# USCCACS/RXMD

Measured on AMD Instinct MI355X. Metric: MD steps/sec (RDX, 979,776 atoms/GPU; one step advances every GPU's domain: weak scaling, wall-clock steps/s of the whole job), higher is better.
Workload: dtype f64

## Files before the change

include/rxmd_hip.h:

```cpp
#ifndef RXMD_HIP_H
#define RXMD_HIP_H
#ifdef __cplusplus
extern "C" {
#endif

typedef struct rxmd_hip_engine *rxmd_handle;

#define RXMD_OK 0
#define RXMD_E_ARG (-1)
#define RXMD_E_FFIELD (-2)
#define RXMD_E_NBUFFER (-3)
#define RXMD_E_MAXNEIGHBS (-4)
#define RXMD_E_MAXNEIGHBS10 (-5)
#define RXMD_E_HIP (-6)
#define RXMD_E_STATE (-7)
#define RXMD_E_COMM (-8)
#define RXMD_E_NAN (-9)

typedef struct rxmd_config {
  const char *ffield_path;
  double lattice[6];
  int vprocs[3];
  int myid;
  int isQEq;
  int NMAXQEq;
  double QEq_tol;
  int qstep;
  double dt_fs;
  double Lex_fqs, Lex_k;
  int nbuffer;
  int maxneighbs;
  int maxneighbs10;
  int device;
  int qeq_mode;
  int lg;
  const char *pqeq_path;
  int efield_dir;
  int reserved1;
  double efield_strength;
} rxmd_config;

void rxmd_hip_default_config(rxmd_config *cfg);
int rxmd_hip_create(const rxmd_config *cfg, rxmd_handle *out);
int rxmd_hip_destroy(rxmd_handle h);
const char *rxmd_hip_last_error(rxmd_handle h);

int rxmd_hip_set_atoms_rxff(rxmd_handle h, int natoms, const double *rec10);
int rxmd_hip_get_atoms_rxff(rxmd_handle h, double *rec10, int capacity);
int rxmd_hip_get_atoms(rxmd_handle h, int capacity, long long *gid, int *type, double *pos, double *v, double *f, double *q);
int rxmd_hip_set_charges(rxmd_handle h, int natoms, const double *q);
int rxmd_hip_set_velocities(rxmd_handle h, int natoms, const double *v);
int rxmd_hip_get_shells(rxmd_handle h, double *spos3, int capacity);
int rxmd_hip_get_bonds(rxmd_handle h, int capacity, int maxnb, int *count, long long *partner_gid, double *bo);
int rxmd_hip_set_shells(rxmd_handle h, int natoms, const double *spos3);

int rxmd_hip_qeq(rxmd_handle h, int *iters, double *est);
int rxmd_hip_force(rxmd_handle h, double pe[14]);
int rxmd_hip_step(rxmd_handle h, int nsteps);
int rxmd_hip_minimise(rxmd_handle h, double ftol, int max_loops, double *pe, long long *evaluations);
int rxmd_hip_last_qeq_iters(rxmd_handle h);
int rxmd_hip_thermostat(rxmd_handle h, int mdmode, double treq_K, double vsfact, double gke_per_atom);
int rxmd_hip_get_energy(rxmd_handle h, double *ke, double *qsum, double pe[14], double astr[6]);

int rxmd_hip_set_lattice(rxmd_handle h, const double lat[6]);
int rxmd_hip_get_lattice(rxmd_handle h, double lat[6]);
int rxmd_hip_set_barostat(rxmd_handle h, int mode, int axes, const double p0_GPa[3], double tau_fs, double bulk_modulus_GPa,
                          int every, double max_strain);
int rxmd_hip_get_barostat(rxmd_handle h, double p6_GPa[6], double mu[3], double *volume, long long *couplings);

int rxmd_hip_set_qeq_precision(rxmd_handle h, int matrix_bits);
int rxmd_hip_get_qeq_precision(rxmd_handle h, int *requested_bits, int *in_use_bits);

int rxmd_hip_QEq(rxmd_handle h, int nbuffer, int natoms, const double *atype, const double *pos, double *q);
int rxmd_hip_FORCE(rxmd_handle h, int nbuffer, int natoms, const double *atype, const double *pos, double *f, const double *q, double pe[14]);
int rxmd_hip_PQEq(rxmd_handle h, int nbuffer, int natoms, const double *atype, const double *pos, double *q, double *spos);
int rxmd_hip_FORCE_pqeq(rxmd_handle h, int nbuffer, int natoms, const double *atype, const double *pos, double *f, const double *q, const double *spos, double pe[14]);
int rxmd_hip_put_lex(rxmd_handle h, int natoms, const double *qsfp, const double *qsfv);
int rxmd_hip_get_lex(rxmd_handle h, int natoms, double *qsfp, double *qsfv);

int rxmd_hip_evaluate_device(rxmd_handle h, int natoms, const long long *gid, const int *type, const double *pos3, const double *q_in,
                             double *f3, double *q_out, double pe[14], double virial6[6], void *stream);

#define RXMD_BONDS_GID 1
long long rxmd_hip_get_bonds_device(rxmd_handle h, int flags, double bo_min, long long capacity, long long *src, long long *dst, double *bo,
                                    double *bo3, double *vec3, void *stream);

int rxmd_hip_bonds_vjp_device(rxmd_handle h, int flags, double bo_min, long long E, const double *grad_bo, const double *grad_bo3,
                              const double *grad_vec3, double *grad_pos3, void *stream);

typedef struct rxmd_stats {
  int natoms, nghost_qeq, nghost_force;
  long long nnz10;
  long long nbonds;
  int max_n10, max_nb;
  int qeq_iters_last; long long qeq_iters_total; long long qeq_calls;
  double ms_qeq, ms_qeq_list, ms_qeq_spmv, ms_force, ms_lists, ms_bo, ms_nonbond, ms_bonded, ms_step_total;
  long long spmv_launches;
  int n10_stride, nbuffer, cells10[3], cells3[3];
  int n_boundary_rows;
  int spmv_noop_launches;
  int reserved[6];
  double ms_ghost_build, ms_migrate, ms_halo, ms_halo_exposed, ms_allreduce, ms_fold;
  long long halo_calls, allreduce_calls;
  double ms_k_list10, ms_k_nonbond, ms_k_e3b, ms_k_e4b, ms_k_ehb, ms_k_bondorder, ms_k_assemble;
  double ms_k_winbuild;
  int win_groups, win_max_units, win_in_use, reserved2;
  double place_ms_first, place_ms_kept;
  double place_total_ms, place_bytes_held;
  int place_draws;
  int spmv_nstep, spmv_var, reserved3;
  double ms_k_blist;
  double ms_bond_exposed;
  int bond_overlap;
  long long spmv_launches_timed;
  int timer_pairs_dropped;
} rxmd_stats;
int rxmd_hip_get_stats(rxmd_handle h, rxmd_stats *out);
int rxmd_hip_reset_timers(rxmd_handle h);
int rxmd_hip_set_qeq_mode(rxmd_handle h, int mode);

int rxmd_hip_get_table(rxmd_handle h, int which, double *out, int capacity);
int rxmd_hip_get_cutoffs(rxmd_handle h, double *rc, int capacity, double *maxrc);
int rxmd_hip_debug_get(rxmd_handle h, int what, double *out, int capacity);

typedef struct rxmd_comm_ops {
  void *ctx;
  long long (*exchange)(void *ctx, int to, const double *send, long long nsend, int from, double *recv, long long cap);
  int (*allreduce_sum)(void *ctx, double *buf, int n);
  long long (*exchange_known)(void *ctx, int to, const double *send, long long nsend, int from, double *recv, long long nrecv);
} rxmd_comm_ops;
int rxmd_hip_set_comm(rxmd_handle h, const rxmd_comm_ops *ops);
int rxmd_hip_rccl_unique_id(unsigned char out128[128]);
int rxmd_hip_comm_init_rccl(rxmd_handle h, const unsigned char id128[128], int rank, int world);
int rxmd_hip_copy_to_host(const double *dev, double *host, long long ndoubles);
int rxmd_hip_copy_to_device(double *dev, const double *host, long long ndoubles);
int rxmd_hip_device_count(void);
int rxmd_hip_set_exchange_buffers(rxmd_handle h, double *send, double *recv, long long ndoubles);
int rxmd_host_comm_selftest(const rxmd_comm_ops *ops, int myid, int nprocs);

long long rxmd_host_geninit(const char *ffield_path, int natoms0, const char *elem4, const double *frac,
                            const double lattice[6], const int mc[3], const int vprocs[3], int myid,
                            double *rec10, long long capacity, double lattice_out[6]);
long long rxmd_host_read_rxff(const char *path, int myid, double lattice_out[6], int vprocs_out[3], double *rec10, long long capacity);
int rxmd_host_ffield_table(const char *ffield_path, const long long *natoms_per_type, int which, double *out, long long capacity);
int rxmd_host_ffield_lg(int on);
int rxmd_host_describe_options(char *buf, int capacity);
int rxmd_hip_has_device_code(void);

#ifdef __cplusplus
}
#endif
#endif
```

rxmd_amd/_lib.py:

```python
import ctypes as C
import os

HERE = os.path.dirname(os.path.abspath(__file__))
SO_PATH = os.environ.get("RXMD_HIP_LIB") or os.path.join(HERE, "librxmd_hip.so")


class RxmdConfig(C.Structure):
    _fields_ = [("ffield_path", C.c_char_p), ("lattice", C.c_double * 6), ("vprocs", C.c_int * 3), ("myid", C.c_int),
                ("isQEq", C.c_int), ("NMAXQEq", C.c_int), ("QEq_tol", C.c_double), ("qstep", C.c_int), ("dt_fs", C.c_double),
                ("Lex_fqs", C.c_double), ("Lex_k", C.c_double), ("nbuffer", C.c_int), ("maxneighbs", C.c_int),
                ("maxneighbs10", C.c_int), ("device", C.c_int), ("qeq_mode", C.c_int), ("lg", C.c_int),
                ("pqeq_path", C.c_char_p), ("efield_dir", C.c_int), ("reserved1", C.c_int), ("efield_strength", C.c_double)]


class RxmdStats(C.Structure):
    _fields_ = [("natoms", C.c_int), ("nghost_qeq", C.c_int), ("nghost_force", C.c_int), ("nnz10", C.c_longlong), ("nbonds", C.c_longlong),
                ("max_n10", C.c_int), ("max_nb", C.c_int), ("qeq_iters_last", C.c_int), ("qeq_iters_total", C.c_longlong), ("qeq_calls", C.c_longlong),
                ("ms_qeq", C.c_double), ("ms_qeq_list", C.c_double), ("ms_qeq_spmv", C.c_double), ("ms_force", C.c_double), ("ms_lists", C.c_double),
                ("ms_bo", C.c_double), ("ms_nonbond", C.c_double), ("ms_bonded", C.c_double), ("ms_step_total", C.c_double),
                ("spmv_launches", C.c_longlong), ("n10_stride", C.c_int), ("nbuffer", C.c_int), ("cells10", C.c_int * 3), ("cells3", C.c_int * 3),
                ("n_boundary_rows", C.c_int), ("spmv_noop_launches", C.c_int), ("reserved", C.c_int * 6),
                ("ms_ghost_build", C.c_double), ("ms_migrate", C.c_double), ("ms_halo", C.c_double), ("ms_halo_exposed", C.c_double),
                ("ms_allreduce", C.c_double), ("ms_fold", C.c_double), ("halo_calls", C.c_longlong), ("allreduce_calls", C.c_longlong),
                ("ms_k_list10", C.c_double), ("ms_k_nonbond", C.c_double), ("ms_k_e3b", C.c_double), ("ms_k_e4b", C.c_double), ("ms_k_ehb", C.c_double),
                ("ms_k_bondorder", C.c_double), ("ms_k_assemble", C.c_double), ("ms_k_winbuild", C.c_double),
                ("win_groups", C.c_int), ("win_max_units", C.c_int), ("win_in_use", C.c_int), ("reserved2", C.c_int),
                ("place_ms_first", C.c_double), ("place_ms_kept", C.c_double),
                ("place_total_ms", C.c_double), ("place_bytes_held", C.c_double), ("place_draws", C.c_int),
                ("spmv_nstep", C.c_int), ("spmv_var", C.c_int), ("reserved3", C.c_int), ("ms_k_blist", C.c_double),
                ("ms_bond_exposed", C.c_double), ("bond_overlap", C.c_int), ("spmv_launches_timed", C.c_longlong), ("timer_pairs_dropped", C.c_int)]

    def asdict(self):
        d = {}
        for name, _ in self._fields_:
            v = getattr(self, name)
            d[name] = list(v) if hasattr(v, "__len__") else v
        d.pop("reserved"); d.pop("reserved2"); d.pop("reserved3")
        return d


EXCHANGE_FN = C.CFUNCTYPE(C.c_longlong, C.c_void_p, C.c_int, C.c_void_p, C.c_longlong, C.c_int, C.c_void_p, C.c_longlong)
ALLREDUCE_FN = C.CFUNCTYPE(C.c_int, C.c_void_p, C.POINTER(C.c_double), C.c_int)


class RxmdCommOps(C.Structure):
    _fields_ = [("ctx", C.c_void_p), ("exchange", EXCHANGE_FN), ("allreduce_sum", ALLREDUCE_FN), ("exchange_known", EXCHANGE_FN)]


H = C.c_void_p
PD = C.c_void_p
SYMBOLS = [
    ("rxmd_hip_default_config", None, [C.POINTER(RxmdConfig)]),
    ("rxmd_hip_create", C.c_int, [C.POINTER(RxmdConfig), C.POINTER(H)]),
    ("rxmd_hip_destroy", C.c_int, [H]),
    ("rxmd_hip_last_error", C.c_char_p, [H]),
    ("rxmd_hip_set_atoms_rxff", C.c_int, [H, C.c_int, PD]),
    ("rxmd_hip_get_atoms_rxff", C.c_int, [H, PD, C.c_int]),
    ("rxmd_hip_get_atoms", C.c_int, [H, C.c_int, PD, PD, PD, PD, PD, PD]),
    ("rxmd_hip_set_charges", C.c_int, [H, C.c_int, PD]),
    ("rxmd_hip_set_velocities", C.c_int, [H, C.c_int, PD]),
    ("rxmd_hip_get_shells", C.c_int, [H, PD, C.c_int]),
    ("rxmd_hip_get_bonds", C.c_int, [H, C.c_int, C.c_int, C.c_void_p, C.c_void_p, PD]),
    ("rxmd_hip_set_shells", C.c_int, [H, C.c_int, PD]),
    ("rxmd_hip_qeq", C.c_int, [H, C.POINTER(C.c_int), C.POINTER(C.c_double)]),
    ("rxmd_hip_force", C.c_int, [H, PD]),
    ("rxmd_hip_step", C.c_int, [H, C.c_int]),
    ("rxmd_hip_get_energy", C.c_int, [H, C.POINTER(C.c_double), C.POINTER(C.c_double), PD, PD]),
    ("rxmd_hip_set_lattice", C.c_int, [H, PD]),
    ("rxmd_hip_get_lattice", C.c_int, [H, PD]),
    ("rxmd_hip_set_barostat", C.c_int, [H, C.c_int, C.c_int, PD, C.c_double, C.c_double, C.c_int, C.c_double]),
    ("rxmd_hip_get_barostat", C.c_int, [H, PD, PD, C.POINTER(C.c_double), C.POINTER(C.c_longlong)]),
    ("rxmd_hip_set_qeq_precision", C.c_int, [H, C.c_int]),
    ("rxmd_hip_get_qeq_precision", C.c_int, [H, C.POINTER(C.c_int), C.POINTER(C.c_int)]),
    ("rxmd_hip_QEq", C.c_int, [H, C.c_int, C.c_int, PD, PD, PD]),
    ("rxmd_hip_FORCE", C.c_int, [H, C.c_int, C.c_int, PD, PD, PD, PD, PD]),
    ("rxmd_hip_evaluate_device", C.c_int, [H, C.c_int, PD, PD, PD, PD, PD, PD, PD, PD, C.c_void_p]),
    ("rxmd_hip_get_bonds_device", C.c_longlong, [H, C.c_int, C.c_double, C.c_longlong, PD, PD, PD, PD, PD, C.c_void_p]),
    ("rxmd_hip_bonds_vjp_device", C.c_int, [H, C.c_int, C.c_double, C.c_longlong, PD, PD, PD, PD, C.c_void_p]),
    ("rxmd_hip_get_stats", C.c_int, [H, C.POINTER(RxmdStats)]),
    ("rxmd_hip_reset_timers", C.c_int, [H]),
    ("rxmd_hip_PQEq", C.c_int, [H, C.c_int, C.c_int, PD, PD, PD, PD]),
    ("rxmd_hip_FORCE_pqeq", C.c_int, [H, C.c_int, C.c_int, PD, PD, PD, PD, PD, PD]),
    ("rxmd_hip_put_lex", C.c_int, [H, C.c_int, PD, PD]),
    ("rxmd_hip_get_lex", C.c_int, [H, C.c_int, PD, PD]),
    ("rxmd_hip_minimise", C.c_int, [H, C.c_double, C.c_int, C.POINTER(C.c_double), C.POINTER(C.c_longlong)]),
    ("rxmd_hip_last_qeq_iters", C.c_int, [H]),
    ("rxmd_hip_thermostat", C.c_int, [H, C.c_int, C.c_double, C.c_double, C.c_double]),
    ("rxmd_hip_rccl_unique_id", C.c_int, [C.c_char_p]),
    ("rxmd_hip_comm_init_rccl", C.c_int, [H, C.c_char_p, C.c_int, C.c_int]),
    ("rxmd_hip_set_qeq_mode", C.c_int, [H, C.c_int]),
    ("rxmd_hip_get_table", C.c_int, [H, C.c_int, PD, C.c_int]),
    ("rxmd_hip_get_cutoffs", C.c_int, [H, PD, C.c_int, C.POINTER(C.c_double)]),
    ("rxmd_hip_debug_get", C.c_int, [H, C.c_int, PD, C.c_int]),
    ("rxmd_hip_set_comm", C.c_int, [H, C.POINTER(RxmdCommOps)]),
    ("rxmd_hip_copy_to_host", C.c_int, [PD, PD, C.c_longlong]),
    ("rxmd_hip_copy_to_device", C.c_int, [PD, PD, C.c_longlong]),
    ("rxmd_hip_device_count", C.c_int, []),
    ("rxmd_hip_set_exchange_buffers", C.c_int, [H, PD, PD, C.c_longlong]),
    ("rxmd_host_comm_selftest", C.c_int, [C.POINTER(RxmdCommOps), C.c_int, C.c_int]),
    ("rxmd_host_geninit", C.c_longlong, [C.c_char_p, C.c_int, C.c_char_p, PD, PD, PD, PD, C.c_int, PD, C.c_longlong, PD]),
    ("rxmd_host_read_rxff", C.c_longlong, [C.c_char_p, C.c_int, PD, PD, PD, C.c_longlong]),
    ("rxmd_host_ffield_table", C.c_int, [C.c_char_p, PD, C.c_int, PD, C.c_longlong]),
    ("rxmd_host_ffield_lg", C.c_int, [C.c_int]),
    ("rxmd_host_describe_options", C.c_int, [C.c_char_p, C.c_int]),
    ("rxmd_hip_has_device_code", C.c_int, []),
]


def describe_options():
    lib = load()
    n = lib.rxmd_host_describe_options(None, 0)
    buf = C.create_string_buffer(n + 1)
    lib.rxmd_host_describe_options(buf, n + 1)
    return buf.value.decode()

_lib = None


def load():
    global _lib
# ... 14 lines not shown
```

rxmd_amd/csrc/bonded.hip:

```cpp
#include "engine.h"

#include <hipcub/hipcub.hpp>

#include <algorithm>
#include <cstdlib>
#include <type_traits>

namespace rxmd {

static inline int nblk(long long n, int b) { return n > 0 ? static_cast<int>((n + b - 1) / b) : 1; }

static constexpr double MINBO0 = 1e-4, cutof2_esub = 1e-4;
static constexpr double MAXANGLE = 0.999999999999, MINANGLE = -0.999999999999, NSMALL = 1e-10;
static constexpr double PI_ = 3.14159265358979;

__device__ inline double wave_sum_b(double v) { return wave_sum64(v); }
__device__ inline void block_energy_add(double v, double *dst) {
  __shared__ double sm[8];
  v = wave_sum_b(v);
  const int w = threadIdx.x >> 6;
  __syncthreads();
  if ((threadIdx.x & 63) == 0) sm[w] = v;
  __syncthreads();
  if (threadIdx.x == 0) {
// ... 894 lines not shown
  }
  if (qn > 0) evaluate(qn);

  wave_lds_sync();
  const double a_cf = s_acc[w][lane][0], a_fx = s_acc[w][lane][1], a_fy = s_acc[w][lane][2], a_fz = s_acc[w][lane][3];
  const double a_cjk1 = s_acc[w][lane][4], a_cjk2 = s_acc[w][lane][5], a_cdk = s_acc[w][lane][6];
  if (sl_me < nj_me) {
    const int o = ob_me + sl_me;
    if (a_cf != 0.0 || a_cjk1 != 0.0) cf1[o] += a_cf + a_cjk1;
    if (a_cjk2 != 0.0) cf2[o] += a_cjk2;
    if (a_cdk != 0.0) cdn[o] += a_cdk;
    if (a_fx != 0.0 || a_fy != 0.0 || a_fz != 0.0) { fnx[o] += a_fx; fny[o] += a_fy; fnz[o] += a_fz; }
  }
  if (self_me) {
    double sx = a_fx, sy = a_fy, sz = a_fz, scd = a_cdk;
    if (ONCE) {
      const int gb = gbase(g_me);
      for (int t = 0; t < nj_me; ++t) { sx -= s_acc[w][gb + t][1]; sy -= s_acc[w][gb + t][2]; sz -= s_acc[w][gb + t][3]; scd += s_acc[w][gb + t][6]; }
    }
    cds[j_me] += scd;
    fx[j_me] += sx; fy[j_me] += sy; fz[j_me] += sz;
  }
  wave_lds_sync();
  }
  }
  e8 = wave_sum_b(e8); e9 = wave_sum_b(e9);
  if (lane == 0) {
    if (e8 != 0.0) atomicAdd(pe + 8, e8);
    if (e9 != 0.0) atomicAdd(pe + 9, e9);
  }
}

__global__ void __launch_bounds__(256) k_e4b_deliver(int nbonds, int TW, const double4 *__restrict__ tkl, unsigned *__restrict__ tflag4,
                                                      double *__restrict__ cf1, double *__restrict__ fnx, double *__restrict__ fny, double *__restrict__ fnz) {
  const int o = xcd_swizzle(blockIdx.x, gridDim.x) * blockDim.x + threadIdx.x;
  if (o >= nbonds) return;
  const int nw = TW >> 2;
  unsigned *fw = tflag4 + static_cast<size_t>(o) * nw;
  const double4 *row = tkl + static_cast<size_t>(o) * TW;
  double c = 0.0, f0 = 0.0, f1 = 0.0, f2 = 0.0;
  bool any = false;
  for (int wd = 0; wd < nw; ++wd) {
    unsigned m = fw[wd];
    if (m == 0u) continue;
    fw[wd] = 0u;
    any = true;
    for (int b = 0; b < 4; ++b, m >>= 8)
      if (m & 255u) { const double4 t = row[4 * wd + b]; c += t.x; f0 += t.y; f1 += t.z; f2 += t.w; }
  }
  if (any) { cf1[o] += c; fnx[o] += f0; fny[o] += f1; fnz[o] += f2; }
}

constexpr int EHB_CAP = 256;
constexpr int EHB_REGIONS = 64;
__global__ void __launch_bounds__(256) k_ehb_donors(int N, unsigned donor_types, const int *__restrict__ boff, const unsigned char *__restrict__ btype, const double *__restrict__ bo0,
                                                     const int *__restrict__ type, int2 *__restrict__ don, int *__restrict__ cnt, int region_cap) {
  const int i = blockIdx.x * blockDim.x + threadIdx.x, lane = threadIdx.x & 63, reg = blockIdx.x & (EHB_REGIONS - 1);
  unsigned hm = 0u;
  if (i < N && ((donor_types >> (type[i] & 31)) & 1u)) {
    const int ob = boff[i], n = min(boff[i + 1] - ob, 32);
    unsigned hs = 0u;
    for (int s = 0; s < n; ++s) hs |= (btype[ob + s] == 2 ? 1u : 0u) << s;
    for (unsigned m_ = hs; m_; m_ &= m_ - 1u) {
      const int s = __ffs(m_) - 1;
      if (bo0[ob + s] > MINBO0) hm |= 1u << s;
    }
  }
  const unsigned long long m = __ballot(hm != 0u);
  if (m == 0ULL) return;
  const int first = __ffsll(static_cast<long long>(m)) - 1;
  int base = 0;
  if (lane == first) base = atomicAdd(cnt + reg, __popcll(m));
  base = __shfl(base, first, 64);
  if (hm != 0u) don[static_cast<size_t>(reg) * region_cap + base + __popcll(m & ((1ULL << lane) - 1ULL))] = make_int2(i, static_cast<int>(hm));
}

template <bool SLOTS>
__global__ void __launch_bounds__(256) k_ehb_sweep(int S10, DevFF ff, const int2 *__restrict__ don, const int *__restrict__ ndon, int region_cap, const int *__restrict__ boff, const int *__restrict__ nbr,
                                                    const int *__restrict__ type, const double *__restrict__ x, const double *__restrict__ y, const double *__restrict__ z,
                                                    const double *__restrict__ bo0, const int *__restrict__ nb10, const int *__restrict__ n10, const double4 *__restrict__ pk, const int *__restrict__ perm,
                                                    double *__restrict__ cf1, double *__restrict__ fnx, double *__restrict__ fny, double *__restrict__ fnz,
                                                    double *__restrict__ fx, double *__restrict__ fy, double *__restrict__ fz, double *__restrict__ pe,
                                                    double *__restrict__ fsx, double *__restrict__ fsy, double *__restrict__ fsz,
                                                    const unsigned short *__restrict__ sl10, const int *__restrict__ rpos, const int *__restrict__ win_k, const unsigned char *__restrict__ stype, int G
#ifdef RXMD_EHB_DEBUG
                                                    , int *dbg, int lim_n, int lim_b, int lim_nb
#endif
                                                    ) {
#ifdef RXMD_EHB_DEBUG
#define EHB_CHECK(code, v, lim, aux) if ((v) < 0 || (v) >= (lim)) { if (atomicCAS(dbg, 0, (code)) == 0) { dbg[1] = (v); dbg[2] = (aux); dbg[3] = (lim); } return; }
#define EHB_CHECKC(code, v, lim, aux) if ((v) < 0 || (v) >= (lim)) { if (atomicCAS(dbg, 0, (code)) == 0) { dbg[1] = (v); dbg[2] = (aux); dbg[3] = (lim); } continue; }
#else
#define EHB_CHECK(code, v, lim, aux)
#define EHB_CHECKC(code, v, lim, aux)
#endif
  __shared__ unsigned s_cand[4][EHB_CAP];
  __shared__ double s_px[4][EHB_CAP], s_py[4][EHB_CAP], s_pz[4][EHB_CAP];
  __shared__ int s_k[4][EHB_CAP];
  __shared__ double s_hp[4][16][4];
  const int lane = threadIdx.x & 63, w = __builtin_amdgcn_readfirstlane(static_cast<int>(threadIdx.x >> 6));
  int pre = ndon[lane & (EHB_REGIONS - 1)];
#pragma unroll
  for (int o = 1; o < EHB_REGIONS; o <<= 1) { const int t = __shfl_up(pre, o, 64); if (lane >= o) pre += t; }
  const int nw = gridDim.x * 4, nd = __shfl(pre, EHB_REGIONS - 1, 64);
  double e10 = 0.0;
  for (int d = blockIdx.x * 4 + w; d < nd; d += nw) {
    const int reg = __popcll(__ballot(pre <= d));
    const int before = reg > 0 ? __shfl(pre, reg - 1, 64) : 0;
    const int2 rec = don[static_cast<size_t>(reg) * region_cap + (d - before)];
    const int i = __builtin_amdgcn_readfirstlane(rec.x);
    const unsigned hmask = static_cast<unsigned>(__builtin_amdgcn_readfirstlane(rec.y));
    EHB_CHECK(1, i, lim_n, d)
    const int ti = type[i], ob = boff[i], n = n10[i] & N10_COUNT;
    EHB_CHECK(2, ob, lim_b - 32, i)
    EHB_CHECK(3, n, S10 + 1, i)
    const double xi = x[i], yi = y[i], zi = z[i];
    const size_t row = static_cast<size_t>(i) * S10;
    const int *wk = SLOTS ? win_k + static_cast<size_t>(rpos[i] / WIN_ROWS) * WIN_MAXUNITS : nullptr;
    const int inx_l = (lane >= 1 && lane <= ff.nso && lane < 16) ? ff.inxn3hb[(ti * ff.n1 + 2) * ff.n1 + lane] : 0;
    if (lane < 16) { const DevHbP hp = ff.hb[inx_l]; s_hp[w][lane][0] = hp.r0hb; s_hp[w][lane][1] = hp.phb1; s_hp[w][lane][2] = hp.phb2; s_hp[w][lane][3] = hp.phb3; }
    int jl = 0; double bl = 0.0, xjl = 0.0, yjl = 0.0, zjl = 0.0;
    if (lane < 32 && ((hmask >> lane) & 1u)) { jl = nbr[ob + lane];
#ifdef RXMD_EHB_DEBUG
      if (jl < 0 || jl >= lim_nb) { if (atomicCAS(dbg, 0, 4) == 0) { dbg[1] = jl; dbg[2] = i; dbg[3] = lane; } jl = 0; }
#endif
      bl = bo0[ob + lane]; xjl = x[jl]; yjl = y[jl]; zjl = z[jl]; }
    V3 fi_t = {0, 0, 0};
    int qn = 0;

    auto flush = [&]() {
      wave_lds_sync();
      for (int q = lane; q < qn; q += 64) {
        EHB_CHECKC(5, static_cast<int>(s_cand[w][q] & NB10_IDX_MASK), lim_nb, i)
        const int ks = static_cast<int>(s_cand[w][q] & NB10_IDX_MASK);
        const double2 pxy = *reinterpret_cast<const double2 *>(pk + ks);
        s_px[w][q] = pxy.x; s_py[w][q] = pxy.y; s_pz[w][q] = reinterpret_cast<const double *>(pk + ks)[2]; s_k[w][q] = perm[ks];
      }
      wave_lds_sync();
      double akx[EHB_CAP / 64], aky[EHB_CAP / 64], akz[EHB_CAP / 64];
#pragma unroll
      for (int b = 0; b < EHB_CAP / 64; ++b) { akx[b] = 0.0; aky[b] = 0.0; akz[b] = 0.0; }
      for (unsigned hm = hmask; hm; hm &= hm - 1u) {
        const int s = __ffs(hm) - 1;
        const int j = __shfl(jl, s, 64);
        const double BOij = __shfl(bl, s, 64);
        const double xj = __shfl(xjl, s, 64), yj = __shfl(yjl, s, 64), zj = __shfl(zjl, s, 64);
        const V3 rij = {xi - xj, yi - yj, zi - zj};
        const double nij = sqrt(dot(rij, rij));
        double cfs = 0.0, nterm = 0.0;
        V3 fi_s = {0, 0, 0}, fj_s = {0, 0, 0};
#pragma unroll
        for (int b = 0; b < EHB_CAP / 64; ++b) {
          const int qq = 64 * b + lane;
          if (qq >= qn) continue;
          const int k = s_k[w][qq];
          if (k == j || k == i) continue;
          const double *hp = s_hp[w][(s_cand[w][qq] >> NB10_IDX_BITS) & 15u];
          const double r0hb = hp[0], phb1 = hp[1], phb2 = hp[2], phb3 = hp[3];
          const double pxk = s_px[w][qq], pyk = s_py[w][qq], pzk = s_pz[w][qq];
          const V3 rik = {xi - pxk, yi - pyk, zi - pzk};
          if (!(dot(rik, rik) < 100.0)) continue;
          const V3 rjk = {xj - pxk, yj - pyk, zj - pzk};
          const double njk = sqrt(dot(rjk, rjk));
          double cos_ijk = -dot(rij, rjk) / (nij * njk);
          if (cos_ijk > MAXANGLE) cos_ijk = MAXANGLE;
          if (cos_ijk < MINANGLE) cos_ijk = MINANGLE;
          const double sh2 = 0.5 * (1.0 - cos_ijk);
          const double sin_xhz4 = sh2 * sh2, cos_xhz1 = 1.0 - cos_ijk;
          const double exp_hb2 = exp(-phb2 * BOij);
          const double exp_hb3 = exp(-phb3 * (r0hb / njk + njk / r0hb - 2.0));
          const double PEhb = phb1 * (1.0 - exp_hb2) * exp_hb3 * sin_xhz4;
          e10 += PEhb; nterm += 1.0;
          cfs += phb1 * phb2 * exp_hb2 * exp_hb3 * sin_xhz4;
          const double CEhb2 = -0.5 * phb1 * (1.0 - exp_hb2) * exp_hb3 * cos_xhz1;
          const double CEhb3 = -PEhb * phb3 * (-r0hb / (njk * njk) + 1.0 / r0hb) * (1.0 / njk);
          V3 fi, fk;
          angle_forces(CEhb2, rij, nij, rjk, njk, fi, fk);
          const V3 ff3 = {CEhb3 * rjk.x, CEhb3 * rjk.y, CEhb3 * rjk.z};
          fi_s.x += fi.x; fi_s.y += fi.y; fi_s.z += fi.z;
          fj_s.x += -(fi.x + fk.x) - ff3.x; fj_s.y += -(fi.y + fk.y) - ff3.y; fj_s.z += -(fi.z + fk.z) - ff3.z;
          akx[b] += fk.x + ff3.x; aky[b] += fk.y + ff3.y; akz[b] += fk.z + ff3.z;
        }
        cfs = wave_sum_b(cfs); nterm = wave_sum_b(nterm);
        fj_s.x = wave_sum_b(fj_s.x); fj_s.y = wave_sum_b(fj_s.y); fj_s.z = wave_sum_b(fj_s.z);
        fi_t.x += fi_s.x; fi_t.y += fi_s.y; fi_t.z += fi_s.z;
        if (lane == 0 && nterm > 0.0) {
          const int o = ob + s;
          cf1[o] += cfs;
          fnx[o] += fj_s.x; fny[o] += fj_s.y; fnz[o] += fj_s.z;
        }
      }
#pragma unroll
      for (int b = 0; b < EHB_CAP / 64; ++b) {
        const int qq = 64 * b + lane;
        if (qq < qn && (akx[b] != 0.0 || aky[b] != 0.0 || akz[b] != 0.0)) {
          const int ks = static_cast<int>(s_cand[w][qq] & NB10_IDX_MASK);
          EHB_CHECKC(6, ks, lim_nb, qq)
          atomicAdd(fsx + ks, akx[b]); atomicAdd(fsy + ks, aky[b]); atomicAdd(fsz + ks, akz[b]);
        }
      }
// ... 52 lines not shown
  k_elnpr_atoms<<<nblk(N, 256), 256, 0, stream>>>(N, dff, boff, type, bt1, bt2, delta, deltalp, dDlp, ecoef, pe_d);
  k_elnpr_bonds<<<nblk(nbonds_res, 256), 256, 0, stream>>>(nbonds_res, dff, bown, nbr, btype, type, bo2, bo3, delta, deltalp, dDlp, ecoef, cf1, cf2, cf3, cdn);
  Timed kt3(this, &st.ms_k_e3b);
  if (opt.e3b_queue != 0 && dff.n1 <= 8 && dff.nvaty <= 255) {
    const int maxl = h_err[2];
    auto go = [&](auto kern, int na, int minw) {
      const int NG = nblk(N, 4 * na);
      kern<<<std::min(NG, (num_cu * minw + 7) & ~7), 256, 0, stream>>>(N, NG, dff, boff, nbr, btype, type, pos[0], pos[1], pos[2], bo0, bo2, bo3, delta, nlp, dDlp, epen, ecoa, cf1, cf2, cf3, cdn, fnx, fny, fnz,
                                                                     cds, frc[0], frc[1], frc[2], pe_d, static_cast<int>(opt.e4b_probe));
    };
    const bool w3 = opt.e3b_queue == 3;
    if (maxl <= 12) { if (w3) go(k_e3q<3, 16>, 16, 3); else go(k_e3q<2, 16>, 16, 2); }
    else if (maxl <= 24) { if (w3) go(k_e3q<3, 8>, 8, 3); else go(k_e3q<2, 8>, 8, 2); }
    else { if (w3) go(k_e3q<3, 4>, 4, 3); else go(k_e3q<2, 4>, 4, 2); }
  } else
    k_e3b<<<nblk(N, 256), 256, 4 * 5 * E3B_CAP * sizeof(double), stream>>>(N, dff, boff, nbr, btype, type, pos[0], pos[1], pos[2], bo0, bo2, bo3, delta, nlp, dDlp, epen, ecoa, cf1, cf2, cf3, cdn, fnx, fny, fnz,
                                          cds, frc[0], frc[1], frc[2], pe_d);
  RX_HIP(hipGetLastError());
  kt3.end();
  BoxImg bx;
  for (int a = 0; a < 3; ++a) { for (int c = 0; c < 3; ++c) { bx.H[3 * a + c] = box.H[a][c]; bx.Hi[3 * a + c] = box.Hi[a][c]; } bx.L[a] = box.lat[a]; }
  bx.ortho = grid.ortho; bx.probe = 0;
  bx.probe = static_cast<int>(opt.e4b_probe);
  const int want = static_cast<int>(opt.e4b_slots);
  const bool narrow = h_err[2] <= 15 && want != 32 && want != 4;
  Timed kt4(this, &st.ms_k_e4b);
  bool once = opt.e4b_once != 0;
  const int TW = (std::max(h_err[2], 8) + 3) & ~3;
  if (once) {
    const size_t need = static_cast<size_t>(std::max(nbonds, 1)) * TW;
    if (need > e4b_cap) {
      size_t fre = 0, tot = 0;
      RX_HIP(hipMemGetInfo(&fre, &tot));
      const size_t want_entries = need + need / 4;
      if (want_entries * 33 > (fre + e4b_cap * 33) / 2) once = false; else alloc_e4b_delivery(want_entries);
    }
  }
  if (once) {
    if (e4b_dirty) RX_HIP(hipMemsetAsync(e4b_flag, 0, e4b_cap, stream));
    e4b_dirty = true;
  }
  const int n4 = dff.n1 * dff.n1 * dff.n1 * dff.n1;
  const size_t tor_bytes = (dff.n1 <= 8 && dff.ntoty <= 255) ? static_cast<size_t>((n4 + 15) & ~15) : 0;
  const bool wpb1 = opt.e4b_wpb == 1;
  auto launch = [&](auto inst, int per_wave) {
    constexpr int L = decltype(inst)::value;
    auto go = [&](auto kern, int wpb) {
      const int VB = nblk(N, per_wave * wpb);
      const int grid = opt.e4b_persist != 0 ? std::min(VB, (num_cu * (12 / wpb) + 7) & ~7) : VB;
      kern<<<grid, 64 * wpb, tor_bytes, stream>>>(N, dff, boff, nbr, btype, nbrcnt, type, gid, pos[0], pos[1], pos[2], bo0, bo2, delta, etor, econ, cf1, cf2, cdn, fnx, fny, fnz,
                                                  cds, frc[0], frc[1], frc[2], pe_d, bx, brev, e4b_t, e4b_flag, TW, VB);
    };
    if (once) { if (wpb1) go(k_e4b<L, true, 1>, 1); else go(k_e4b<L, true, 4>, 4); }
    else      { if (wpb1) go(k_e4b<L, false, 1>, 1); else go(k_e4b<L, false, 4>, 4); }
    RX_HIP(hipGetLastError());
  };
  if (want == 4) launch(std::integral_constant<int, 1>{}, 4);
  else if (narrow && want != 16) launch(std::integral_constant<int, 0>{}, 8);
  else if (narrow) launch(std::integral_constant<int, 4>{}, 4);
  else launch(std::integral_constant<int, 5>{}, 2);
  if (once) {
    k_e4b_deliver<<<nblk(nbonds, 256), 256, 0, stream>>>(nbonds, TW, e4b_t, reinterpret_cast<unsigned *>(e4b_flag), cf1, fnx, fny, fnz);
    e4b_dirty = false;
  }
  kt4.end();
  Timed kth(this, &st.ms_k_ehb);
  if (ehb_donor_types != 0u) {
    const int region_cap = (nblk(N, 256) + EHB_REGIONS - 1) / EHB_REGIONS * 256;
    if (static_cast<size_t>(region_cap) * EHB_REGIONS > ehb_don_cap) throw EngineError(RXMD_E_STATE, "hydrogen-bond donor list: capacity");
    RX_HIP(hipMemsetAsync(ehb_cnt, 0, sizeof(int) * EHB_REGIONS, stream));
    k_ehb_donors<<<nblk(N, 256), 256, 0, stream>>>(N, ehb_donor_types, boff, btype, bo0, type, ehb_don, ehb_cnt, region_cap);
    k_zero3<<<nblk(G, 256), 256, 0, stream>>>(G, fsort[0], fsort[1], fsort[2]);
    if (ehb_blocks_per_cu == 0) {
      int nbk = 0;
      RX_HIP(hipOccupancyMaxActiveBlocksPerMultiprocessor(&nbk, k_ehb_sweep<false>, 256, 0));
      ehb_blocks_per_cu = std::max(nbk, 1);
      RX_HIP(hipOccupancyMaxActiveBlocksPerMultiprocessor(&nbk, k_ehb_sweep<true>, 256, 0));
      ehb_blocks_per_cu_sl = std::max(nbk, 1);
    }
    const bool slots = !nb10_valid;
    const int ehb_grid = num_cu * (slots ? ehb_blocks_per_cu_sl : ehb_blocks_per_cu);
#ifdef RXMD_EHB_DEBUG
    RX_HIP(hipMemsetAsync(ehb_cnt + EHB_REGIONS, 0, 4 * sizeof(int), stream));
#define RX_EHB(SL) k_ehb_sweep<SL><<<ehb_grid, 256, 0, stream>>>(S10, dff, ehb_don, ehb_cnt, region_cap, boff, nbr, type, pos[0], pos[1], pos[2], bo0, nb10, n10, sorted_xyzi, perm, cf1, fnx, fny, fnz, frc[0], frc[1], frc[2], pe_d, fsort[0], fsort[1], fsort[2], sl10, rpos, win_k, sorted_type, G, ehb_cnt + EHB_REGIONS, N, static_cast<int>(bcap), NB)
    if (slots) RX_EHB(true); else RX_EHB(false);
#undef RX_EHB
    { int hd[EHB_REGIONS + 4]; RX_HIP(hipMemcpyAsync(hd, ehb_cnt, sizeof(hd), hipMemcpyDeviceToHost, stream)); RX_HIP(hipStreamSynchronize(stream));
      for (int r = 1; r < EHB_REGIONS; ++r) hd[0] += hd[r];
      hd[4] = hd[EHB_REGIONS]; hd[5] = hd[EHB_REGIONS + 1]; hd[6] = hd[EHB_REGIONS + 2]; hd[7] = hd[EHB_REGIONS + 3];
      std::fprintf(stderr, "[ehb debug] donors %d  blocks/CU %d  first violation: code %d value %d aux %d lim %d   (N %d bcap %zu NB %d S10 %d rows10 %d)\n", hd[0], ehb_blocks_per_cu, hd[4], hd[5], hd[6], hd[7], N, bcap, NB, S10, rows10); }
#else
#define RX_EHB(SL) k_ehb_sweep<SL><<<ehb_grid, 256, 0, stream>>>(S10, dff, ehb_don, ehb_cnt, region_cap, boff, nbr, type, pos[0], pos[1], pos[2], bo0, nb10, n10, sorted_xyzi, perm, cf1, fnx, fny, fnz, frc[0], frc[1], frc[2], pe_d, fsort[0], fsort[1], fsort[2], sl10, rpos, win_k, sorted_type, G)
    if (slots) RX_EHB(true); else RX_EHB(false);
#undef RX_EHB
#endif
    k_add_sorted3<<<nblk(G, 256), 256, 0, stream>>>(G, perm, fsort[0], fsort[1], fsort[2], frc[0], frc[1], frc[2]);
  }
}

}
```

rxmd_amd/csrc/capi.hip:

```cpp
#include <algorithm>
#include <chrono>
#include <cmath>
#include <cstdio>
#include <cstring>
#include <fstream>
#include <new>
#include <string>
#include <vector>

#include "engine.h"

namespace rxmd { double stream_probe_ms(Engine &e, int blocks); void spmv_bisect_ms(Engine &e, double *out4); void spmv_isolated_ms(Engine &e, double *out); void spmv_tile_probe_ms(Engine &e, double *out); }
using rxmd::Engine;
using rxmd::EngineError;

struct rxmd_hip_engine {
  Engine *e = nullptr;
  std::string err;
};

static thread_local std::string g_create_error;

template <class F>
static int guarded(rxmd_handle h, F &&f) {
// ... 319 lines not shown
int rxmd_hip_QEq(rxmd_handle h, int nbuffer, int natoms, const double *atype, const double *pos, double *q) {
  if (!atype || !pos || !q) return RXMD_E_ARG;
  return guarded(h, [&](Engine &e) {
    require_lex(e, natoms);
    upload_reference_arrays(e, nbuffer, natoms, atype, pos, q);
    e.lex_pending = false;
    e.qeq();
    RX_HIP(hipMemcpy(q, e.q, sizeof(double) * natoms, hipMemcpyDeviceToHost));
  });
}

int rxmd_hip_FORCE(rxmd_handle h, int nbuffer, int natoms, const double *atype, const double *pos, double *f, const double *q, double pe[14]) {
  if (!atype || !pos || !f || !q) return RXMD_E_ARG;
  return guarded(h, [&](Engine &e) {
    upload_reference_arrays(e, nbuffer, natoms, atype, pos, q);
    e.force();
    for (int a = 0; a < 3; ++a)
      RX_HIP(hipMemcpy(f + a * static_cast<size_t>(nbuffer), e.frc[a], sizeof(double) * natoms, hipMemcpyDeviceToHost));
    if (pe) std::memcpy(pe, e.pe, sizeof(double) * 14);
  });
}

static void upload_shells(Engine &e, int nbuffer, int natoms, const double *spos) {
  if (!e.ff.pqeq) throw EngineError(RXMD_E_STATE, "the engine was created without a PQEq parameter file");
  for (int a = 0; a < 3; ++a) RX_HIP(hipMemcpy(e.shl[a], spos + a * static_cast<size_t>(nbuffer), sizeof(double) * natoms, hipMemcpyHostToDevice));
}
int rxmd_hip_PQEq(rxmd_handle h, int nbuffer, int natoms, const double *atype, const double *pos, double *q, double *spos) {
  if (!atype || !pos || !q || !spos) return RXMD_E_ARG;
  return guarded(h, [&](Engine &e) {
    require_lex(e, natoms);
    upload_reference_arrays(e, nbuffer, natoms, atype, pos, q);
    e.lex_pending = false;
    upload_shells(e, nbuffer, natoms, spos);
    e.qeq();
    RX_HIP(hipMemcpy(q, e.q, sizeof(double) * natoms, hipMemcpyDeviceToHost));
    for (int a = 0; a < 3; ++a) RX_HIP(hipMemcpy(spos + a * static_cast<size_t>(nbuffer), e.shl[a], sizeof(double) * natoms, hipMemcpyDeviceToHost));
  });
}
int rxmd_hip_FORCE_pqeq(rxmd_handle h, int nbuffer, int natoms, const double *atype, const double *pos, double *f, const double *q, const double *spos, double pe[14]) {
  if (!atype || !pos || !f || !q || !spos) return RXMD_E_ARG;
  return guarded(h, [&](Engine &e) {
    upload_reference_arrays(e, nbuffer, natoms, atype, pos, q);
    upload_shells(e, nbuffer, natoms, spos);
    e.force();
    for (int a = 0; a < 3; ++a)
      RX_HIP(hipMemcpy(f + a * static_cast<size_t>(nbuffer), e.frc[a], sizeof(double) * natoms, hipMemcpyDeviceToHost));
    if (pe) std::memcpy(pe, e.pe, sizeof(double) * 14);
  });
}

int rxmd_hip_evaluate_device(rxmd_handle h, int natoms, const long long *gid, const int *type, const double *pos3, const double *q_in,
                             double *f3, double *q_out, double pe[14], double virial6[6], void *stream) {
  return guarded(h, [&](Engine &e) { e.evaluate_device(natoms, gid, type, pos3, q_in, f3, q_out, pe, virial6, static_cast<hipStream_t>(stream)); });
}

long long rxmd_hip_get_bonds_device(rxmd_handle h, int flags, double bo_min, long long capacity, long long *src, long long *dst, double *bo,
                                    double *bo3, double *vec3, void *stream) {
  long long n = 0;
  const int rc = guarded(h, [&](Engine &e) { n = e.bonds_device(flags, bo_min, capacity, src, dst, bo, bo3, vec3, static_cast<hipStream_t>(stream)); });
  return rc < 0 ? rc : n;
}

int rxmd_hip_bonds_vjp_device(rxmd_handle h, int flags, double bo_min, long long E, const double *grad_bo, const double *grad_bo3,
                              const double *grad_vec3, double *grad_pos3, void *stream) {
  return guarded(h, [&](Engine &e) { e.bonds_vjp_device(flags, bo_min, E, grad_bo, grad_bo3, grad_vec3, grad_pos3, static_cast<hipStream_t>(stream)); });
}

int rxmd_hip_get_stats(rxmd_handle h, rxmd_stats *out) {
  if (!out) return RXMD_E_ARG;
  return guarded(h, [&](Engine &e) {
    if (e.atoms_set && e.lists_valid) {
      RX_HIP(hipStreamSynchronize(e.stream));
      e.collect_timers();
      std::vector<int> n10(e.N), nb(e.G);
      RX_HIP(hipMemcpy(n10.data(), e.n10, sizeof(int) * e.N, hipMemcpyDeviceToHost));
      RX_HIP(hipMemcpy(nb.data(), e.nbrcnt, sizeof(int) * e.G, hipMemcpyDeviceToHost));
      long long s10 = 0, sb = 0; int m10 = 0, mb = 0;
      for (int v : n10) { v &= rxmd::N10_COUNT; s10 += v; m10 = std::max(m10, v); }
      for (int v : nb) { sb += v; mb = std::max(mb, v); }
      e.st.nnz10 = s10; e.st.nbonds = sb; e.st.max_n10 = m10; e.st.max_nb = mb;
    }
    e.st.natoms = e.N;
    e.st.n_boundary_rows = (e.multi() && e.lists_valid && !e.rows_split_pending_invalid()) ? e.n_bnd : 0;
    e.st.win_groups = e.win_groups; e.st.win_max_units = e.win_maxunits; e.st.win_in_use = e.win_used ? 1 : 0;
    e.st.spmv_launches_timed = e.pass_timed_n;
    e.st.ms_qeq_spmv = e.pass_timed_n > 0 ? e.pass_timed_ms / static_cast<double>(e.pass_timed_n) * static_cast<double>(e.st.spmv_launches) : 0.0;
    *out = e.st;
  });
}

int rxmd_hip_reset_timers(rxmd_handle h) {
  return guarded(h, [&](Engine &e) {
    e.st.ms_qeq = e.st.ms_qeq_list = e.st.ms_qeq_spmv = e.st.ms_force = e.st.ms_lists = e.st.ms_bo = e.st.ms_nonbond = e.st.ms_bonded = e.st.ms_step_total = 0.0;
    e.st.spmv_launches = 0; e.st.spmv_noop_launches = 0; e.st.qeq_iters_total = 0; e.st.qeq_calls = 0;
    e.st.ms_ghost_build = e.st.ms_migrate = e.st.ms_halo = e.st.ms_halo_exposed = e.st.ms_allreduce = e.st.ms_fold = 0.0;
    e.st.halo_calls = e.st.allreduce_calls = 0; e.st.timer_pairs_dropped = 0; e.pass_timed_ms = 0.0; e.pass_timed_n = 0; e.st.spmv_launches_timed = 0;
    e.st.ms_k_list10 = e.st.ms_k_nonbond = e.st.ms_k_e3b = e.st.ms_k_e4b = e.st.ms_k_ehb = e.st.ms_k_bondorder = e.st.ms_k_assemble = e.st.ms_k_winbuild = e.st.ms_k_blist = e.st.ms_bond_exposed = 0.0;
  });
}

int rxmd_hip_set_qeq_mode(rxmd_handle h, int mode) {
  return guarded(h, [&](Engine &e) {
    if (mode != 0 && mode != 1) throw EngineError(RXMD_E_ARG, "qeq_mode must be 0 or 1");
    e.cfg.qeq_mode = mode;
  });
}

int rxmd_hip_get_table(rxmd_handle h, int which, double *out, int capacity) {
  int n = 0;
  const int rc = guarded(h, [&](Engine &e) {
    if (!e.tables_ready) throw EngineError(RXMD_E_STATE, "tables are built when atoms are first set");
    n = e.ff.nboty;
    if (!out || capacity < n * rxmd::NTABLE) throw EngineError(RXMD_E_ARG, "capacity too small");
    const std::vector<double> *src[5] = {&e.ff.tblEvdw, &e.ff.tbldEvdw, &e.ff.tblEclmb, &e.ff.tbldEclmb, &e.ff.tblQEq};
    if (which < 0 || which > 4) throw EngineError(RXMD_E_ARG, "which must be 0..4");
    for (int r = 1; r <= n; ++r)
      for (int i = 1; i <= rxmd::NTABLE; ++i) out[static_cast<size_t>(r - 1) * rxmd::NTABLE + (i - 1)] = (*src[which])[static_cast<size_t>(r) * (rxmd::NTABLE + 2) + i];
  });
  return rc < 0 ? rc : n;
}

int rxmd_hip_get_cutoffs(rxmd_handle h, double *rc, int capacity, double *maxrc) {
  int n = 0;
  const int r = guarded(h, [&](Engine &e) {
    if (!e.tables_ready) throw EngineError(RXMD_E_STATE, "cutoffs are computed when atoms are first set");
    n = e.ff.nboty;
    if (rc) { if (capacity < n) throw EngineError(RXMD_E_ARG, "capacity too small"); for (int k = 1; k <= n; ++k) rc[k - 1] = e.ff.bond[k].rc; }
    if (maxrc) *maxrc = e.ff.maxrc;
  });
  return r < 0 ? r : n;
}

int rxmd_hip_debug_get(rxmd_handle h, int what, double *out, int capacity) {
  int n = 0;
  const int rc = guarded(h, [&](Engine &e) {
    if (!e.atoms_set) throw EngineError(RXMD_E_STATE, "atoms were never set");
    RX_HIP(hipStreamSynchronize(e.stream));
    auto pull_d = [&](const double *src, int cnt, int stride, int off) {
      std::vector<double> t(cnt);
      RX_HIP(hipMemcpy(t.data(), src, sizeof(double) * cnt, hipMemcpyDeviceToHost));
      for (int i = 0; i < cnt; ++i) out[static_cast<size_t>(i) * stride + off] = t[i];
    };
    const int G = e.G, N = e.N;
    switch (what) {
      case 0: n = G; if (capacity < n) throw EngineError(RXMD_E_ARG, "capacity"); pull_d(e.delta, G, 1, 0); break;
      case 1: n = G; if (capacity < n) throw EngineError(RXMD_E_ARG, "capacity"); pull_d(e.deltap, G, 1, 0); break;
      case 2: { n = G; if (capacity < n) throw EngineError(RXMD_E_ARG, "capacity"); std::vector<int> t(G); RX_HIP(hipMemcpy(t.data(), e.nbrcnt, sizeof(int) * G, hipMemcpyDeviceToHost)); for (int i = 0; i < G; ++i) out[i] = t[i]; break; }
      case 3: n = G; if (capacity < 3 * n) throw EngineError(RXMD_E_ARG, "capacity"); for (int a = 0; a < 3; ++a) pull_d(e.pos[a], G, 3, a); break;
      case 4: { n = G; if (capacity < n) throw EngineError(RXMD_E_ARG, "capacity"); std::vector<long long> t(G); RX_HIP(hipMemcpy(t.data(), e.gid, sizeof(long long) * G, hipMemcpyDeviceToHost)); for (int i = 0; i < G; ++i) out[i] = static_cast<double>(t[i]); break; }
      case 5: { n = G; if (capacity < n) throw EngineError(RXMD_E_ARG, "capacity"); std::vector<int> t(G); RX_HIP(hipMemcpy(t.data(), e.type, sizeof(int) * G, hipMemcpyDeviceToHost)); for (int i = 0; i < G; ++i) out[i] = t[i]; break; }
      case 6: { n = N; if (capacity < n) throw EngineError(RXMD_E_ARG, "capacity"); std::vector<int> t(N); RX_HIP(hipMemcpy(t.data(), e.n10, sizeof(int) * N, hipMemcpyDeviceToHost)); for (int i = 0; i < N; ++i) out[i] = t[i] & rxmd::N10_COUNT; break; }
      case 7: {
        n = N; if (capacity < n) throw EngineError(RXMD_E_ARG, "capacity");
        std::vector<int> c(N); RX_HIP(hipMemcpy(c.data(), e.n10, sizeof(int) * N, hipMemcpyDeviceToHost));
        for (int &v : c) v &= rxmd::N10_COUNT;
        std::vector<double> row(e.S10);
        for (int i = 0; i < N; ++i) {
          RX_HIP(hipMemcpy(row.data(), e.hess + static_cast<size_t>(i) * e.S10, sizeof(double) * c[i], hipMemcpyDeviceToHost));
          double s = 0; for (int k = 0; k < c[i]; ++k) s += row[k];
          out[i] = s;
        }
        break;
      }
      case 8: n = G; if (capacity < n) throw EngineError(RXMD_E_ARG, "capacity"); pull_d(e.cd, G, 1, 0); break;
      case 9: n = G; if (capacity < n) throw EngineError(RXMD_E_ARG, "capacity"); pull_d(e.q, G, 1, 0); break;
      case 10: n = G; if (capacity < n) throw EngineError(RXMD_E_ARG, "capacity"); pull_d(e.cc_, G, 1, 0); break;
      case 14: {
        n = 2; if (capacity < 2) throw EngineError(RXMD_E_ARG, "capacity");
        out[0] = rxmd::poison_enabled() ? 1.0 : 0.0;
        RX_HIP(hipMemcpy(out + 1, e.hess + (e.S10 - 1), sizeof(double), hipMemcpyDeviceToHost));
        break;
      }
      case 15: n = 2; if (capacity < 2) throw EngineError(RXMD_E_ARG, "capacity"); out[0] = e.nb10_valid ? 1.0 : 0.0; out[1] = e.nb10_sticky ? 1.0 : 0.0; break;
      case 13: {
        n = static_cast<int>(e.est_trace.size()); if (capacity < n) throw EngineError(RXMD_E_ARG, "capacity");
        for (int k = 0; k < n; ++k) out[k] = e.est_trace[k];
        break;
      }
      case 11: {
        n = N; if (capacity < n) throw EngineError(RXMD_E_ARG, "capacity");
        if (!e.win_valid) { for (int i = 0; i < N; ++i) out[i] = -1.0; break; }
        e.require_nb10();
        RX_HIP(hipStreamSynchronize(e.stream));
        const size_t nrs = static_cast<size_t>(e.win_groups) * rxmd::WIN_ROWS;
        std::vector<int> c(N), rs(nrs), wc(e.win_groups), wk(static_cast<size_t>(e.win_groups) * rxmd::WIN_MAXUNITS);
        RX_HIP(hipMemcpy(c.data(), e.n10, sizeof(int) * N, hipMemcpyDeviceToHost));
        RX_HIP(hipMemcpy(rs.data(), e.rows_sorted, sizeof(int) * nrs, hipMemcpyDeviceToHost));
        RX_HIP(hipMemcpy(wc.data(), e.win_cnt, sizeof(int) * e.win_groups, hipMemcpyDeviceToHost));
        RX_HIP(hipMemcpy(wk.data(), e.win_k, sizeof(int) * wk.size(), hipMemcpyDeviceToHost));
        std::vector<int> ent(e.S10); std::vector<unsigned short> sl(e.S10);
        for (int i = 0; i < N; ++i) out[i] = -2.0;
        for (size_t r = 0; r < nrs; ++r) {
          const int i = rs[r], g = static_cast<int>(r / rxmd::WIN_ROWS);
          if (i < 0 || i >= N) continue;
          const int cnt = c[i] & rxmd::N10_COUNT;
          RX_HIP(hipMemcpy(ent.data(), e.nb10 + static_cast<size_t>(i) * e.S10, sizeof(int) * cnt, hipMemcpyDeviceToHost));
          RX_HIP(hipMemcpy(sl.data(), e.sl10 + static_cast<size_t>(i) * e.S10, sizeof(unsigned short) * cnt, hipMemcpyDeviceToHost));
          int good = 0;
          for (int k = 0; k < cnt; ++k) {
            const unsigned en = static_cast<unsigned>(ent[k]);
            const int slot = sl[k] & 0x7fff, unit = slot / rxmd::WIN_UNIT;
            const bool gh = (sl[k] & 0x8000) != 0;
            if (unit < wc[g] && wk[static_cast<size_t>(g) * rxmd::WIN_MAXUNITS + unit] + (slot % rxmd::WIN_UNIT) == static_cast<int>(en & rxmd::NB10_IDX_MASK) && gh == ((en & rxmd::NB10_GHOST) != 0)) ++good;
          }
          out[i] = good;
        }
        break;
      }
      case 12: {
        n = 4; if (capacity < 8) throw EngineError(RXMD_E_ARG, "capacity");
        const int grids[4] = {2048, 8192, 32768, 131072};
        for (int g = 0; g < 4; ++g) { out[2 * g] = rxmd::stream_probe_ms(e, grids[g]); out[2 * g + 1] = static_cast<double>(e.rows10) * e.S10 * 8.0; }
        n = 8; break;
      }
#ifdef RXMD_EXPERIMENTS
      case 104: n = 20; if (capacity < 20) throw EngineError(RXMD_E_ARG, "capacity"); rxmd::spmv_isolated_ms(e, out); break;
      case 105: n = 5; if (capacity < 5) throw EngineError(RXMD_E_ARG, "capacity"); rxmd::spmv_tile_probe_ms(e, out); break;
      case 102: n = 7; if (capacity < 7) throw EngineError(RXMD_E_ARG, "capacity"); rxmd::spmv_bisect_ms(e, out); break;
#endif
      default: throw EngineError(RXMD_E_ARG, "unknown debug tap");
    }
  });
  return rc < 0 ? rc : n;
}

int rxmd_hip_copy_to_host(const double *dev, double *host, long long n) {
  if (n < 0 || (n > 0 && (!dev || !host))) return RXMD_E_ARG;
  return (n == 0 || hipMemcpy(host, dev, sizeof(double) * static_cast<size_t>(n), hipMemcpyDeviceToHost) == hipSuccess) ? RXMD_OK : RXMD_E_HIP;
}
int rxmd_hip_copy_to_device(double *dev, const double *host, long long n) {
  if (n < 0 || (n > 0 && (!dev || !host))) return RXMD_E_ARG;
  return (n == 0 || hipMemcpy(dev, host, sizeof(double) * static_cast<size_t>(n), hipMemcpyHostToDevice) == hipSuccess) ? RXMD_OK : RXMD_E_HIP;
}
int rxmd_hip_device_count(void) {
  int n = 0;
  return hipGetDeviceCount(&n) == hipSuccess ? n : 0;
}

int rxmd_hip_set_comm(rxmd_handle h, const rxmd_comm_ops *ops) {
  return guarded(h, [&](Engine &e) {
    if (!ops) { e.has_comm = false; return; }
    e.comm = *ops; e.has_comm = true;
  });
}

int rxmd_hip_comm_init_rccl(rxmd_handle h, const unsigned char id128[128], int rank, int world) {
  return guarded(h, [&](Engine &e) {
    if (!id128) throw EngineError(RXMD_E_ARG, "NULL unique id");
    e.rccl_init(id128, rank, world);
  });
}

int rxmd_hip_set_exchange_buffers(rxmd_handle h, double *send, double *recv, long long ndoubles) {
  return guarded(h, [&](Engine &e) {
    if (!send || !recv || ndoubles < 1024) throw EngineError(RXMD_E_ARG, "bad exchange buffers");
    e.bufs.free_group(rxmd::G_XBUF);
    e.xbuf_send = send; e.xbuf_recv = recv; e.xbuf_doubles = static_cast<size_t>(ndoubles); e.xbuf_owned = false;
  });
}

int rxmd_host_comm_selftest(const rxmd_comm_ops *ops, int myid, int nprocs) {
  if (!ops || !ops->exchange || !ops->allreduce_sum || nprocs < 1 || myid < 0 || myid >= nprocs) return RXMD_E_ARG;
  const int right = (myid + 1) % nprocs, left = (myid + nprocs - 1) % nprocs;
  std::vector<double> snd(4096), rcv(4096);
  for (int dir = 0; dir < 2; ++dir) {
    const int to = dir ? left : right, from = dir ? right : left;
    const long long ns = 7 + 13 * myid + dir;
    for (long long k = 0; k < ns; ++k) snd[k] = 1000.0 * myid + k + 0.5 * dir;
    const long long nr = ops->exchange(ops->ctx, to, snd.data(), ns, from, rcv.data(), 4096);
    if (nr != 7 + 13 * from + dir) return RXMD_E_COMM;
    for (long long k = 0; k < nr; ++k) if (rcv[k] != 1000.0 * from + k + 0.5 * dir) return RXMD_E_COMM;
    const long long nz = ops->exchange(ops->ctx, to, snd.data(), 0, from, rcv.data(), 4096);
    if (nz != 0) return RXMD_E_COMM;
    if (ops->exchange_known) {
      const long long nk = ops->exchange_known(ops->ctx, to, snd.data(), ns, from, rcv.data(), 7 + 13 * from + dir);
      if (nk != 7 + 13 * from + dir) return RXMD_E_COMM;
      for (long long k = 0; k < nk; ++k) if (rcv[k] != 1000.0 * from + k + 0.5 * dir) return RXMD_E_COMM;
    }
  }
  double v[3] = {1.0 * (myid + 1), 0.25, -2.0 * myid};
// ... 105 lines not shown
```

rxmd_amd/csrc/engine.h:

```cpp
#pragma once
#include <hip/hip_runtime.h>

#include <string>
#include <type_traits>
#include <vector>

#include "../../include/rxmd_hip.h"
#include "ffparams.h"
#include "options.h"

namespace rxmd {

#define RX_HIP(call)                                                                              \
  do {                                                                                            \
    hipError_t e_ = (call);                                                                       \
    if (e_ != hipSuccess) throw EngineError(RXMD_E_HIP, std::string(#call) + ": " + hipGetErrorString(e_)); \
  } while (0)

struct EngineError {
  int code;
  std::string msg;
  EngineError(int c, std::string m) : code(c), msg(std::move(m)) {}
};

// ... 28 lines not shown
struct Box {
  double H[3][3], Hi[3][3];
  double lat[6];
  double lbox[3];
  double obox[3];
  double volume;
};

struct Grid {
  int n[3];
  double org[3];
  double inv[3];
  int ncell;
  int fz, nzf;
  int nfine;
  double wid[3];
  double cw[3];
  double iwz;
  int ortho;
  int probe;
};

struct RefMesh {
  double Hi[9], obox[3];
  double lc[3];
  double nbl[3];
  double nblr[3];
  double qlo[3], qhi[3];
};

constexpr int WAVE = 64;

enum { S_MU = 0, S_LMIN_S, S_LMIN_T, S_GOLD_S, S_GOLD_T, S_GNEW_S, S_GNEW_T, S_EST, S_GH_S, S_GH_T, S_HSH_S, S_HSH_T, S_SSUM, S_TSUM, S_BETA_S, S_BETA_T, S_RAW0, S_RAW1, S_RAW2, S_RAW3, S_RAW4, S_RAW5, S_RAW6, S_RAW7, S_STOP, S_STOP1, S_TOL, S_COUNT };
constexpr int SCAL_CG_N = 32, SCAL_N = 208, H_SCAL_N = 320;
constexpr int SCAL_PE = 32, SCAL_PE_N = 16, H_SCAL_PE = 32;
constexpr int SCAL_ASTR = 48;
constexpr int SCAL_PRINTE = 56, H_SCAL_PRINTE = 56;
constexpr int SCAL_REDUCE = 64, H_SCAL_REDUCE = 48;
constexpr int SCAL_EVAL_HEAD = 72, H_SCAL_EVAL_VIRIAL = 310;
constexpr int H_SCAL_TOL = 60;
constexpr int S_SNAP = 128, S_SNAP_STRIDE = 32;
constexpr int H_SCAL_SNAP = 64, H_SNAP_STRIDE = 64, H_SNAP_SEQ = 63;
constexpr int H_SCAL_TSUM = 192, H_SCAL_TSUM_N = 6 * 16;
constexpr int SCAL_BAR_HEAD = 192, SCAL_BAR_STEP = 200, H_SCAL_BAR_OUT = 288, H_SCAL_BAR_REDUCE = 304;
struct ScalSlot { int at, n; };
constexpr bool slots_disjoint_within(const ScalSlot *s, int count, int total) {
  for (int i = 0; i < count; ++i) for (int j = 0; j <= i; ++j)
    if (s[i].at < 0 || s[i].n <= 0 || s[i].at + s[i].n > total || (j < i && s[i].at < s[j].at + s[j].n && s[j].at < s[i].at + s[i].n)) return false;
  return true;
}
constexpr ScalSlot SCAL_SLOTS[] = {{0, SCAL_CG_N}, {SCAL_PE, SCAL_PE_N}, {SCAL_ASTR, 6}, {SCAL_PRINTE, 6}, {SCAL_REDUCE, 8}, {SCAL_EVAL_HEAD, 6}, {S_SNAP, 2 * S_SNAP_STRIDE}, {SCAL_BAR_HEAD, 6}, {SCAL_BAR_STEP, 6}};
constexpr ScalSlot H_SCAL_SLOTS[] = {{0, SCAL_CG_N}, {H_SCAL_PE, SCAL_PE_N}, {H_SCAL_REDUCE, 8}, {H_SCAL_PRINTE, 2}, {H_SCAL_TOL, 1}, {H_SCAL_SNAP, 2 * H_SNAP_STRIDE}, {H_SCAL_TSUM, H_SCAL_TSUM_N}, {H_SCAL_BAR_OUT, 9}, {H_SCAL_BAR_REDUCE, 6}, {H_SCAL_EVAL_VIRIAL, 6}};
static_assert(slots_disjoint_within(SCAL_SLOTS, sizeof(SCAL_SLOTS) / sizeof(ScalSlot), SCAL_N), "two slots of the device scalar block overlap, or one leaves the block");
static_assert(slots_disjoint_within(H_SCAL_SLOTS, sizeof(H_SCAL_SLOTS) / sizeof(ScalSlot), H_SCAL_N), "two slots of the pinned scalar block overlap, or one leaves the block");
static_assert(S_COUNT <= SCAL_CG_N && S_COUNT <= S_SNAP_STRIDE && S_COUNT <= H_SNAP_SEQ, "the CG scalars fit their range and either snapshot slot");
static_assert(S_RAW0 + 8 <= S_STOP, "the eight raw sums stay inside the CG scalars");

__device__ inline int xcd_swizzle(int bid, int nwg) {
  const int q = nwg >> 3, r = nwg & 7, x = bid & 7;
  return (x < r ? x * (q + 1) : r * (q + 1) + (x - r) * q) + (bid >> 3);
}

template <int CTRL, int ROW_MASK>
__device__ inline double dpp_move(double v) {
  const int lo = __double2loint(v), hi = __double2hiint(v);
  if (ROW_MASK == 0xf) return __hiloint2double(__builtin_amdgcn_mov_dpp(hi, CTRL, ROW_MASK, 0xf, false), __builtin_amdgcn_mov_dpp(lo, CTRL, ROW_MASK, 0xf, false));
  return __hiloint2double(__builtin_amdgcn_update_dpp(0, hi, CTRL, ROW_MASK, 0xf, false), __builtin_amdgcn_update_dpp(0, lo, CTRL, ROW_MASK, 0xf, false));
}
__device__ inline double wave_sum64(double v) {
  v += dpp_move<0xb1, 0xf>(v);
  v += dpp_move<0x4e, 0xf>(v);
  v += dpp_move<0x141, 0xf>(v);
  v += dpp_move<0x140, 0xf>(v);
  v += dpp_move<0x142, 0xa>(v);
  v += dpp_move<0x143, 0xc>(v);
  return __hiloint2double(__builtin_amdgcn_readlane(__double2hiint(v), 63), __builtin_amdgcn_readlane(__double2loint(v), 63));
}

#ifndef WIN_ROWS_DEF
#define WIN_ROWS_DEF 16
#endif
constexpr int WIN_ROWS = WIN_ROWS_DEF;
constexpr int WIN_UNIT = 8;
constexpr int WIN_MAXUNITS = 448;
constexpr int WIN_BMW = 2048;

enum class Fill : unsigned char { None, Zero, Pattern };
void *dev_alloc(size_t bytes, Fill fill);
void dev_free(void *p);
void *pinned_alloc(size_t bytes, bool coherent_mapped);
void pinned_free(void *p);
bool poison_enabled();
template <class T> void dev_alloc(T *&p, size_t n, Fill fill) { p = static_cast<T *>(dev_alloc(n * sizeof(T), fill)); }
template <class T> void dev_free(T *&p) { dev_free(static_cast<void *>(p)); p = nullptr; }

struct Engine;
enum class Dim : unsigned char { Fixed, NB, Rows10, List10, Cap };
enum class Refill : unsigned char { Never, Whole, Ghosts };
enum class Space : unsigned char { Device, Pinned, PinnedCoherent };
enum { G_SETUP, G_BOND, G_WIN, G_CELLSTART, G_LIST10, G_PARTIALS, G_ON_DEMAND, G_CUBTMP = G_ON_DEMAND, G_FFBLOB, G_PQBLOB, G_E4B, G_SEG, G_SEG_PINNED, G_XBUF, G_DH_SERVE, G_BGRAPH, G_BVJP, G_COUNT };
enum : unsigned { BUF_PQEQ = 1u, BUF_RESIDENT = 2u, BUF_QEQ_F32 = 4u };
struct Buf { void **pp; size_t elem; int group; Dim dim; size_t mul, add_; Fill fill; Refill refill; unsigned flags; Space space; size_t bytes; };
struct Buffers {
  std::vector<Buf> v;
  size_t cap[G_COUNT] = {};
  template <class T> void add(T *&p, int group, Dim dim, size_t mul, size_t addend, Fill fill, Refill refill, unsigned flags = 0) {
    size_t elem = 1;
    if constexpr (!std::is_void_v<T>) elem = sizeof(T);
    add_raw(reinterpret_cast<void **>(&p), elem, group, dim, mul, addend, fill, refill, flags);
  }
  void add_raw(void **pp, size_t elem, int group, Dim dim, size_t mul, size_t addend, Fill fill, Refill refill, unsigned flags = 0) {
    v.push_back(Buf{pp, elem, group, dim, mul, addend, fill, refill, flags, Space::Device, 0});
  }
  template <class T> void add_pinned(T *&p, int group, size_t n, bool coherent_mapped) {
    v.push_back(Buf{reinterpret_cast<void **>(&p), sizeof(T), group, Dim::Fixed, 0, n, Fill::Zero, Refill::Never, 0u, coherent_mapped ? Space::PinnedCoherent : Space::Pinned, 0});
  }
  size_t count(const Buf &b, const Engine &e) const;
  void alloc_one(Buf &b, const Engine &e); void free_one(Buf &b);
  void alloc_setup(const Engine &e);
  void alloc_group(const Engine &e, int group, size_t capacity = 0);
  void free_group(int group); void free_all();
  void refill(const Engine &e);
  std::vector<std::vector<char>> save_residents(const Engine &e) const;
  void restore_residents(const std::vector<std::vector<char>> &h);
};
constexpr size_t EHB_DON_EXTRA = 64 * 256 + 256;

template <class T> struct Restore {
  T &ref; const T old;
  explicit Restore(T &r) : ref(r), old(r) {}
  Restore(T &r, T inside) : ref(r), old(r) { r = inside; }
  ~Restore() { ref = old; }
};
struct StreamSwap {
  hipStream_t &a, &b; bool *inside;
  StreamSwap(hipStream_t &a_, hipStream_t &b_, bool *inside_ = nullptr) : a(a_), b(b_), inside(inside_) { std::swap(a, b); if (inside) *inside = true; }
  ~StreamSwap() { if (inside) *inside = false; std::swap(a, b); }
};

struct ScaleArgs;
struct WinPassArgs; struct RowPassArgs;
struct Engine {
  const Options opt = Options::from_env();
  rxmd_config cfg{};
  std::string ffield_path, pqeq_path, err;
  ForceField ff;
  Box box{};
  int vID[3] = {0, 0, 0}, target_node[7] = {0}, nprocs = 1;
  double dt = 0, Lex_w2 = 0;
  std::vector<double> dthm, hmas;
  rxmd_comm_ops comm{};
  bool has_comm = false, tables_ready = false, atoms_set = false, lists_valid = false, ghosts_valid = false;

  int NB = 0, MAXNB = 30, S10 = 0, rows10 = 0;
  int max_row10 = 0, min_row10 = 0;
  int num_cu = 256;
  int N = 0, G = 0, copyptr[7] = {0};
  int cc[3] = {1, 1, 1};
  double shell[3] = {0, 0, 0};
  Grid grid{};
  RefMesh rmesh{};

  Buffers bufs;
  void declare_buffers();
  DevFF dff{};
  void *ffblob = nullptr, *pqblob = nullptr;
// ... 90 lines not shown
  long long bonds_device(int flags, double bo_min, long long capacity, long long *src_d, long long *dst_d, double *bo_d, double *bo3_d, double *vec3_d, hipStream_t user);
  int *bg_flag = nullptr, *bg_off = nullptr;
  long long select_bonds(double bo_min);
  void bonds_vjp_device(int flags, double bo_min, long long E, const double *grad_bo_d, const double *grad_bo3_d, const double *grad_vec3_d, double *grad_pos3_d, hipStream_t user);
  double *bv_c1 = nullptr, *bv_c2 = nullptr, *bv_c3 = nullptr, *bv_t = nullptr, *bv_cc = nullptr, *bv_g[3] = {nullptr, nullptr, nullptr}; int bv_nb = 0;
  void build_ghosts_and_lists(bool qeq_prepass = false);
  void qeq_start_vectors();
  int *rows_int = nullptr, *rows_bnd = nullptr; int n_bnd = 0; bool rows_split_pending = false;
  bool rows_split_pending_invalid() const { return n_bnd < 0 || n_bnd > N; }
  bool sums_from_list = false;
  void qeq();
  struct WinInstance { int nstep, var; bool f32; };
  WinInstance win_instance() const;
  WinPassArgs win_args(bool roword = false) const;
  RowPassArgs row_args() const;
  struct PassCall { int mode; bool store; double2 *ra = nullptr, *rg = nullptr; const int *rowlist = nullptr; int nrows = 0, pbase = 0; const double *stopflag = nullptr; bool roword = false; };
  int matrix_pass(const PassCall &c);
  void cg_reduce(int stage, int nsets, const double *stopflag = nullptr);
  struct CgCall { int nmax, vb, vb_upd; bool onepass, runahead, est_with_update, cg_scatter; };
  double qeq_start(const CgCall &c);
  int qeq_runahead(const CgCall &c, double &Est);
  int qeq_host_paced(const CgCall &c, double &Est);
  struct TimedSection;
  void qeq_finish(int it, double Est, TimedSection &t_qeq);
  void force(bool defer_host_read = false, bool observe_energy = true);
  void finish_force();
  bool force_pending = false;
  unsigned long long snap_seq = 0; double snap_expect[2] = {0.0, 0.0};
  void wait_snapshot(int parity, double seq);
  unsigned long long pass_counter = 0; bool pass_timed_k[2] = {false, false}; double pass_timed_ms = 0.0; long long pass_timed_n = 0;
  void step(int nsteps);
  void migrate();
  void thermostat(int mdmode, double treq_K, double vsfact, double gke);
  int minimise(double ftol, int max_loops, double *pe_final, long long *evaluations);

  void set_lattice(const double lat[6], bool check_ranks);
  void apply_lattice(const double lat[6]);
  void check_lattice(const double lat[6]) const;
  struct BoxGeom { int cc[3]; double shell[3]; Grid grid; RefMesh rmesh; };
  BoxGeom geometry_for(const Box &b) const;
  void derive_box_geometry();
  long long capacity_want(const double shell_n[3]) const;
  void grow_capacity(int new_nb);
  void alloc_window_groups(size_t ng);
  size_t cellstart_cap = 0, win_ng_cap = 0;
  long long nsize_setup = 0;
  int bar_mode = 0, bar_axes = 7, bar_every = 1;
  double bar_p0[3] = {0, 0, 0}, bar_tau = 0, bar_B = 0, bar_max = 0;
  double bar_p6[6] = {0, 0, 0, 0, 0, 0}, bar_mu[3] = {1, 1, 1}, bar_vol = 0;
  long long bar_couplings = 0;
  void set_barostat(int mode, int axes, const double p0[3], double tau_fs, double bulk_GPa, int every, double max_strain);
  void barostat_couple();

  void setup_after_atoms(const std::vector<long long> &natoms_per_type_global);
  void upload_ff();
  void alloc_device();
  void free_device();
  void ghost_build();
  void ghost_build_fused(); void migrate_fused(); void ensure_seg_buffers(int nblocks);
  unsigned long long *h_pub = nullptr; unsigned pub_seq = 0u;
  void pinned_wait(int nwords, unsigned seq, const char *what);
  int *seg_cnt = nullptr, *seg_tot = nullptr, *h_seg = nullptr; unsigned char *seg_code_ = nullptr; int seg_blocks_cap = 0;
  void bin_cells();
  void build_bonded_list(bool pack_only = false);
  void build_list10();
  void build_prologue(int what);
  bool list10_retry = false;
  void build_windows();
  void tune_window_placement();
  bool place_tuned = false;
  int *rows_sorted = nullptr, *win_k = nullptr, *win_cnt = nullptr;
  int *win_flag = nullptr;
  int *rowcols = nullptr, *grp_base = nullptr;
  int *win_gint = nullptr, *win_gbnd = nullptr; int win_nbnd = 0;
  unsigned short *sl10 = nullptr;
  double2 *r_qst = nullptr, *r_hst = nullptr, *r_hst2 = nullptr, *r_gst = nullptr, *r_sall = nullptr, *r_sgh = nullptr, *r_wall = nullptr, *r_wgh = nullptr;
  bool rows_live = false;
  int *r_type = nullptr, *r_n10 = nullptr, *r_xpos = nullptr, *rpos = nullptr, *g_rrow = nullptr;
  int win_groups = 0, win_maxunits = 0;
  size_t win_groups_bound(long long n) const { return win_groups_bound_for(grid, n); }
  static size_t win_groups_bound_for(const Grid &g, long long n) { return static_cast<size_t>(n) / WIN_ROWS + static_cast<size_t>(g.n[0]) * g.n[1] + 1; }
  double qeq_iters_smooth = -1.0;
  bool win_valid = false, win_used = false;
  void halo_refresh(double2 *v2, double *v1);
  void halo_staged(double *v, int ncomp);
  struct Round { int d0, n; };
  bool stage_pairs = true;
  bool known_counts_pair() const { return stage_pairs && (nccl || (has_comm && comm.exchange_known)); }
  int *flags2 = nullptr, *scanout2 = nullptr;
  int *sel_flags(int k) const { return k ? flags2 : flags; }
  int *sel_scan(int k) const { return k ? scanout2 : scanout; }
  int stage_sends(int d) const { return sendoff[d + 1] - sendoff[d]; }
  int stage_ghosts(int d) const { return copyptr[d] - copyptr[d - 1]; }
  void select_round(Round r, int nscan, double dr, int skip_dead, int total[2]);
  void exchange_round(Round r, bool reverse, const long long nsend[2], long long nrecv[2], bool counts_known);
  void rccl_exchange_round(int n, const int to[2], const int from[2], const long long nsend[2], long long nrecv[2], bool counts_known);
  long long *gowner = nullptr;
  bool halo_direct = false, dh_ready = false;
  int *dh_ghost = nullptr, *dh_serve = nullptr;
  int *dh_keys = nullptr, *dh_keys2 = nullptr, *dh_vals = nullptr, *dh_off = nullptr; int dh_serve_cap = 0;
  std::vector<long long> dh_need_off, dh_serve_off;
  void direct_halo_setup();
  void halo_direct_exchange(double *v, int ncomp);
  void exchange_many(const std::vector<long long> &soff, const std::vector<long long> &roff, int ncomp);
  void rccl_exchange_many(const std::vector<long long> &soff, const std::vector<long long> &roff, int ncomp);
  void ensure_xbuf(size_t doubles);
  size_t migrate_xbuf_doubles(size_t from_send_count) const;
  void grow_xbuf_keep_send(size_t need, size_t keep);
  bool multi() const { return nprocs > 1 || force_staged; }
  void *nccl = nullptr; double *cnt_dev = nullptr, *cnt_host = nullptr; bool force_staged = false, force_remote = false;
  void rccl_init(const unsigned char id128[128], int rank, int world);
  void rccl_destroy();
  void rccl_allreduce_dev(double *dev, int n);
  void sync_stream();
  void sync_event(hipEvent_t e);
  double comm_timeout_s = 300.0;
  bool spin_wait = true;
  void allreduce_scal4(int n = 4);
  void allreduce_host(double *buf, int n);
  void allreduce_device(double *dev, int n, int h_stage, int site = -1);
  void ghost_build_staged();
  void sorted_copy(const double2 *v);
  void fold_ghost_forces(double *fx, double *fy, double *fz);
  void bond_orders();
  void bonded_energies();
  void charge_halo();
  void nonbonded(bool to_fnb = false, bool energy = true);
  void pqeq_sorted_shells();
  void pqeq_update_shells();
  bool pq_matrix_stale = false;
  void nonbonded_pqeq();
  void efield_force();
  void remove_momentum();
  void type_sums_device();
  double *tsum = nullptr; struct ScaleArgs *sargs = nullptr;
  void assemble_forces();
  void accumulate_stress(bool kinetic);
  void check_device_error(const char *where, bool fetch = true);
  void fetch_device_error();
  double reduce_partials(int ncomp, int nblocks, double *out);
  struct KtPair { hipEvent_t a = nullptr, b = nullptr; double *dst = nullptr, *dst2 = nullptr; long long *cnt = nullptr; double scale = 1.0; };
  std::vector<KtPair> kt_free, kt_pending;
  KtPair kt_cur{};
  unsigned long long kt_site_calls[4] = {0, 0, 0, 0};
  int kt_every = 1, kt_phase = 0;
  struct Timed {
    Engine &e; const bool section; KtPair p{};
    Timed(Engine *eng, double *dst, double *dst2 = nullptr, long long *cnt = nullptr, int site = -1, bool section_ = false) : e(*eng), section(section_) {
      double scale = 1.0;
      if (!section && site < 0 && e.kt_every > 1) {
        if (cnt) { *cnt += 1; cnt = nullptr; }
        if (e.kt_phase % e.kt_every != 0) return;
        scale = static_cast<double>(e.kt_every);
      }
      if (site >= 0) {
        if (cnt) { *cnt += 1; cnt = nullptr; }
        const unsigned long long every = static_cast<unsigned long long>(e.opt.pass_timing_every > 1 ? e.opt.pass_timing_every : 1);
        if ((e.kt_site_calls[site & 3]++ % every) != 0) return;
        scale = static_cast<double>(every);
      }
      if (e.kt_free.empty() || (!section && e.kt_cur.a)) { if (e.kt_free.empty()) ++e.st.timer_pairs_dropped; return; }
      p = e.kt_free.back(); e.kt_free.pop_back();
      p.dst = dst; p.dst2 = dst2; p.cnt = cnt; p.scale = scale;
      hipEventRecord(p.a, e.stream);
      if (!section) e.kt_cur = p;
    }
// ... 20 lines not shown
```

rxmd_amd/csrc/engine.hip:

```cpp
#include "engine.h"
#include <cstdlib>

#include <hipcub/hipcub.hpp>

#include <algorithm>
#include <cmath>
#include <cstring>

namespace rxmd {

static const double UTIME = 1e3 / 20.455;
static const int NMINCELL = 4;
static inline int nblk(long long n, int b) { return n > 0 ? static_cast<int>((n + b - 1) / b) : 1; }


static void make_box(Box &b, const double lat[6], const int vprocs[3], const int vID[3]) {
  const double pi = std::atan(1.0) * 4.0;
  const double la = lat[0], lb = lat[1], lc = lat[2];
  const double lal = lat[3] * pi / 180.0, lbe = lat[4] * pi / 180.0, lga = lat[5] * pi / 180.0;
  const double hh1 = lc * (std::cos(lal) - std::cos(lbe) * std::cos(lga)) / std::sin(lga);
  const double hh2 = lc * std::sqrt(1.0 - std::cos(lal) * std::cos(lal) - std::cos(lbe) * std::cos(lbe) - std::cos(lga) * std::cos(lga) +
                                    2 * std::cos(lal) * std::cos(lbe) * std::cos(lga)) / std::sin(lga);
  double(*H)[3] = b.H;
  H[0][0] = la; H[1][0] = 0; H[2][0] = 0;
// ... 487 lines not shown
}
__global__ void k_sorted_pos(int G, int N, const int *perm, const int *groot, const double *x, const double *y, const double *z, const int *type, double4 *out, unsigned char *st, int *rootperm, int *invpos) {
  const int k = blockIdx.x * blockDim.x + threadIdx.x;
  if (k >= G) return;
  const int i = perm[k];
  const double xi = x[i], yi = y[i], zi = z[i];
  const int ti = type[i];
  out[k] = make_double4(xi, yi, zi, __longlong_as_double((static_cast<long long>(ti) << 32) | static_cast<unsigned int>(i)));
  st[k] = static_cast<unsigned char>(ti);
  rootperm[k] = (i < N) ? i : groot[i];
  invpos[i] = k;
}
__global__ void k_sorted_vec(int G, const int *__restrict__ rootperm, const double2 *__restrict__ v, double2 *__restrict__ xs) {
  const int k = blockIdx.x * blockDim.x + threadIdx.x;
  if (k < G) xs[k] = v[rootperm[k]];
}

void Engine::bin_cells() {
  k_cell_ids<<<nblk(G, 256), 256, 0, stream>>>(G, grid, spos[0], spos[1], spos[2], cellid, perm_in);
  size_t tb = cubtmp_bytes;
  int bits = 1;
  while ((1LL << bits) < grid.nfine + 1 && bits < 31) ++bits;
  RX_HIP(hipcub::DeviceRadixSort::SortPairs(cubtmp, tb, cellid, cellid_sorted, perm_in, perm, G, 0, bits, stream));
  k_cell_starts<<<nblk(grid.nfine + 1, 256), 256, 0, stream>>>(G, grid.nfine, cellid_sorted, cellstart);
  sorted_positions();
  if (ff.pqeq) pqeq_sorted_shells();
}
void Engine::sorted_positions() {
  k_sorted_pos<<<nblk(G, 256), 256, 0, stream>>>(G, N, perm, groot, pos[0], pos[1], pos[2], type, sorted_xyzi, sorted_type, rootperm, invpos);
  sorted_w_charge = false;
}

void Engine::sorted_copy(const double2 *v) {
  if (multi()) {
    halo_staged(reinterpret_cast<double *>(const_cast<double2 *>(v)), 2);
    k_sorted_vec<<<nblk(G, 256), 256, 0, stream>>>(G, perm, v, xs);
    return;
  }
  k_sorted_vec<<<nblk(G, 256), 256, 0, stream>>>(G, rootperm, v, xs);
}

__global__ void k_publish_words(int n, const int *__restrict__ src, unsigned long long *hpub, unsigned seq) {
  if (threadIdx.x < n) __hip_atomic_store(hpub + threadIdx.x, (static_cast<unsigned long long>(seq) << 32) | static_cast<unsigned>(src[threadIdx.x]), __ATOMIC_RELAXED, __HIP_MEMORY_SCOPE_SYSTEM);
}
void Engine::build_ghosts_and_lists(bool qeq_prepass) {
  if (!atoms_set) throw EngineError(RXMD_E_STATE, "atoms were never set");
  TimedSection t_lists(this, &st.ms_lists);
  bufs.refill(*this);
  { Timed kt(this, &st.ms_ghost_build); ghost_build(); }
  bin_cells();
  build_prologue(3);
  { Timed kt(this, &st.ms_k_blist); build_bonded_list(); }
  sums_from_list = qeq_prepass;
  if (qeq_prepass) qeq_start_vectors();
  build_list10();
  if (h_pub && !multi()) {
    const unsigned seq = ++pub_seq;
    k_publish_words<<<1, 64, 0, stream>>>(16, d_err, h_pub, seq);
    pinned_wait(16, seq, "list build");
    for (int k = 0; k < 16; ++k) h_err[k] = static_cast<int>(h_pub[k] & 0xffffffffull);
  } else
    fetch_device_error();
  if (static_cast<size_t>(h_err[7]) > bcap) {
    free_bond_tables();
    alloc_bond_tables(static_cast<size_t>(h_err[7]) + static_cast<size_t>(h_err[7]) / 4 + 4096);
    build_bonded_list(true);
    fetch_device_error();
  }
  try {
    check_device_error("list build", false);
  } catch (const EngineError &er) {
    if (er.code != RXMD_E_MAXNEIGHBS10 || cfg.maxneighbs10 > 0) { collect_timers(); throw; }
    const int need = h_err[1];
    S10 = (static_cast<int>(need * 1.1) + 64 + 63) / 64 * 64;
    bufs.free_group(G_LIST10); bufs.alloc_group(*this, G_LIST10);
    st.n10_stride = S10;
    { Restore<bool> retry(list10_retry, true); build_list10(); }
    check_device_error("list build");
  }
  nbonds = h_err[7]; nbonds_res = h_err[9];
  win_groups = h_err[8];
  max_row10 = h_err[3]; min_row10 = std::min(h_err[4], h_err[3]);
  win_maxunits = h_err[5]; win_valid = win_groups > 0 && h_err[6] == 0 && win_maxunits > 0 && (!multi() || (win_nbnd >= 0 && win_nbnd <= win_groups)) && !opt.spmv_no_win;
  lists_valid = true;
  if (!nb10_valid && !win_valid) require_nb10();
  collect_timers();
  pq_matrix_stale = false;
}

void Engine::set_qeq_precision(int bits) {
  if (bits != 64 && bits != 32) throw EngineError(RXMD_E_ARG, "matrix_bits must be 64 or 32");
  if (bits == 32 && ff.pqeq) throw EngineError(RXMD_E_ARG, "the fp32 matrix stream is not available with PQEq (it carries a second value stream)");
  if (bits == qeq_bits_req) return;
  qeq_bits_req = bits;
  lists_valid = false;
  if (hess) {
    sync_stream();
    bufs.free_group(G_LIST10); bufs.alloc_group(*this, G_LIST10);
    nb10_valid = false;
  }
}

struct Mat3 { double m[9]; };
__global__ void k_affine_remap(int n, Mat3 M, double *__restrict__ x, double *__restrict__ y, double *__restrict__ z,
                               double *__restrict__ dx, double *__restrict__ dy, double *__restrict__ dz) {
  const int i = blockIdx.x * blockDim.x + threadIdx.x;
  if (i >= n) return;
  const double r0 = x[i], r1 = y[i], r2 = z[i];
  x[i] = M.m[0] * r0 + M.m[1] * r1 + M.m[2] * r2;
  y[i] = M.m[3] * r0 + M.m[4] * r1 + M.m[5] * r2;
  z[i] = M.m[6] * r0 + M.m[7] * r1 + M.m[8] * r2;
  if (dx) {
    const double d0 = dx[i], d1 = dy[i], d2 = dz[i];
    dx[i] = M.m[0] * d0 + M.m[1] * d1 + M.m[2] * d2;
    dy[i] = M.m[3] * d0 + M.m[4] * d1 + M.m[5] * d2;
    dz[i] = M.m[6] * d0 + M.m[7] * d1 + M.m[8] * d2;
  }
}

void Engine::check_lattice(const double lat[6]) const {
  if (!lattice_spans_box(lat)) throw EngineError(RXMD_E_ARG, "lattice does not span a box (edges must be positive, angles inside (0,180) and not coplanar)");
  if (tables_ready)
    for (int a = 0; a < 3; ++a)
      if (static_cast<int>(lat[a] / cfg.vprocs[a] / ff.maxrc) < 1) throw EngineError(RXMD_E_ARG, "local box smaller than the bond cutoff");
  if (bar_mode == 2 && !lattice_orthorhombic(lat)) throw EngineError(RXMD_E_ARG, "the per-axis barostat (mode 2) is on: the lattice must stay orthorhombic");
}

long long Engine::capacity_want(const double shell_n[3]) const {
  const long long nsize = std::max<long long>(nsize_setup, N);
  double fac = 1.0;
  for (int a = 0; a < 3; ++a) fac *= 1.0 + 2.0 * std::min(shell_n[a] / box.lbox[a], 1.0);
  const long long want = static_cast<long long>(nsize * fac * 1.12) + 4096;
  return std::min<long long>(want, 2000000000LL);
}

void Engine::set_lattice(const double lat[6], bool check_ranks) {
  bool local_ok = true;
  std::string why;
  try { check_lattice(lat); } catch (const EngineError &er) { if (nprocs == 1 || !check_ranks) throw; local_ok = false; why = er.msg; }
  if (check_ranks && nprocs > 1) {
    double s[7];
    for (int a = 0; a < 6; ++a) s[a] = cfg.myid == 0 ? lat[a] : 0.0;
    s[6] = local_ok ? 0.0 : 1.0;
    allreduce_host(s, 7);
    double bad = 0.0;
    for (int a = 0; a < 6; ++a) if (!(s[a] == lat[a])) bad = 1.0;
    allreduce_host(&bad, 1);
    if (!local_ok) throw EngineError(RXMD_E_ARG, why);
    if (s[6] != 0.0) throw EngineError(RXMD_E_ARG, "set_lattice is collective: another rank's lattice failed its checks");
    if (bad != 0.0) throw EngineError(RXMD_E_ARG, "set_lattice is collective: the ranks passed different lattices");
  }
  apply_lattice(lat);
}

void Engine::apply_lattice(const double lat[6]) {
  if (force_pending) finish_force();
  Box nbx{};
  make_box(nbx, lat, cfg.vprocs, vID);
  BoxGeom g{};
  if (tables_ready) {
    g = geometry_for(nbx);
    const long long want = cfg.nbuffer <= 0 ? capacity_want(g.shell) : NB;
    if (want >= (1LL << NB10_IDX_BITS)) throw EngineError(RXMD_E_NBUFFER, "the new lattice needs more than 2^26 atoms+ghosts per GPU (the packed 10 A list entry)");
    if (want > NB) grow_capacity(static_cast<int>(want));
    const size_t need_cs = static_cast<size_t>(g.grid.nfine) + 2, need_ng = win_groups_bound_for(g.grid, rows10) + 1;
    if (need_cs > cellstart_cap || need_ng > win_ng_cap) sync_stream();
// ... 55 lines not shown
```

rxmd_amd/csrc/lists.hip:

```cpp
#include "engine.h"

#include <hipcub/hipcub.hpp>

#include <cstdlib>

namespace rxmd {

static inline int nblk(long long n, int b) { return n > 0 ? static_cast<int>((n + b - 1) / b) : 1; }


constexpr double SWEEP_PAD = 1e-6;
__device__ inline double axis_gap(const Grid &g, int a, double s, int c_self, int c2) {
  if (c2 == c_self) return 0.0;
  const double face = g.org[a] + static_cast<double>(c2 > c_self ? c2 : c2 + 1) * g.cw[a];
  const double d = (c2 > c_self ? face - s : s - face) * g.wid[a];
  return d > 0.0 ? d : 0.0;
}
__device__ inline void ref_norm(const RefMesh &m, double x, double y, double z, double (&s)[3]) {
  s[0] = (m.Hi[0] * x + m.Hi[1] * y + m.Hi[2] * z) - m.obox[0];
  s[1] = (m.Hi[3] * x + m.Hi[4] * y + m.Hi[5] * z) - m.obox[1];
  s[2] = (m.Hi[6] * x + m.Hi[7] * y + m.Hi[8] * z) - m.obox[2];
}
__device__ inline bool ref_bonded_cells_adjacent(const RefMesh &m, const double (&si)[3], const double (&sj)[3]) {
  for (int a = 0; a < 3; ++a) {
// ... 102 lines not shown
  const int j = nbr_sm[static_cast<size_t>(i) * BL_STRIDE + s];
  const int nj = nbrcnt[j];
  const int4 *lj = reinterpret_cast<const int4 *>(nbr_sm + static_cast<size_t>(j) * BL_STRIDE);
  int4 v[BL_STRIDE / 4];
#pragma unroll
  for (int q = 0; q < BL_STRIDE / 4; ++q) v[q] = (4 * q < nj) ? lj[q] : make_int4(-1, -1, -1, -1);
  int found = -1;
#pragma unroll
  for (int q = 0; q < BL_STRIDE / 4; ++q) {
    if (4 * q + 0 < nj && v[q].x == i) found = 4 * q + 0;
    if (4 * q + 1 < nj && v[q].y == i) found = 4 * q + 1;
    if (4 * q + 2 < nj && v[q].z == i) found = 4 * q + 2;
    if (4 * q + 3 < nj && v[q].w == i) found = 4 * q + 3;
  }
  if (found < 0) { atomicCAS(&err[0], DERR_NONE, DERR_NBRINDX); found = 0; }
  nbr[ob + s] = j; brev[ob + s] = boff[j] + found; bown[ob + s] = i; btype[ob + s] = static_cast<unsigned char>(type[j]);
}

__device__ inline bool pq_lookup(const DevFF &ff, const double4 *__restrict__ tab, int row, double r2, double &E, double &F) {
  if (r2 > ff.rctap2) { E = 0.0; F = 0.0; return false; }
  const int itb = static_cast<int>(r2 * ff.UDRi);
  double t = r2 - itb * ff.UDR;
  t = t * ff.UDRi;
  const double4 nd = tab[static_cast<size_t>(row) * (NTABLE + 2) + itb];
  E = nd.x + t * nd.y; F = nd.z + t * nd.w;
  return true;
}
__device__ inline double wave_sum_l(double v) { return wave_sum64(v); }

template <bool ORTHO>
__global__ void __launch_bounds__(32 * WIN_ROWS) k_win_columns(int N, Grid g, const int *__restrict__ cellid, const int *__restrict__ cellstart,
                                                               const double *__restrict__ spx, const double *__restrict__ spy, const double *__restrict__ spz, double rcp,
                                                               const int *__restrict__ rows_sorted, int *__restrict__ rowcols, int *__restrict__ grp_base,
                                                               int *__restrict__ win_k, int *__restrict__ win_cnt, int *err) {
  __shared__ int t_lo[32], t_hi[32];
  const int lane = threadIdx.x & 63, w = __builtin_amdgcn_readfirstlane(static_cast<int>(threadIdx.x >> 6));
  const int grp = xcd_swizzle(blockIdx.x, gridDim.x);
  if (grp >= err[8]) return;
  if (threadIdx.x < 32) { t_lo[threadIdx.x] = 0x7fffffff; t_hi[threadIdx.x] = -1; }
  __syncthreads();
  const int l5 = lane & 31;
  const int ridx = grp * WIN_ROWS + 2 * w + (lane >> 5);
  const int i = rows_sorted[ridx];
  if (i < N) {
    const int c = cellid[i];
    const int cy = (c / g.nzf) % g.n[1], cx = c / (g.nzf * g.n[1]);
    int k0 = 0, len = 0;
    if (l5 < 25) column_run<ORTHO>(g, cellstart, spx[i], spy[i], spz[i], cx, cy, cx + l5 / 5 - 2, cy + l5 % 5 - 2, rcp, k0, len);
    if (len > 0) { atomicMin(&t_lo[l5], k0); atomicMax(&t_hi[l5], k0 + len); }
    __builtin_nontemporal_store(k0, rowcols + static_cast<size_t>(ridx) * 64 + l5); __builtin_nontemporal_store(len, rowcols + static_cast<size_t>(ridx) * 64 + 32 + l5);
  }
  __syncthreads();
  if (w != 0) return;
  int lo8 = 0, nu = 0;
  if (lane < 25 && t_hi[lane] >= 0) { lo8 = t_lo[lane] & ~(WIN_UNIT - 1); nu = (t_hi[lane] - lo8 + WIN_UNIT - 1) / WIN_UNIT; }
  int inc = nu;
#pragma unroll
  for (int o = 1; o < 32; o <<= 1) { const int t2 = __shfl_up(inc, o, 64); if (lane >= o) inc += t2; }
  const int ub = inc - nu, nunits = __shfl(inc, 31, 64);
  if (lane < 32) grp_base[static_cast<size_t>(grp) * 32 + lane] = lo8 - WIN_UNIT * ub;
  const bool fail = nunits > WIN_MAXUNITS;
  if (lane == 0) {
    win_cnt[grp] = fail ? 0 : nunits;
    if (fail) atomicExch(&err[6], 1);
    if (__hip_atomic_load(&err[5], __ATOMIC_RELAXED, __HIP_MEMORY_SCOPE_AGENT) < nunits) atomicMax(&err[5], nunits);
  }
  if (!fail && lane < 25)
    for (int u = 0; u < nu; ++u) win_k[static_cast<size_t>(grp) * WIN_MAXUNITS + ub + u] = lo8 + WIN_UNIT * u;
}

constexpr int L10_ROWS = 8;
constexpr int L10_CAP = 1600;
template <bool SELFCHECK, bool PQ, bool ORTHO, bool F32 = false>
__global__ void __launch_bounds__(64 * L10_ROWS) k_list10(int N, int S10, Grid g, RefMesh rm, DevFF ff, const int *__restrict__ cellid, const int *__restrict__ cellstart,
                                                 const double4 *__restrict__ sorted,
                                                 const double *__restrict__ x, const double *__restrict__ y, const double *__restrict__ z,
                                                 const double *__restrict__ spx, const double *__restrict__ spy, const double *__restrict__ spz,
                                                 const int *__restrict__ type, const long long *__restrict__ gid,
                                                 int *__restrict__ nb10, double *__restrict__ hess, int *__restrict__ n10, int *err,
                                                 const double4 *__restrict__ sorted_shl, const double *__restrict__ shx, const double *__restrict__ shy, const double *__restrict__ shz,
                                                 double *__restrict__ hsc, double4 *__restrict__ pqrow,
                                                 const double2 *__restrict__ xs0, double2 *__restrict__ s_all, double2 *__restrict__ s_gh, int *__restrict__ rowflag,
                                                 const int *__restrict__ rows_sorted, unsigned short *__restrict__ sl10, const int *__restrict__ rowcols, const int *__restrict__ grp_base, int *__restrict__ gflag,
                                                 float *__restrict__ hess32 = nullptr) {
  __shared__ int s_q[L10_ROWS][128];
  __shared__ int s_K[L10_ROWS][32], s_E[L10_ROWS][32], s_L[L10_ROWS][32];
  __shared__ int s_ix2[256];
  __shared__ double s_x[L10_CAP], s_y[L10_CAP], s_z[L10_CAP];
  __shared__ int s_j[L10_CAP];
  __shared__ int t_lo[32], t_hi[32], t_off[33];
  const int lane = threadIdx.x & 63, w = __builtin_amdgcn_readfirstlane(static_cast<int>(threadIdx.x >> 6));
  for (int t = threadIdx.x; t < ff.n1 * ff.n1 && t < 256; t += blockDim.x) s_ix2[t] = ff.inxn2[t];
  if (threadIdx.x < 32) { t_lo[threadIdx.x] = 0x7fffffff; t_hi[threadIdx.x] = -1; }
  __syncthreads();
  const int ridx = xcd_swizzle(blockIdx.x, gridDim.x) * L10_ROWS + w;
  if (ridx - w >= err[8] * WIN_ROWS) return;
  const int i_raw = rows_sorted[ridx];
  const bool rowlive = i_raw < N;
  const int i = rowlive ? i_raw : 0;
  const int grp = ridx / WIN_ROWS;
  constexpr bool live = true;
  int *sq = s_q[w];
  int *cK = s_K[w], *cE = s_E[w], *cL = s_L[w];
  const double xi = x[i], yi = y[i], zi = z[i];
  const int ti = type[i];
  const size_t row = static_cast<size_t>(i) * S10;
  double sni[3] = {0.0, 0.0, 0.0};
  if (!ORTHO) ref_norm(rm, xi, yi, zi, sni);
  double sxi = 0.0, syi = 0.0, szi = 0.0, Zi = 0.0, p_f = 0.0, p_hz = 0.0, p_bz = 0.0, p_ss = 0.0;
  if (PQ) { sxi = shx[i]; syi = shy[i]; szi = shz[i]; Zi = ff.Zpq[ti]; }
  double ra = 0.0, rg = 0.0;
  bool anyghost = false;
  int cnt = 0;
  int qn = 0;
  bool staged = false;

  auto emit = [&](int nproc) {
#ifdef RXMD_EXPERIMENTS
    if (g.probe == 2) { cnt += nproc; return; }
#endif
    if (lane < nproc) {
      const int qw = sq[lane], slot = cnt + lane;
      if (slot < S10) {
        const int t_ = qw >> 20, cc_ = qw & 0xfffff;
        const int k = cK[t_] + cc_;
        double px, py, pz; int j, tj;
        if (staged) { const int li = cL[t_] + cc_; px = s_x[li]; py = s_y[li]; pz = s_z[li]; const int jw = s_j[li]; j = jw & static_cast<int>(NB10_IDX_MASK); tj = (jw >> NB10_IDX_BITS) & 31; }
        else { const double4 p = sorted[k]; const long long wv = __double_as_longlong(p.w); px = p.x; py = p.y; pz = p.z; j = static_cast<int>(wv & 0xffffffffLL); tj = static_cast<int>((wv >> 32) & 255); }
        const double d0 = xi - px, d1 = yi - py, d2 = zi - pz;
        const double r2 = d0 * d0 + d1 * d1 + d2 * d2;
        const float r2f = static_cast<float>(r2);
        double h = 0.0, hc = 0.0;
        const int inxn = s_ix2[ti * ff.n1 + tj];
        bool inq = true;
        if (!ORTHO && j >= N) {
          const double g0 = spx[j], g1 = spy[j], g2 = spz[j];
          inq = g0 > rm.qlo[0] && g0 <= rm.qhi[0] && g1 > rm.qlo[1] && g1 <= rm.qhi[1] && g2 > rm.qlo[2] && g2 <= rm.qhi[2];
        }
        if (PQ) {
          if (inq && static_cast<double>(r2f) < ff.rctap2) {
            const double C0q = 14.4;
            const double4 sj = sorted_shl[k];
            const double Zj = ff.Zpq[tj];
            const int prow = ff.inxnpq[ti * ff.npq1 + tj];
            double E, F;
            pq_lookup(ff, ff.tabPcc, prow, r2, E, F);
            h = C0q * E;
            p_hz += h * Zj;
            double e0 = d0 - sj.x, e1 = d1 - sj.y, e2 = d2 - sj.z;
            pq_lookup(ff, ff.tabPsc, prow, e0 * e0 + e1 * e1 + e2 * e2, E, F);
            p_f += h * Zj - C0q * E * Zj;
            e0 = d0 + sxi; e1 = d1 + syi; e2 = d2 + szi;
            pq_lookup(ff, ff.tabPsc, prow, e0 * e0 + e1 * e1 + e2 * e2, E, F);
            hc = C0q * E * Zi;
            p_bz += hc * Zj;
            e0 -= sj.x; e1 -= sj.y; e2 -= sj.z;
            pq_lookup(ff, ff.tabPss, prow, e0 * e0 + e1 * e1 + e2 * e2, E, F);
            p_ss += 0.5 * C0q * E * Zi * Zj;
          }
          __builtin_nontemporal_store(hc, hsc + row + slot);
        } else if (inq && static_cast<double>(r2f) < ff.rctap2 && inxn != 0) {
          const int itb = static_cast<int>(static_cast<double>(r2f) * ff.UDRi);
          double drtb = static_cast<double>(r2f) - itb * ff.UDR;
          drtb = drtb * ff.UDRi;
          const double2 T = ff.tabQEq2[static_cast<size_t>(inxn) * (NTABLE + 2) + itb];
          h = (1.0 - drtb) * T.x + drtb * T.y;
          if (F32) h = static_cast<double>(static_cast<float>(h));
        }
        {
#ifdef RXMD_EXPERIMENTS
          if (!(g.probe & 4))
#endif
          __builtin_nontemporal_store(static_cast<unsigned short>((k - cE[t_]) | (j >= N ? 0x8000 : 0)), sl10 + row + slot);
        }
        if (xs0) {
          const double qsj = xs0[k].x;
          ra += h * qsj;
          if (PQ) rg += hc * qsj; else if (j >= N) rg += h * qsj;
        }
        anyghost |= (j >= N);
#ifdef RXMD_EXPERIMENTS
        if (!(g.probe & 8))
#endif
        if (nb10) {
          unsigned ent = static_cast<unsigned>(k) | (static_cast<unsigned>(tj) << NB10_IDX_BITS) | (j >= N ? NB10_GHOST : 0u);
          if (SELFCHECK && gid[j] == gid[i]) ent |= NB10_SELF;
          __builtin_nontemporal_store(static_cast<int>(ent), nb10 + row + slot);
        }
#ifdef RXMD_EXPERIMENTS
// ... 116 lines not shown
    if (lane == 0) pqrow[i] = make_double4(p_f, p_hz, p_bz, p_ss);
  }
  const unsigned long long mg = __ballot(anyghost);
  if (lane == 0 && rowflag) rowflag[i] = (mg != 0ULL) ? 1 : 0;
  if (lane == 0) {
    n10[i] = cnt | (mg != 0ULL ? N10_GHOST_ROW : 0);
    if (__hip_atomic_load(&err[3], __ATOMIC_RELAXED, __HIP_MEMORY_SCOPE_AGENT) < cnt) atomicMax(&err[3], cnt);
    if (__hip_atomic_load(&err[4], __ATOMIC_RELAXED, __HIP_MEMORY_SCOPE_AGENT) > cnt) atomicMin(&err[4], cnt);
    if (gflag && mg != 0ULL) gflag[grp] = 1;
  }
  }
}

__global__ void k_split_rows(int N, const int *__restrict__ flag, const int *__restrict__ scan, int *__restrict__ rows_int, int *__restrict__ rows_bnd) {
  const int i = blockIdx.x * blockDim.x + threadIdx.x;
  if (i >= N) return;
  if (flag[i]) rows_bnd[scan[i]] = i; else rows_int[i - scan[i]] = i;
}

__global__ void k_resident_flags(int G, int N, const int *__restrict__ perm, int *__restrict__ flag, int *__restrict__ rows_sorted, int nrows_fill, int *__restrict__ win_cnt, int *__restrict__ win_flag, int ngroups_fill) {
  const int k = blockIdx.x * blockDim.x + threadIdx.x;
  if (k <= G) flag[k] = (k < G && perm[k] < N) ? 1 : 0;
  for (int t = k; t < nrows_fill; t += gridDim.x * blockDim.x) rows_sorted[t] = 0x7f7f7f7f;
  for (int t = k; t < ngroups_fill; t += gridDim.x * blockDim.x) { win_cnt[t] = 0; win_flag[t] = 0; }
  if (k == 0) win_flag[ngroups_fill] = 0;
}
__global__ void k_col_groups(int ncol, int nzf, const int *__restrict__ cellstart, const int *__restrict__ rank, int *__restrict__ colg) {
  const int c = blockIdx.x * blockDim.x + threadIdx.x;
  if (c > ncol) return;
  colg[c] = c < ncol ? (rank[cellstart[(c + 1) * nzf]] - rank[cellstart[c * nzf]] + WIN_ROWS - 1) / WIN_ROWS : 0;
}
__global__ void k_rows_sorted(int G, int N, int nzf, const int *__restrict__ perm, const int *__restrict__ rank, const int *__restrict__ cid_sorted, const int *__restrict__ cellstart,
                              const int *__restrict__ colgo, int *__restrict__ rows_sorted, int *__restrict__ rpos, int ncol, int *__restrict__ err) {
  const int k = blockIdx.x * blockDim.x + threadIdx.x;
  if (k == 0) err[8] = colgo[ncol];
  if (k >= G || perm[k] >= N) return;
  const int c = cid_sorted[k] / nzf;
  const int r = rank[k] - rank[cellstart[c * nzf]];
  const int place = (colgo[c] + r / WIN_ROWS) * WIN_ROWS + (r % WIN_ROWS);
  rows_sorted[place] = perm[k];
  rpos[perm[k]] = place;
}
__global__ void k_split_groups(int ng, const int *__restrict__ flag, const int *__restrict__ scan, int *__restrict__ g_int, int *__restrict__ g_bnd) {
  const int g = blockIdx.x * blockDim.x + threadIdx.x;
  if (g >= ng) return;
  if (flag[g]) g_bnd[scan[g]] = g; else g_int[g - scan[g]] = g;
}

void Engine::build_windows() {
  win_groups = static_cast<int>(win_groups_bound(N));
  k_resident_flags<<<nblk(G + 1, 256), 256, 0, stream>>>(G, N, perm, flags2, rows_sorted, win_groups * WIN_ROWS, win_cnt, win_flag, win_groups);
  size_t tb = cubtmp_bytes;
  RX_HIP(hipcub::DeviceScan::ExclusiveSum(cubtmp, tb, flags2, scanout2, G + 1, stream));
  const int ncol = grid.n[0] * grid.n[1];
  k_col_groups<<<nblk(ncol + 1, 256), 256, 0, stream>>>(ncol, grid.nzf, cellstart, scanout2, flags);
  tb = cubtmp_bytes;
  RX_HIP(hipcub::DeviceScan::ExclusiveSum(cubtmp, tb, flags, scanout, ncol + 1, stream));
  k_rows_sorted<<<nblk(G, 256), 256, 0, stream>>>(G, N, grid.nzf, perm, scanout2, cellid_sorted, cellstart, scanout, rows_sorted, rpos, ncol, d_err);
}

__global__ void k_build_prologue(int *__restrict__ err, int *__restrict__ nbrcnt_end, int what) {
  if (threadIdx.x != 0 || blockIdx.x != 0) return;
  if (what & 1) { err[2] = 0; *nbrcnt_end = 0; }
  if (what & 2) { err[3] = 0; err[4] = 0x7f7f7f7f; err[5] = 0; err[6] = 0; }
}
void Engine::build_prologue(int what) { k_build_prologue<<<1, 64, 0, stream>>>(d_err, nbrcnt + G, what); }

void Engine::build_bonded_list(bool pack_only) {
  if (!pack_only) {
  if (grid.ortho) k_bonded_list<true><<<nblk(G, 256), 256, 0, stream>>>(G, MAXNB, grid, rmesh, dff, cellid, cellstart, sorted_xyzi, pos[0], pos[1], pos[2], spos[0], spos[1], spos[2], type, nbr_sm, nbrcnt, d_err);
  else k_bonded_list<false><<<nblk(G, 256), 256, 0, stream>>>(G, MAXNB, grid, rmesh, dff, cellid, cellstart, sorted_xyzi, pos[0], pos[1], pos[2], spos[0], spos[1], spos[2], type, nbr_sm, nbrcnt, d_err);
  }
  size_t tb = cubtmp_bytes;
  RX_HIP(hipcub::DeviceScan::ExclusiveSum(cubtmp, tb, nbrcnt, boff, G + 1, stream));
  k_bond_csr<<<dim3(nblk(G, 32), (MAXNB + 7) / 8), 256, 0, stream>>>(G, N, NB, static_cast<long long>(bcap), nbr_sm, nbrcnt, boff, nbr, brev, bown, type, btype, d_err);
}

bool Engine::needs_nb10(bool selfcheck) const {
#ifdef RXMD_EXPERIMENTS
  return true;
#endif
  return nb10_sticky || opt.nb10_always || ff.pqeq || selfcheck || opt.spmv_win == 0 || opt.nonbond_win == 0 || opt.spmv_no_win || !win_valid;
}
void Engine::require_nb10() {
  if (nb10_valid) return;
  nb10_sticky = true;
  if (!lists_valid) return;
  const bool wv = win_valid, wq = sorted_w_charge;
  const int wg = win_groups;
  if (wq) sorted_positions();
  { Restore<bool> sums(sums_from_list, false), retry(list10_retry, true); build_list10(); }
  win_valid = wv; win_groups = wg;
  if (wq) sorted_charge_only();
}

constexpr int L10_ROWS_LAUNCH = L10_ROWS;
void Engine::build_list10() {
  grid.probe = static_cast<int>(opt.list_probe);
  if (list10_retry) build_prologue(2);
  const bool selfcheck = (grid.wid[0] < 2.0 * ff.rctap + 1.0) || (grid.wid[1] < 2.0 * ff.rctap + 1.0) || (grid.wid[2] < 2.0 * ff.rctap + 1.0);
  list_selfcheck = selfcheck;
  int *const nb10_w = needs_nb10(selfcheck) ? nb10 : nullptr;
  nb10_valid = nb10_w != nullptr;
#define RX_LIST10(SC, PQF) do { if (grid.ortho) RX_LIST10_O(SC, PQF, true); else RX_LIST10_O(SC, PQF, false); } while (0)
#define RX_LIST10_O(SC, PQF, OR) do { if (!PQF && f32) RX_LIST10_F(SC, false, OR, true); else RX_LIST10_F(SC, PQF, OR, false); } while (0)
#define RX_LIST10_F(SC, PQF, OR, F)                                                                                                            \
  k_list10<SC, PQF, OR, F><<<std::max(win_groups, 1) * (WIN_ROWS / L10_ROWS_LAUNCH), 64 * L10_ROWS_LAUNCH, 0, stream>>>(N, S10, grid, rmesh, dff, cellid, cellstart, sorted_xyzi, pos[0], pos[1], pos[2], spos[0], spos[1], spos[2], type, gid, \
                                                    nb10_w, hess, n10, d_err, sorted_shl, shl[0], shl[1], shl[2], hsc, pqrow, sums_from_list ? xs : nullptr, sall, sgh, multi() ? flags : nullptr, \
                                                    rows_sorted, sl10, rowcols, grp_base, gflag, F ? hess32 : nullptr)
  const bool f32 = qeq_bits_req == 32 && !ff.pqeq && hess32 != nullptr;
  win_valid = false;
  build_windows();
  int *gflag = win_flag;
  Timed kt10(this, &st.ms_k_list10);
  if (grid.ortho) k_win_columns<true><<<std::max(win_groups, 1), 32 * WIN_ROWS, 0, stream>>>(N, grid, cellid, cellstart, spos[0], spos[1], spos[2], dff.rctap_pad, rows_sorted, rowcols, grp_base, win_k, win_cnt, d_err);
  else k_win_columns<false><<<std::max(win_groups, 1), 32 * WIN_ROWS, 0, stream>>>(N, grid, cellid, cellstart, spos[0], spos[1], spos[2], dff.rctap_pad, rows_sorted, rowcols, grp_base, win_k, win_cnt, d_err);
  if (ff.pqeq) { if (selfcheck) RX_LIST10(true, true); else RX_LIST10(false, true); }
  else { if (selfcheck) RX_LIST10(true, false); else RX_LIST10(false, false); }
  kt10.end();
#undef RX_LIST10
#undef RX_LIST10_O
#undef RX_LIST10_F
  if (multi()) {
    size_t tb = cubtmp_bytes;
    RX_HIP(hipcub::DeviceScan::ExclusiveSum(cubtmp, tb, win_flag, scanout2, win_groups + 1, stream));
    k_split_groups<<<nblk(win_groups, 256), 256, 0, stream>>>(win_groups, win_flag, scanout2, win_gint, win_gbnd);
    RX_HIP(hipMemcpyAsync(&win_nbnd, scanout2 + win_groups, sizeof(int), hipMemcpyDeviceToHost, stream));
  }
  if (multi()) {
    RX_HIP(hipMemsetAsync(flags + N, 0, sizeof(int), stream));
    size_t tb = cubtmp_bytes;
    RX_HIP(hipcub::DeviceScan::ExclusiveSum(cubtmp, tb, flags, scanout, N + 1, stream));
    k_split_rows<<<nblk(N, 256), 256, 0, stream>>>(N, flags, scanout, rows_int, rows_bnd);
    RX_HIP(hipMemcpyAsync(&n_bnd, scanout + N, sizeof(int), hipMemcpyDeviceToHost, stream));
    rows_split_pending = true;
  }
}

}
```

rxmd_amd/csrc/nonbonded.hip:

```cpp
#include "engine.h"

#include <cstdlib>

namespace rxmd {

static inline int nblk(long long n, int b) { return n > 0 ? static_cast<int>((n + b - 1) / b) : 1; }
static constexpr double CEchrge = 23.02;

__global__ void k_sorted_charge(int G, const int *__restrict__ rootperm, const double *__restrict__ q, double4 *__restrict__ pk) {
  const int k = blockIdx.x * blockDim.x + threadIdx.x;
  if (k < G) pk[k].w = q[rootperm[k]];
}

__device__ inline double wave_sum_n(double v) { return wave_sum64(v); }

struct NbAcc { double f0, f1, f2, v0, v1, v2, v3, v4, v5, e11, e12; };
template <bool ENERGY>
__device__ inline void nb_pair(const DevFF &ff, const int *__restrict__ ix2, double xi, double yi, double zi, double qi, const double4 &pj, int tj, NbAcc &a) {
  const double d0 = xi - pj.x, d1 = yi - pj.y, d2 = zi - pj.z;
  const double r2 = d0 * d0 + d1 * d1 + d2 * d2;
  if (r2 > ff.rctap2) return;
  const int inxn = ix2[tj];
  const int itb = static_cast<int>(r2 * ff.UDRi);
  double t = r2 - itb * ff.UDR;
  t = t * ff.UDRi;
  const DevNBTab nd = ff.tabNB[static_cast<size_t>(inxn) * (NTABLE + 2) + itb];
  const double qij = qi * pj.w;
  const double CEvdw = nd.CEvdw + t * nd.dCEvdw_;
  const double CEclmb = (nd.CEclmb + t * nd.dCEclmb_) * qij;
  if (ENERGY) {
    a.e11 += 0.5 * (nd.Evdw + t * nd.dEvdw_);
    a.e12 += 0.5 * (nd.Eclmb + t * nd.dEclmb_) * qij;
  }
  const double c = CEvdw + CEclmb;
  a.f0 -= c * d0; a.f1 -= c * d1; a.f2 -= c * d2;
  const double hc = -0.5 * c;
  a.v0 += hc * d0 * d0; a.v1 += hc * d1 * d1; a.v2 += hc * d2 * d2; a.v3 += hc * d1 * d2; a.v4 += hc * d2 * d0; a.v5 += hc * d0 * d1;
}

#ifndef NB_UNR
#define NB_UNR 8
#endif
#ifndef NB_WPB
#define NB_WPB 8
#endif
template <bool ENERGY>
__global__ void __launch_bounds__(64 * NB_WPB) k_nonbond(int N, int S10, DevFF ff, const int *__restrict__ nb10, const int *__restrict__ n10,
                                                  const double4 *__restrict__ pk, const double *__restrict__ x, const double *__restrict__ y, const double *__restrict__ z,
                                                  const double *__restrict__ q, const int *__restrict__ type,
                                                  double *__restrict__ fx, double *__restrict__ fy, double *__restrict__ fz, double *__restrict__ pe, int assign) {
  __shared__ double sm[NB_WPB][3], sv[NB_WPB][6];
  const int lane = threadIdx.x & 63, w = __builtin_amdgcn_readfirstlane(static_cast<int>(threadIdx.x >> 6));
  if (threadIdx.x < 6 * NB_WPB) sv[threadIdx.x / 6][threadIdx.x % 6] = 0.0;
  __syncthreads();
  const int i = xcd_swizzle(blockIdx.x, gridDim.x) * (blockDim.x >> 6) + w;
  double e11 = 0.0, e12 = 0.0, e13 = 0.0;
  if (i < N) {
    const double xi = x[i], yi = y[i], zi = z[i], qi = q[i];
    const int ti = type[i];
    const int n = n10[i] & N10_COUNT;
    const size_t row = static_cast<size_t>(i) * S10;
    const int *ix2 = ff.inxn2 + ti * ff.n1;
    NbAcc acc = {0.0, 0.0, 0.0, 0.0, 0.0, 0.0, 0.0, 0.0, 0.0, 0.0, 0.0};
    for (int k0 = lane; k0 < n; k0 += 64 * NB_UNR) {
      unsigned ee[NB_UNR];
#pragma unroll
      for (int u = 0; u < NB_UNR; ++u) { const int k = k0 + 64 * u; ee[u] = (k < n) ? static_cast<unsigned>(__builtin_nontemporal_load(nb10 + row + k)) : NB10_SELF; }
#pragma unroll
      for (int u = 0; u < NB_UNR; ++u) {
        const unsigned e = ee[u];
        if (e & NB10_SELF) continue;
        nb_pair<ENERGY>(ff, ix2, xi, yi, zi, qi, pk[e & NB10_IDX_MASK], static_cast<int>((e >> NB10_IDX_BITS) & 15u), acc);
      }
    }
    e11 = acc.e11; e12 = acc.e12;
    double f0 = wave_sum_n(acc.f0), f1 = wave_sum_n(acc.f1), f2 = wave_sum_n(acc.f2);
    double v0 = acc.v0, v1 = acc.v1, v2 = acc.v2, v3 = acc.v3, v4 = acc.v4, v5 = acc.v5;
    v0 = wave_sum_n(v0); v1 = wave_sum_n(v1); v2 = wave_sum_n(v2); v3 = wave_sum_n(v3); v4 = wave_sum_n(v4); v5 = wave_sum_n(v5);
    if (lane == 0) {
      if (assign) { fx[i] = f0; fy[i] = f1; fz[i] = f2; }
      else { fx[i] += f0; fy[i] += f1; fz[i] += f2; }
      if (ENERGY) { const DevAtomP ap = ff.atom[ti]; e13 = CEchrge * (ap.chi * qi + 0.5 * ap.eta * qi * qi); }
      sv[w][0] = v0 - xi * f0; sv[w][1] = v1 - yi * f1; sv[w][2] = v2 - zi * f2; sv[w][3] = v3 - yi * f2; sv[w][4] = v4 - zi * f0; sv[w][5] = v5 - xi * f1;
    }
  }
  if (ENERGY) {
    e11 = wave_sum_n(e11); e12 = wave_sum_n(e12); e13 = wave_sum_n(e13);
    if (lane == 0) { sm[w][0] = e11; sm[w][1] = e12; sm[w][2] = e13; }
  }
  __syncthreads();
  if (ENERGY && threadIdx.x < 3) {
    double s = 0.0;
    for (int k = 0; k < NB_WPB; ++k) s += sm[k][threadIdx.x];
    if (s != 0.0) atomicAdd(pe + 11 + threadIdx.x, s);
  }
  static_assert(SCAL_ASTR == SCAL_PE + 16, "pe = scal + SCAL_PE: the stress accumulators astr are pe + 16");
  if (threadIdx.x >= 64 && threadIdx.x < 70) {
    const int c = threadIdx.x - 64;
    double s = 0.0;
    for (int k = 0; k < NB_WPB; ++k) s += sv[k][c];
    if (s != 0.0) atomicAdd(pe + 16 + c, s);
  }
}

template <bool ENERGY>
__global__ void __launch_bounds__(64 * WIN_ROWS, 8) k_nonbond_win(int N, int G, int S10, DevFF ff, const unsigned short *__restrict__ sl10, const int *__restrict__ n10,
                                                                const int *__restrict__ rows_sorted, const int *__restrict__ win_k, const int *__restrict__ win_cnt, int maxunits,
                                                                const double4 *__restrict__ pk, const unsigned char *__restrict__ stype,
                                                                const double *__restrict__ x, const double *__restrict__ y, const double *__restrict__ z,
                                                                const double *__restrict__ q, const int *__restrict__ type,
                                                                double *__restrict__ fx, double *__restrict__ fy, double *__restrict__ fz, double *__restrict__ pe, int assign) {
  extern __shared__ double4 s_p[];
  unsigned char *s_t = reinterpret_cast<unsigned char *>(s_p + static_cast<size_t>(maxunits) * WIN_UNIT);
  __shared__ double sm[WIN_ROWS][3], sv[WIN_ROWS][6];
  constexpr int NT = 64 * WIN_ROWS;
  const int lane = threadIdx.x & 63, w = __builtin_amdgcn_readfirstlane(static_cast<int>(threadIdx.x >> 6));
  const int grp = xcd_swizzle(blockIdx.x, gridDim.x);
  const int ridx = grp * WIN_ROWS + w;
  const int i = min(rows_sorted[ridx], N);
  const int nslots = WIN_UNIT * win_cnt[grp];
  const int *wk = win_k + static_cast<size_t>(grp) * WIN_MAXUNITS;
  const int capslots = WIN_UNIT * maxunits;
  for (int t = threadIdx.x; t < min(nslots, capslots); t += NT) {
    const int pos = min(wk[t / WIN_UNIT] + (t & (WIN_UNIT - 1)), G - 1);
    s_p[t] = pk[pos]; s_t[t] = stype[pos];
  }
  if (threadIdx.x < 6 * WIN_ROWS) sv[threadIdx.x / 6][threadIdx.x % 6] = 0.0;
  __syncthreads();
  double e11 = 0.0, e12 = 0.0, e13 = 0.0;
  if (i < N) {
    const double xi = x[i], yi = y[i], zi = z[i], qi = q[i];
    const int ti = type[i];
    const int n = n10[i] & N10_COUNT;
    const size_t row = static_cast<size_t>(i) * S10;
    const int *ix2 = ff.inxn2 + ti * ff.n1;
    NbAcc acc = {0.0, 0.0, 0.0, 0.0, 0.0, 0.0, 0.0, 0.0, 0.0, 0.0, 0.0};
    for (int k0 = lane; k0 < n; k0 += 64 * NB_UNR) {
      unsigned ee[NB_UNR];
#pragma unroll
      for (int u = 0; u < NB_UNR; ++u) { const int k = k0 + 64 * u; ee[u] = (k < n) ? static_cast<unsigned>(__builtin_nontemporal_load(sl10 + row + k)) : 0xffffu; }
#pragma unroll
      for (int u = 0; u < NB_UNR; ++u) {
        if (ee[u] == 0xffffu) continue;
        const int sl = static_cast<int>(ee[u] & 0x7fffu);
        if (sl < capslots) nb_pair<ENERGY>(ff, ix2, xi, yi, zi, qi, s_p[sl], static_cast<int>(s_t[sl]), acc);
        else { const int pos = min(wk[sl / WIN_UNIT] + (sl & (WIN_UNIT - 1)), G - 1); nb_pair<ENERGY>(ff, ix2, xi, yi, zi, qi, pk[pos], static_cast<int>(stype[pos]), acc); }
      }
    }
    e11 = acc.e11; e12 = acc.e12;
    const double f0 = wave_sum_n(acc.f0), f1 = wave_sum_n(acc.f1), f2 = wave_sum_n(acc.f2);
    const double v0 = wave_sum_n(acc.v0), v1 = wave_sum_n(acc.v1), v2 = wave_sum_n(acc.v2), v3 = wave_sum_n(acc.v3), v4 = wave_sum_n(acc.v4), v5 = wave_sum_n(acc.v5);
    if (lane == 0) {
      if (assign) { fx[i] = f0; fy[i] = f1; fz[i] = f2; }
      else { fx[i] += f0; fy[i] += f1; fz[i] += f2; }
      if (ENERGY) { const DevAtomP ap = ff.atom[ti]; e13 = CEchrge * (ap.chi * qi + 0.5 * ap.eta * qi * qi); }
      sv[w][0] = v0 - xi * f0; sv[w][1] = v1 - yi * f1; sv[w][2] = v2 - zi * f2; sv[w][3] = v3 - yi * f2; sv[w][4] = v4 - zi * f0; sv[w][5] = v5 - xi * f1;
    }
  }
  if (ENERGY) {
    e11 = wave_sum_n(e11); e12 = wave_sum_n(e12); e13 = wave_sum_n(e13);
    if (lane == 0) { sm[w][0] = e11; sm[w][1] = e12; sm[w][2] = e13; }
  }
  __syncthreads();
  if (ENERGY && threadIdx.x < 3) {
    double s = 0.0;
    for (int k = 0; k < WIN_ROWS; ++k) s += sm[k][threadIdx.x];
    if (s != 0.0) atomicAdd(pe + 11 + threadIdx.x, s);
  }
  static_assert(SCAL_ASTR == SCAL_PE + 16, "pe = scal + SCAL_PE: the stress accumulators astr are pe + 16");
  if (threadIdx.x >= 64 && threadIdx.x < 70) {
    const int c = threadIdx.x - 64;
    double s = 0.0;
    for (int k = 0; k < WIN_ROWS; ++k) s += sv[k][c];
    if (s != 0.0) atomicAdd(pe + 16 + c, s);
  }
}

void Engine::sorted_charge_only() { k_sorted_charge<<<nblk(G, 256), 256, 0, stream>>>(G, multi() ? perm : rootperm, q, sorted_xyzi); sorted_w_charge = true; }
void Engine::charge_halo() {
  sorted_w_charge = true;
  if (multi()) {
    halo_staged(q, 1);
    k_sorted_charge<<<nblk(G, 256), 256, 0, stream>>>(G, perm, q, sorted_xyzi);
  } else
    k_sorted_charge<<<nblk(G, 256), 256, 0, stream>>>(G, rootperm, q, sorted_xyzi);
}

void Engine::nonbonded(bool to_fnb, bool energy) {
  double *f0 = to_fnb ? fnb[0] : frc[0], *f1 = to_fnb ? fnb[1] : frc[1], *f2 = to_fnb ? fnb[2] : frc[2];
  const int assign = to_fnb ? 1 : 0;
  const bool win_env = opt.nonbond_win != 0;
  const int units = std::min(win_maxunits, 296);
  const size_t lds = static_cast<size_t>(units) * WIN_UNIT * (sizeof(double4) + 1) + 16;
  if (win_valid && win_env && !list_selfcheck) {
#define RX_NB_WIN(EN) k_nonbond_win<EN><<<win_groups, 64 * WIN_ROWS, lds, stream>>>(N, G, S10, dff, sl10, n10, rows_sorted, win_k, win_cnt, units, sorted_xyzi, sorted_type, pos[0], pos[1], pos[2], q, type, \
                                                                 f0, f1, f2, scal + SCAL_PE, assign)
    if (energy) RX_NB_WIN(true); else RX_NB_WIN(false);
#undef RX_NB_WIN
    RX_HIP(hipGetLastError());
    return;
  }
  require_nb10();
  if (energy) k_nonbond<true><<<nblk(N, NB_WPB), 64 * NB_WPB, 0, stream>>>(N, S10, dff, nb10, n10, sorted_xyzi, pos[0], pos[1], pos[2], q, type, f0, f1, f2, scal + SCAL_PE, assign);
  else k_nonbond<false><<<nblk(N, NB_WPB), 64 * NB_WPB, 0, stream>>>(N, S10, dff, nb10, n10, sorted_xyzi, pos[0], pos[1], pos[2], q, type, f0, f1, f2, scal + SCAL_PE, assign);
}

}
```

rxmd_amd/csrc/pqeq.hip:

```cpp
#include "engine.h"

namespace rxmd {

static inline int nblk(long long n, int b) { return n > 0 ? static_cast<int>((n + b - 1) / b) : 1; }
static constexpr double CEchrge = 23.02;
static constexpr double Cclmb0 = 332.0638;

__device__ inline bool pq_lookup2(const DevFF &ff, const double4 *__restrict__ tab, int row, double r2, double &E, double &F) {
  if (r2 > ff.rctap2) { E = 0.0; F = 0.0; return false; }
  const int itb = static_cast<int>(r2 * ff.UDRi);
  double t = r2 - itb * ff.UDR;
  t = t * ff.UDRi;
  const double4 nd = tab[static_cast<size_t>(row) * (NTABLE + 2) + itb];
  E = nd.x + t * nd.y; F = nd.z + t * nd.w;
  return true;
}
__device__ inline double wave_sum_p(double v) { return wave_sum64(v); }

__global__ void k_sorted_shl(int G, const int *__restrict__ perm, const double *__restrict__ sx, const double *__restrict__ sy, const double *__restrict__ sz, double4 *__restrict__ out) {
  const int k = blockIdx.x * blockDim.x + threadIdx.x;
  if (k >= G) return;
  const int i = perm[k];
  out[k] = make_double4(sx[i], sy[i], sz[i], 0.0);
}
__global__ void k_ghost_copy1(int N, int G, const int *__restrict__ groot, double *__restrict__ v) {
  const int g = N + blockIdx.x * blockDim.x + threadIdx.x;
  if (g < G) v[g] = v[groot[g]];
}

void Engine::pqeq_sorted_shells() {
  for (int a = 0; a < 3; ++a) {
    if (multi()) halo_staged(shl[a], 1);
    else if (G > N) k_ghost_copy1<<<nblk(G - N, 256), 256, 0, stream>>>(N, G, groot, shl[a]);
  }
  k_sorted_shl<<<nblk(G, 256), 256, 0, stream>>>(G, perm, shl[0], shl[1], shl[2], sorted_shl);
}

__global__ void __launch_bounds__(256) k_shell_update(int N, int S10, DevFF ff, const int *__restrict__ nb10, const int *__restrict__ n10,
                                                       const double4 *__restrict__ pk, const double4 *__restrict__ sorted_shl,
                                                       const double *__restrict__ x, const double *__restrict__ y, const double *__restrict__ z, const int *__restrict__ type,
                                                       const double *__restrict__ sx, const double *__restrict__ sy, const double *__restrict__ sz,
                                                       double *__restrict__ nx, double *__restrict__ ny, double *__restrict__ nz, int edir, double efield) {
  const int lane = threadIdx.x & 63;
  const int i = xcd_swizzle(blockIdx.x, gridDim.x) * (blockDim.x >> 6) + __builtin_amdgcn_readfirstlane(static_cast<int>(threadIdx.x >> 6));
  if (i >= N) return;
  const int ti = type[i];
  const double s0 = sx[i], s1 = sy[i], s2 = sz[i];
  const double hx = x[i] + s0, hy = y[i] + s1, hz = z[i] + s2;
  const double Zi = ff.Zpq[ti], Ki = ff.Kspq[ti];
  const int n = n10[i] & N10_COUNT;
  const size_t row = static_cast<size_t>(i) * S10;
  double f0 = 0.0, f1 = 0.0, f2 = 0.0;
  constexpr int SU = 8;
  for (int k0 = lane; k0 < n; k0 += 64 * SU) {
    unsigned ee[SU];
#pragma unroll
    for (int u = 0; u < SU; ++u) { const int k = k0 + 64 * u; ee[u] = (k < n) ? static_cast<unsigned>(__builtin_nontemporal_load(nb10 + row + k)) : 0xffffffffu; }
#pragma unroll
    for (int u = 0; u < SU; ++u) {
    const unsigned e = ee[u];
    if (e == 0xffffffffu) continue;
    const int p = e & NB10_IDX_MASK, tj = (e >> NB10_IDX_BITS) & 15u;
    const double4 pj = pk[p], sj = sorted_shl[p];
    const int prow = ff.inxnpq[ti * ff.npq1 + tj];
    const double Zj = ff.Zpq[tj], qjc = pj.w + Zj;
    double d0 = hx - pj.x, d1 = hy - pj.y, d2 = hz - pj.z, E, F;
    pq_lookup2(ff, ff.tabPsc, prow, d0 * d0 + d1 * d1 + d2 * d2, E, F);
    double c = Cclmb0 * F * qjc * Zi;
    f0 += c * d0; f1 += c * d1; f2 += c * d2;
    d0 -= sj.x; d1 -= sj.y; d2 -= sj.z;
    pq_lookup2(ff, ff.tabPss, prow, d0 * d0 + d1 * d1 + d2 * d2, E, F);
    c = Cclmb0 * F * Zi * Zj;
    f0 -= c * d0; f1 -= c * d1; f2 -= c * d2;
    }
  }
  f0 = wave_sum_p(f0); f1 = wave_sum_p(f1); f2 = wave_sum_p(f2);
  if (lane == 0) {
    f0 -= Ki * s0; f1 -= Ki * s1; f2 -= Ki * s2;
    if (edir == 1) f0 -= Zi * efield; else if (edir == 2) f1 -= Zi * efield; else if (edir == 3) f2 -= Zi * efield;
    double r0 = f0 / Ki, r1 = f1 / Ki, r2 = f2 / Ki;
    const double ddr = sqrt(r0 * r0 + r1 * r1 + r2 * r2);
    if (ddr > 1e-3) { r0 = r0 / ddr * 1e-3; r1 = r1 / ddr * 1e-3; r2 = r2 / ddr * 1e-3; }
    nx[i] = s0 + r0; ny[i] = s1 + r1; nz[i] = s2 + r2;
  }
}

__global__ void k_sorted_charge_p(int G, const int *__restrict__ rootperm, const double *__restrict__ q, double4 *__restrict__ pk) {
  const int k = blockIdx.x * blockDim.x + threadIdx.x;
  if (k < G) pk[k].w = q[rootperm[k]];
}

void Engine::pqeq_update_shells() {
  sorted_w_charge = true;
  if (multi()) { halo_staged(q, 1); k_sorted_charge_p<<<nblk(G, 256), 256, 0, stream>>>(G, perm, q, sorted_xyzi); }
  else k_sorted_charge_p<<<nblk(G, 256), 256, 0, stream>>>(G, rootperm, q, sorted_xyzi);
  require_nb10();
  k_shell_update<<<nblk(N, 4), 256, 0, stream>>>(N, S10, dff, nb10, n10, sorted_xyzi, sorted_shl, pos[0], pos[1], pos[2], type, shl[0], shl[1], shl[2], cds, cd, cc_,
                                                cfg.efield_dir, cfg.efield_strength * 23.060538);
  double *tmp[3] = {cds, cd, cc_};
  for (int a = 0; a < 3; ++a) RX_HIP(hipMemcpyAsync(shl[a], tmp[a], sizeof(double) * N, hipMemcpyDeviceToDevice, stream));
  pqeq_sorted_shells();
  pq_matrix_stale = true;
}

__global__ void __launch_bounds__(256) k_nonbond_pqeq(int N, int S10, DevFF ff, const int *__restrict__ nb10, const int *__restrict__ n10,
                                                       const double4 *__restrict__ pk, const double4 *__restrict__ sorted_shl,
                                                       const double *__restrict__ x, const double *__restrict__ y, const double *__restrict__ z,
                                                       const double *__restrict__ q, const int *__restrict__ type,
                                                       const double *__restrict__ sx, const double *__restrict__ sy, const double *__restrict__ sz,
                                                       double *__restrict__ fx, double *__restrict__ fy, double *__restrict__ fz, double *__restrict__ pe) {
  __shared__ double sm[4][3], sv[4][6];
  const int lane = threadIdx.x & 63, w = __builtin_amdgcn_readfirstlane(static_cast<int>(threadIdx.x >> 6));
  if (threadIdx.x < 24) sv[threadIdx.x / 6][threadIdx.x % 6] = 0.0;
  __syncthreads();
  const int i = xcd_swizzle(blockIdx.x, gridDim.x) * (blockDim.x >> 6) + w;
  double e11 = 0.0, e12 = 0.0, e13 = 0.0;
  if (i < N) {
    const double xi = x[i], yi = y[i], zi = z[i], qi = q[i];
    const double s0 = sx[i], s1 = sy[i], s2 = sz[i];
    const int ti = type[i];
    const double Zi = ff.Zpq[ti], qic = qi + Zi;
    const int n = n10[i] & N10_COUNT;
    const size_t row = static_cast<size_t>(i) * S10;
    const int *ix2 = ff.inxn2 + ti * ff.n1;
    double f0 = 0.0, f1 = 0.0, f2 = 0.0;
    double v0 = 0.0, v1 = 0.0, v2 = 0.0, v3 = 0.0, v4 = 0.0, v5 = 0.0;
    constexpr int PU = 4;
    for (int k0 = lane; k0 < n; k0 += 64 * PU) {
      unsigned ee[PU];
#pragma unroll
      for (int u = 0; u < PU; ++u) { const int k = k0 + 64 * u; ee[u] = (k < n) ? static_cast<unsigned>(__builtin_nontemporal_load(nb10 + row + k)) : NB10_SELF; }
#pragma unroll
      for (int u = 0; u < PU; ++u) {
      const unsigned e = ee[u];
      if (e & NB10_SELF) continue;
      const int p = e & NB10_IDX_MASK, tj = (e >> NB10_IDX_BITS) & 15u;
      const double4 pj = pk[p], sj = sorted_shl[p];
      const double d0 = xi - pj.x, d1 = yi - pj.y, d2 = zi - pj.z;
      const double r2 = d0 * d0 + d1 * d1 + d2 * d2;
      if (r2 > ff.rctap2) continue;
      const int inxn = ix2[tj];
      const int itb = static_cast<int>(r2 * ff.UDRi);
      double t = r2 - itb * ff.UDR;
      t = t * ff.UDRi;
      const DevNBTab nd = ff.tabNB[static_cast<size_t>(inxn) * (NTABLE + 2) + itb];
      e11 += 0.5 * (nd.Evdw + t * nd.dEvdw_);
      const double CEvdw = nd.CEvdw + t * nd.dCEvdw_;
      const double Zj = ff.Zpq[tj], qjc = pj.w + Zj;
      const int prow = ff.inxnpq[ti * ff.npq1 + tj];
      double E, F, a0, a1, a2, c;
      double g0 = CEvdw * d0, g1 = CEvdw * d1, g2 = CEvdw * d2, ec;
      pq_lookup2(ff, ff.tabPcc, prow, r2, E, F);
      c = Cclmb0 * qic * qjc; ec = c * E; g0 += c * F * d0; g1 += c * F * d1; g2 += c * F * d2;
      a0 = d0 + s0; a1 = d1 + s1; a2 = d2 + s2;
      pq_lookup2(ff, ff.tabPsc, prow, a0 * a0 + a1 * a1 + a2 * a2, E, F);
      c = -Cclmb0 * Zi * qjc; ec += c * E; g0 += c * F * a0; g1 += c * F * a1; g2 += c * F * a2;
      a0 = d0 - sj.x; a1 = d1 - sj.y; a2 = d2 - sj.z;
      pq_lookup2(ff, ff.tabPsc, prow, a0 * a0 + a1 * a1 + a2 * a2, E, F);
      c = -Cclmb0 * Zj * qic; ec += c * E; g0 += c * F * a0; g1 += c * F * a1; g2 += c * F * a2;
      a0 += s0; a1 += s1; a2 += s2;
      pq_lookup2(ff, ff.tabPss, prow, a0 * a0 + a1 * a1 + a2 * a2, E, F);
      c = Cclmb0 * Zi * Zj; ec += c * E; g0 += c * F * a0; g1 += c * F * a1; g2 += c * F * a2;
      e12 += 0.5 * ec;
      f0 -= g0; f1 -= g1; f2 -= g2;
      v0 -= 0.5 * d0 * g0; v1 -= 0.5 * d1 * g1; v2 -= 0.5 * d2 * g2; v3 -= 0.5 * d1 * g2; v4 -= 0.5 * d2 * g0; v5 -= 0.5 * d0 * g1;
      }
    }
    f0 = wave_sum_p(f0); f1 = wave_sum_p(f1); f2 = wave_sum_p(f2);
    v0 = wave_sum_p(v0); v1 = wave_sum_p(v1); v2 = wave_sum_p(v2); v3 = wave_sum_p(v3); v4 = wave_sum_p(v4); v5 = wave_sum_p(v5);
    if (lane == 0) {
      sv[w][0] = v0 - xi * f0; sv[w][1] = v1 - yi * f1; sv[w][2] = v2 - zi * f2; sv[w][3] = v3 - yi * f2; sv[w][4] = v4 - zi * f0; sv[w][5] = v5 - xi * f1;
      fx[i] += f0; fy[i] += f1; fz[i] += f2;
      const DevAtomP ap = ff.atom[ti];
      e13 = CEchrge * (ap.chi * qi + 0.5 * ap.eta * qi * qi) + 0.5 * ff.Kspq[ti] * (s0 * s0 + s1 * s1 + s2 * s2);
    }
  }
  e11 = wave_sum_p(e11); e12 = wave_sum_p(e12); e13 = wave_sum_p(e13);
  if (lane == 0) { sm[w][0] = e11; sm[w][1] = e12; sm[w][2] = e13; }
  __syncthreads();
  if (threadIdx.x < 3) {
    double s = 0.0;
    for (int k = 0; k < 4; ++k) s += sm[k][threadIdx.x];
    if (s != 0.0) atomicAdd(pe + 11 + threadIdx.x, s);
  }
  static_assert(SCAL_ASTR == SCAL_PE + 16, "pe = scal + SCAL_PE: the stress accumulators astr are pe + 16");
  if (threadIdx.x >= 64 && threadIdx.x < 70) {
    const int c = threadIdx.x - 64;
    const double s = sv[0][c] + sv[1][c] + sv[2][c] + sv[3][c];
    if (s != 0.0) atomicAdd(pe + 16 + c, s);
  }
}

__global__ void k_efield(int N, DevFF ff, const int *__restrict__ type, const double *__restrict__ q, double ev, double *__restrict__ f) {
  const int i = blockIdx.x * blockDim.x + threadIdx.x;
  if (i < N) f[i] += -(q[i] + ff.Zpq[type[i]]) * ev;
}
void Engine::efield_force() {
  if (cfg.efield_dir < 1 || cfg.efield_dir > 3) return;
  k_efield<<<nblk(N, 256), 256, 0, stream>>>(N, dff, type, q, cfg.efield_strength * 23.060538, frc[cfg.efield_dir - 1]);
}

void Engine::nonbonded_pqeq() {
  require_nb10();
  k_nonbond_pqeq<<<nblk(N, 4), 256, 0, stream>>>(N, S10, dff, nb10, n10, sorted_xyzi, sorted_shl, pos[0], pos[1], pos[2], q, type, shl[0], shl[1], shl[2],
                                                frc[0], frc[1], frc[2], scal + SCAL_PE);
}

}
```

rxmd_amd/csrc/qeq.hip:

```cpp
#include "spmv_kernels.h"

#include <chrono>
#include <map>
#include <mutex>
#include <tuple>
#include <cstdio>

#include <cmath>
#include <memory>
#include <utility>
#include <vector>

namespace rxmd {

__global__ void __launch_bounds__(256) k_stream_probe(size_t n16, const f64x2 *__restrict__ a, double *__restrict__ out) {
  double s = 0.0;
  for (size_t i = static_cast<size_t>(blockIdx.x) * blockDim.x + threadIdx.x; i < n16; i += static_cast<size_t>(gridDim.x) * blockDim.x) {
    const f64x2 v = __builtin_nontemporal_load(a + i);
    s += v.x + v.y;
  }
  if (s == 12345.678) out[0] = s;
}
double stream_probe_ms(Engine &e, int blocks) {
  const size_t n16 = static_cast<size_t>(e.rows10) * e.S10 / 2;
// ... 202 lines not shown
  r_type[r] = type[a]; r_n10[r] = n10[a]; r_xpos[r] = invpos[a]; rpos[a] = r;
}
__global__ void k_ghost_rows(int N, int G, const int *__restrict__ groot, const int *__restrict__ rpos, int *__restrict__ g_rrow) {
  const int t = N + blockIdx.x * blockDim.x + threadIdx.x;
  if (t < G) g_rrow[t] = rpos[groot[t]];
}
__global__ void k_rows_exit(int R, int N, const int *__restrict__ rows, const double *__restrict__ scal, const double2 *__restrict__ r_qst, double2 *__restrict__ qst, double *__restrict__ q) {
  const int r = blockIdx.x * blockDim.x + threadIdx.x;
  if (r >= R) return;
  const int a = rows[r];
  if (a >= N || a < 0) return;
  const double2 v = r_qst[r];
  qst[a] = v;
  q[a] = v.x - scal[S_MU] * v.y;
}

__global__ void k_apply_q(int N, const double *__restrict__ scal, const double2 *__restrict__ qst, double *__restrict__ q) {
  const int i = blockIdx.x * blockDim.x + threadIdx.x;
  if (i >= N) return;
  const double2 v = qst[i];
  q[i] = v.x - scal[S_MU] * v.y;
}
__global__ void k_direction(int N, int first, const double *__restrict__ scal, const double2 *__restrict__ gst, double2 *__restrict__ hst) {
  const int i = blockIdx.x * blockDim.x + threadIdx.x;
  if (i >= N) return;
  const double2 g = gst[i];
  if (first) { hst[i] = g; return; }
  const double2 h = hst[i];
  hst[i] = make_double2(g.x + scal[S_BETA_S] * h.x, g.y + scal[S_BETA_T] * h.y);
}
__global__ void k_qeq_init(int N, int isQEq, double fqs, double *__restrict__ q, double *__restrict__ qsfp, double *__restrict__ qsfv, double2 *__restrict__ qst, double2 *__restrict__ hst) {
  const int i = blockIdx.x * blockDim.x + threadIdx.x;
  if (i >= N) return;
  hst[i] = make_double2(0.0, 0.0);
  if (isQEq == 1) { qsfp[i] = q[i]; qsfv[i] = 0.0; qst[i] = make_double2(q[i], 0.0); }
  else { qst[i] = make_double2(fqs * qsfp[i] + (1.0 - fqs) * q[i], 0.0); }
}

__global__ void __launch_bounds__(256) k_grad_start(int N, DevFF ff, const int *__restrict__ type, const double2 *__restrict__ qst, const double *__restrict__ q,
                                                     const double2 *__restrict__ sall, const double2 *__restrict__ sgh, double2 *__restrict__ gst,
                                                     double *__restrict__ partials, const double4 *__restrict__ pqrow) {
  double g1s = 0.0, g2s = 0.0, es = 0.0;
  for (int i = blockIdx.x * blockDim.x + threadIdx.x; i < N; i += gridDim.x * blockDim.x) {
    const int ti = type[i];
    const DevAtomP ap = ff.atom[ti];
    const double2 qv = qst[i], a = sall[i], g = sgh[i];
    const double g1 = -ap.chi - ap.eta * qv.x - a.x - (pqrow ? pqrow[i].x : 0.0), g2 = -1.0 - ap.eta * qv.y - a.y;
    gst[i] = make_double2(g1, g2);
    const double qi = q[i];
    g1s += g1 * g1; g2s += g2 * g2;
    if (pqrow) es += pq_est_row(ap, ff.Zpq[ti], pqrow[i], qi, a.x, g.x);
    else es += ap.chi * qi + 0.5 * ap.eta * qi * qi + 0.5 * qi * (a.x + (a.x - g.x));
  }
  double acc[4] = {wave_sum(g1s), wave_sum(g2s), wave_sum(es), 0.0};
  block_store_partials<4>(acc, partials, 4);
}

__global__ void k_sorted_part(int G, int N, const int *__restrict__ perm, const double2 *__restrict__ v, double2 *__restrict__ xs, int ghosts) {
  const int k = blockIdx.x * blockDim.x + threadIdx.x;
  if (k >= G) return;
  const int i = perm[k];
  if ((i >= N) == (ghosts != 0)) xs[k] = v[i];
}

void Engine::qeq_start_vectors() {
  k_qeq_init<<<nblk(N, 256), 256, 0, stream>>>(N, cfg.isQEq, cfg.Lex_fqs, q, qsfp, qsfv, qst, hst);
  sorted_copy(qst);
}

void Engine::allreduce_scal4(int n) {
  if (nprocs == 1 && !nccl) return;
  allreduce_device(scal + S_RAW0, n, H_SCAL_REDUCE, 0);
}

Engine::WinInstance Engine::win_instance() const {
  if (qeq_bits_req == 32 && !ff.pqeq && hess32 != nullptr && (S10 & 3) == 0) return {2, WIN_PREFETCH | WIN_LEAN, true};
  if (ff.pqeq) return opt.pq_prefetch != 0 ? WinInstance{1, WIN_PREFETCH, false} : WinInstance{2, WIN_PREFETCH | WIN_LEAN, false};
  const bool one_trip = opt.spmv_one_trip != 0 && max_row10 > 256 && max_row10 <= 384;
  return one_trip ? WinInstance{3, WIN_LEAN, false} : WinInstance{2, WIN_PREFETCH | WIN_LEAN, false};
}
WinPassArgs Engine::win_args(bool roword) const {
  WinPassArgs a{N, G, S10, dff, sl10, hess, hess32, n10, rows_sorted, win_k, win_cnt, xs, hst, gst, qst, q, type, scal, partials, wall, wgh, hsc, pqrow,
                nullptr, win_groups, 0, nullptr, win_flag, 0, win_maxunits, stream};
  if (roword) { a.n10 = r_n10; a.type = r_type; a.hst = r_hst; a.gst = r_gst; a.rs_all = r_wall; a.rs_gh = r_wgh; a.roword = 1; }
  return a;
}
RowPassArgs Engine::row_args() const {
  return RowPassArgs{N, S10, dff, nb10, hess, n10, xs, hst, gst, qst, q, type, scal, partials, wall, wgh, hsc, pqrow, opt.no_xcd_swizzle ? 0 : 1 ,
                     nullptr, N, 0, nullptr, stream};
}
template <class F> static void with_mode_store(int mode, bool store, F &&f) {
  using std::integral_constant;
  if (mode == MODE_HSH) { if (store) f(integral_constant<int, MODE_HSH>{}, std::true_type{}); else f(integral_constant<int, MODE_HSH>{}, std::false_type{}); }
  else { if (store) f(integral_constant<int, MODE_GRAD>{}, std::true_type{}); else f(integral_constant<int, MODE_GRAD>{}, std::false_type{}); }
}
static void launch_win_instance(int mode, bool store, bool pq, Engine::WinInstance wi, const WinPassArgs &a) {
  constexpr int DEF = WIN_PREFETCH | WIN_LEAN;
  with_mode_store(mode, store, [&](auto m, auto s) {
    constexpr int M = decltype(m)::value; constexpr bool S = decltype(s)::value;
    if (!pq && wi.f32 && wi.nstep == 2 && wi.var == DEF) launch_win<M, S, false, 2, DEF, float>(a);
    else if (!pq && !wi.f32 && wi.nstep == 2 && wi.var == DEF) launch_win<M, S, false, 2, DEF>(a);
    else if (!pq && !wi.f32 && wi.nstep == 3 && wi.var == WIN_LEAN) launch_win<M, S, false, 3, WIN_LEAN>(a);
    else if (pq && !wi.f32 && wi.nstep == 1 && wi.var == WIN_PREFETCH) launch_win<M, S, true, 1, WIN_PREFETCH>(a);
    else if (pq && !wi.f32 && wi.nstep == 2 && wi.var == DEF) launch_win<M, S, true, 2, DEF>(a);
    else throw EngineError(RXMD_E_STATE, "no window-pass instance <pq " + std::to_string(pq) + ", nstep " + std::to_string(wi.nstep) + ", var " + std::to_string(wi.var) + (wi.f32 ? ", float>" : ", double>"));
  });
}
int Engine::matrix_pass(const PassCall &c) {
  win_used = false;
  if (win_valid && opt.spmv_win != 0 && (!c.rowlist || c.rowlist == rows_int || c.rowlist == rows_bnd)) {
    win_used = true;
    WinPassArgs a = win_args(c.roword);
    a.grouplist = !c.rowlist ? nullptr : (c.rowlist == rows_int ? win_gint : win_gbnd);
    a.ngroups = !c.rowlist ? win_groups : (c.rowlist == rows_int ? win_groups - win_nbnd : win_nbnd);
    if (a.ngroups == 0) return 0;
    a.rs_all = c.ra; a.rs_gh = c.rg; a.pbase = c.pbase; a.stopflag = c.stopflag;
    const WinInstance wi = win_instance();
    st.spmv_nstep = wi.nstep; st.spmv_var = wi.var; qeq_bits_used = wi.f32 ? 32 : 64;
    launch_win_instance(c.mode, c.store, ff.pqeq != 0, wi, a);
    return a.ngroups;
  }
  RowPassArgs a = row_args();
  a.rs_all = c.ra; a.rs_gh = c.rg; a.rowlist = c.rowlist; a.nrows = c.nrows; a.pbase = c.pbase; a.stopflag = c.stopflag;
  st.spmv_nstep = 0; st.spmv_var = 0;
  qeq_bits_used = 64;
  require_nb10();
  const bool pq = ff.pqeq != 0, pipe = !opt.spmv_no_pipe;
  with_mode_store(c.mode, c.store, [&](auto m, auto s) {
    constexpr int M = decltype(m)::value; constexpr bool S = decltype(s)::value;
    if (pq) { if (pipe) launch_row<M, S, true, 1>(a); else launch_row<M, S, true, 0>(a); }
    else { if (pipe) launch_row<M, S, false, 1>(a); else launch_row<M, S, false, 0>(a); }
  });
  return a.nblocks();
}
void Engine::cg_reduce(int stage, int nsets, const double *stopflag) {
  double *lvl1 = partials + partials_cap;
  const int fused_stage = multi() ? 0 : stage;
  k_reduce_fused<<<nsets > 1024 ? 128 : 1, 256, 0, stream>>>(nsets, partials, lvl1, tickets, fused_stage, scal, stopflag);
  if (!multi()) return;
  allreduce_scal4();
  k_scalar_algebra<<<1, 64, 0, stream>>>(stage, scal);
}

void Engine::tune_window_placement() {
  if (qeq_bits_req == 32) return;
  place_tuned = true;
  const int tries = static_cast<int>(opt.place_tries);
  if (tries <= 1 || !win_valid || N < 65536) return;
  const size_t ne = static_cast<size_t>(rows10) * S10;
  auto room_for_candidate = [&] { size_t fr = 0, tot = 0; if (hipMemGetInfo(&fr, &tot) == hipSuccess && fr >= 2 * ne * (ff.pqeq ? 18 : 10)) return true; (void)hipGetLastError(); return false; };
  if (!room_for_candidate()) return;
  struct Cand {
    double *h = nullptr, *c = nullptr; unsigned short *s = nullptr;
    ~Cand() { if (h) (void)hipFree(h); if (s) (void)hipFree(s); if (c) (void)hipFree(c); }
  };
  auto time_pass = [&](const double *h, const unsigned short *sl, const double *hc) {
    WinPassArgs a = win_args(rows_live);
    a.hess = h; a.sl10 = sl; a.hsc = hc;
    const WinInstance wi = win_instance();
    return timed_launches_ms(*this, 5, 30, [&] { launch_win_instance(MODE_HSH, true, ff.pqeq != 0, wi, a); });
  };
#ifdef RXMD_EXPERIMENTS
  if (opt.place_scan > 0) {
    if (!ff.pqeq) {
      const int nslab = std::max(1, static_cast<int>(opt.place_scan));
      const size_t MB2 = size_t(2) << 20, hb = ne * sizeof(double), sb = ne * sizeof(unsigned short);
      const size_t pad = size_t(64) << 20, total = hb + sb + 3 * pad;
      const size_t offs[] = {0, 4096, 8192, 16384, 32768, 65536, 131072, 262144, 524288, size_t(1) << 20, (size_t(1) << 20) + 4096, size_t(2) << 20, size_t(4) << 20, size_t(8) << 20, size_t(16) << 20, size_t(32) << 20};
      std::fprintf(stderr, "[place_scan] engine's own placement: %.4f ms  hess %p sl10 %p  (ne %zu)\n", time_pass(hess, sl10, hsc), static_cast<void *>(hess), static_cast<void *>(sl10), ne);
      std::vector<char *> held;
      for (int sidx = 0; sidx < nslab; ++sidx) {
        char *slab = nullptr;
        if (hipMalloc(reinterpret_cast<void **>(&slab), total) != hipSuccess) { (void)hipGetLastError(); break; }
        held.push_back(slab);
        auto at = [&](size_t oh, size_t os) {
          double *h2 = reinterpret_cast<double *>(slab + oh);
          unsigned short *s2 = reinterpret_cast<unsigned short *>(slab + ((pad + hb + MB2 - 1) / MB2) * MB2 + os);
          RX_HIP(hipMemcpyAsync(h2, hess, hb, hipMemcpyDeviceToDevice, stream));
          RX_HIP(hipMemcpyAsync(s2, sl10, sb, hipMemcpyDeviceToDevice, stream));
          const double t = time_pass(h2, s2, hsc);
          std::fprintf(stderr, "[place_scan] slab %d %p  oh %9zu  os %9zu  %.4f ms\n", sidx, static_cast<void *>(slab), oh, os, t);
        };
        for (size_t os : offs) at(0, os);
        for (size_t oh : offs) if (oh) at(oh, 0);
        at(0, 0);
      }
      auto seq_ms = [&](const void *ptr) { return timed_launches_ms(*this, 0, 5, [&] { k_stream_probe<<<num_cu * 8, 256, 0, stream>>>(hb / 16, reinterpret_cast<const f64x2 *>(ptr), partials); }); };
      auto on_slab = [&](const char *how, char *slab) {
        double *h2 = reinterpret_cast<double *>(slab);
        unsigned short *s2 = reinterpret_cast<unsigned short *>(slab + ((pad + hb + MB2 - 1) / MB2) * MB2);
        RX_HIP(hipMemcpyAsync(h2, hess, hb, hipMemcpyDeviceToDevice, stream));
        RX_HIP(hipMemcpyAsync(s2, sl10, sb, hipMemcpyDeviceToDevice, stream));
        const double t = time_pass(h2, s2, hsc), t_hv = time_pass(h2, sl10, hsc), t_sv = time_pass(hess, s2, hsc);
        std::fprintf(stderr, "[place_scan] %-28s %p  pass %.4f ms (its values + engine slots %.4f, engine values + its slots %.4f)  sequential read of its value stream %.4f ms = %.0f GB/s\n", how, static_cast<void *>(slab), t, t_hv, t_sv, seq_ms(h2), hb / (seq_ms(h2) * 1e-3) / 1e9);
      };
      std::fprintf(stderr, "[place_scan] engine's own value stream: sequential read %.4f ms\n", seq_ms(hess));
      for (char *p : held) on_slab("hipMalloc slab (above)", p);
      for (int c = 0; c < 3; ++c) {
        char *slab = nullptr;
        if (hipExtMallocWithFlags(reinterpret_cast<void **>(&slab), total, hipDeviceMallocContiguous) != hipSuccess) { (void)hipGetLastError(); std::fprintf(stderr, "[place_scan] contiguous allocation refused\n"); break; }
        on_slab("hipDeviceMallocContiguous", slab);
        held.push_back(slab);
      }
      for (size_t chunk : {size_t(2) << 20, size_t(64) << 20, size_t(1) << 30}) {
        for (int rep = 0; rep < 2; ++rep) {
// ... 290 lines not shown
```

rxmd_amd/csrc/spmv_kernels.h:

```cpp
#pragma once
#include "engine.h"

#include <type_traits>

namespace rxmd {

static inline int nblk(long long n, int b) { return n > 0 ? static_cast<int>((n + b - 1) / b) : 1; }

enum { MODE_HSH = 0, MODE_GRAD = 1 };
typedef double f64x2 __attribute__((ext_vector_type(2)));
#ifndef SPMV_UNR
#define SPMV_UNR 4
#endif
constexpr int UNR = SPMV_UNR;
__device__ inline double wave_sum(double v) { return wave_sum64(v); }

template <int NC>
__device__ inline void block_store_partials(double (&acc)[NC], double *partials, int ncomp_stride) {
  __shared__ double sm[16][NC];
  const int w = threadIdx.x >> 6, lane = threadIdx.x & 63, nw = blockDim.x >> 6;
  if (lane == 0)
    for (int c = 0; c < NC; ++c) sm[w][c] = acc[c];
  __syncthreads();
  if (threadIdx.x < NC) {
    double s = 0.0;
    for (int k = 0; k < nw; ++k) s += sm[k][threadIdx.x];
    __hip_atomic_store(partials + static_cast<size_t>(blockIdx.x) * ncomp_stride + threadIdx.x, s, __ATOMIC_RELAXED, __HIP_MEMORY_SCOPE_AGENT);
  }
}

__device__ inline double pq_est_row(const DevAtomP &ap, double Zi, const double4 &pr, double qi, double hq, double bq) {
  return ap.chi * qi + 0.5 * ap.eta * qi * qi + 0.5 * (qi + Zi) * (hq + pr.y) + pr.w - (bq + pr.z);
}
template <int MODE, bool STORE, bool PQ, int PIPE>
__global__ void __launch_bounds__(1024) k_spmv(int N, int S10, DevFF ff, const int *__restrict__ nb10, const double *__restrict__ hess, const int *__restrict__ n10,
                                               const double2 *__restrict__ xv, const double2 *__restrict__ hst, double2 *__restrict__ gst,
                                               const double2 *__restrict__ qst, const double *__restrict__ q, const int *__restrict__ type,
                                               const double *__restrict__ scal, double *__restrict__ partials,
                                               double2 *__restrict__ rs_all, double2 *__restrict__ rs_gh,
                                               const double *__restrict__ hsc, const double4 *__restrict__ pqrow, int swz,
                                               const int *__restrict__ rowlist, int nrows, int pbase, const double *__restrict__ stopflag) {
  if (stopflag && *stopflag != 0.0) return;
  const int lane = threadIdx.x & 63;
  const int wpb = blockDim.x >> 6;
  const int widx = (swz ? xcd_swizzle(blockIdx.x, gridDim.x) : static_cast<int>(blockIdx.x)) * wpb + __builtin_amdgcn_readfirstlane(static_cast<int>(threadIdx.x >> 6));
  const int row = rowlist ? (widx < nrows ? rowlist[widx] : N) : widx;
  __shared__ double s_row[16][4];
  const int wave_in_wg = __builtin_amdgcn_readfirstlane(static_cast<int>(threadIdx.x >> 6));
  if (row < N) {
    const size_t base = static_cast<size_t>(row) * S10;
    unsigned e[UNR];
    double h[UNR], c[UNR];
    auto request = [&](int kb, int bound, unsigned (&ee)[UNR], double (&hh)[UNR], double (&cc)[UNR]) {
#pragma unroll
      for (int u = 0; u < UNR; ++u) {
        const int k = kb + lane + 64 * u;
        const bool ok = k < bound;
        ee[u] = ok ? static_cast<unsigned>(__builtin_nontemporal_load(nb10 + base + k)) : 0u;
        hh[u] = ok ? __builtin_nontemporal_load(hess + base + k) : 0.0;
        if (PQ && (MODE == MODE_GRAD || STORE)) cc[u] = ok ? __builtin_nontemporal_load(hsc + base + k) : 0.0;
      }
    };
    if (PIPE) request(0, S10, e, h, c);
    const int n = n10[row] & N10_COUNT;
    double as = 0.0, at = 0.0, gs_ = 0.0, gt_ = 0.0;
    if (PIPE) {
#pragma unroll
      for (int u = 0; u < UNR; ++u) { const bool ok = lane + 64 * u < n; e[u] = ok ? e[u] : 0u; h[u] = ok ? h[u] : 0.0; if (PQ) c[u] = ok ? c[u] : 0.0; }
    }
    for (int kb = 0; kb < n; kb += 64 * UNR) {
      if (PIPE == 0 || (PIPE == 1 && kb > 0)) request(kb, n, e, h, c);
#pragma unroll
      for (int u = 0; u < UNR; ++u) {
        const double2 v = xv[e[u] & NB10_IDX_MASK];
        as += h[u] * v.x;
        at += h[u] * v.y;
        if ((MODE == MODE_GRAD || STORE) && !PQ) { const double hg = (e[u] & NB10_GHOST) ? h[u] : 0.0; gs_ += hg * v.x; gt_ += hg * v.y; }
        if ((MODE == MODE_GRAD || STORE) && PQ) { gs_ += c[u] * v.x; gt_ += c[u] * v.y; }
      }
    }
    as = wave_sum(as); at = wave_sum(at);
    if (MODE == MODE_GRAD || STORE) { gs_ = wave_sum(gs_); gt_ = wave_sum(gt_); }
    if (lane == 0) { s_row[wave_in_wg][0] = as; s_row[wave_in_wg][1] = at; s_row[wave_in_wg][2] = gs_; s_row[wave_in_wg][3] = gt_; }
  }
  __syncthreads();
  if (wave_in_wg != 0) return;
  {
    const int r_idx = (swz ? xcd_swizzle(blockIdx.x, gridDim.x) : static_cast<int>(blockIdx.x)) * wpb + lane;
    const int r = (lane < wpb) ? (rowlist ? (r_idx < nrows ? rowlist[r_idx] : N) : r_idx) : N;
    double a0 = 0.0, a1 = 0.0, a2 = 0.0, a3 = 0.0;
    if (r < N) {
      const double as = s_row[lane][0], at = s_row[lane][1], gs_ = s_row[lane][2], gt_ = s_row[lane][3];
      const int t = type[r];
      const double2 pa = (MODE == MODE_HSH) ? hst[r] : qst[r];
      const DevAtomP ap = ff.atom[t];
      if (STORE) { rs_all[r] = make_double2(as, at); rs_gh[r] = make_double2(gs_, gt_); }
      if (MODE == MODE_HSH) {
        const double2 pb = gst[r];
        const double ts = ap.eta * pa.x + as, tt = ap.eta * pa.y + at;
        a0 = ts * pa.x; a1 = tt * pa.y;
        a2 = pb.x * pa.x; a3 = pb.y * pa.y;
      } else {
        const double mu = scal[S_MU];
        const double fpq = PQ ? pqrow[r].x : 0.0;
        const double g1 = -ap.chi - ap.eta * pa.x - as - fpq;
        const double g2 = -1.0 - ap.eta * pa.y - at;
        gst[r] = make_double2(g1, g2);
        a0 = g1 * g1; a1 = g2 * g2;
        const double qi = q[r];
        const double hq_all = as - mu * at, hq_res = (as - gs_) - mu * (at - gt_);
        if (PQ) a2 = pq_est_row(ap, ff.Zpq[t], pqrow[r], qi, hq_all, gs_ - mu * gt_);
        else a2 = ap.chi * qi + 0.5 * ap.eta * qi * qi + 0.5 * qi * (hq_all + hq_res);
      }
    }
    a0 = wave_sum(a0); a1 = wave_sum(a1); a2 = wave_sum(a2); a3 = wave_sum(a3);
    if (lane < 4) {
      const double v = lane == 0 ? a0 : (lane == 1 ? a1 : (lane == 2 ? a2 : a3));
      __hip_atomic_store(partials + (static_cast<size_t>(pbase) + blockIdx.x) * 4 + lane, v, __ATOMIC_RELAXED, __HIP_MEMORY_SCOPE_AGENT);
    }
  }
}

[[maybe_unused]] constexpr int WIN_RANKROWS = 1;
constexpr int WIN_PREFETCH = 2, WIN_LEAN = 4;
template <class VT> struct WinVal;
template <> struct WinVal<double> { typedef double2 pair; static __device__ inline pair make(double a, double b) { return make_double2(a, b); } };
template <> struct WinVal<float> { typedef float2 pair; static __device__ inline pair make(float a, float b) { return make_float2(a, b); } };
template <int MODE, bool STORE, bool PQ, int NSTEP = 2, int VAR = 0, class VT = double>
__global__ void __launch_bounds__(64 * WIN_ROWS, 8) k_spmv_win(int N, int G, int S10, DevFF ff, const unsigned short *__restrict__ sl10, const VT *__restrict__ hess, const int *__restrict__ n10,
                                                            const int *__restrict__ rows_sorted, const int *__restrict__ win_k, const int *__restrict__ win_cnt,
                                                            const double2 *__restrict__ xv, const double2 *__restrict__ hst, double2 *__restrict__ gst,
                                                            const double2 *__restrict__ qst, const double *__restrict__ q, const int *__restrict__ type,
                                                            const double *__restrict__ scal, double *__restrict__ partials,
                                                            double2 *__restrict__ rs_all, double2 *__restrict__ rs_gh,
                                                            const double *__restrict__ hsc, const double4 *__restrict__ pqrow,
                                                            const int *__restrict__ grouplist, int ngroups, int pbase, const double *__restrict__ stopflag,
                                                            const int *__restrict__ gflags = nullptr, int roword = 0) {
  if (stopflag && *stopflag != 0.0) return;
  extern __shared__ double2 s_x[];
  __shared__ double s_row[WIN_ROWS][4];
  __shared__ int s_arrived;
  constexpr int STEPS = NSTEP;
  constexpr int NT = 64 * WIN_ROWS;
  typedef double d2v __attribute__((ext_vector_type(2)));
  typedef VT h2v __attribute__((ext_vector_type(2)));
  typedef typename WinVal<VT>::pair hpair;
  static_assert(std::is_same<VT, double>::value || (!PQ && NSTEP == 2), "the float value stream: plain QEq, two batches per register set");
  const int lane = threadIdx.x & 63;
  const int wave = __builtin_amdgcn_readfirstlane(static_cast<int>(threadIdx.x >> 6));
  const int gidx = xcd_swizzle(blockIdx.x, gridDim.x);
  const int grp = grouplist ? (gidx < ngroups ? grouplist[gidx] : -1) : (gidx < ngroups ? gidx : -1);
  if (grp < 0) return;
  const int ridx = grp * WIN_ROWS + wave;
  const int row = min(rows_sorted[ridx], N);
  const int nslots = WIN_UNIT * win_cnt[grp];
  const int *wk = win_k + static_cast<size_t>(grp) * WIN_MAXUNITS;
  const int t0 = threadIdx.x, t1 = threadIdx.x + NT;
  const int wk0 = wk[t0 / WIN_UNIT], wk1 = wk[t1 / WIN_UNIT];
  const bool live = row < N;
#ifdef RXMD_EXPERIMENTS
  const size_t base = static_cast<size_t>(live ? ((VAR & WIN_RANKROWS) ? ridx : row) : 0) * S10;
#else
  const size_t base = static_cast<size_t>(live ? row : 0) * S10;
#endif
  const h2v *hv2 = reinterpret_cast<const h2v *>(hess + base);
  const d2v *cv2 = reinterpret_cast<const d2v *>(PQ ? hsc + base : nullptr);
  const unsigned *sl2 = reinterpret_cast<const unsigned *>(sl10 + base);
  const bool gh = !((VAR & WIN_LEAN) != 0 && !PQ && gflags != nullptr) || gflags[grp] != 0;
  auto whole = [&](auto ghc) {
  constexpr bool GHC = decltype(ghc)::value;
  hpair v[STEPS]; double2 c[STEPS]; unsigned ss[STEPS];
  auto request = [&](int kb, int bound) {
#pragma unroll
    for (int u = 0; u < STEPS; ++u) {
      const int k = kb + 128 * u + 2 * lane;
      const bool ok = k < bound;
      if (ok) { const h2v t2 = __builtin_nontemporal_load(hv2 + (k >> 1)); v[u] = WinVal<VT>::make(t2.x, t2.y); } else v[u] = WinVal<VT>::make(0.0, 0.0);
      ss[u] = ok ? __builtin_nontemporal_load(sl2 + (k >> 1)) : 0u;
      if (PQ && (MODE == MODE_GRAD || STORE)) { if (ok) { const d2v t2 = __builtin_nontemporal_load(cv2 + (k >> 1)); c[u] = make_double2(t2.x, t2.y); } else c[u] = make_double2(0.0, 0.0); }
    }
  };
  double2 x0 = make_double2(0.0, 0.0), x1 = x0;
  if (t0 < nslots) x0 = xv[min(wk0 + (t0 & (WIN_UNIT - 1)), G - 1)];
  if (t1 < nslots) x1 = xv[min(wk1 + (t1 & (WIN_UNIT - 1)), G - 1)];
  request(0, live ? S10 : 0);
  const int rowc = live ? (roword ? ridx : row) : 0;
  const int n = live ? (n10[rowc] & N10_COUNT) : 0;
  const int tl_t = type[rowc];
  const double2 tl_a = (MODE == MODE_HSH) ? hst[rowc] : qst[rowc];
  const double2 tl_b = (MODE == MODE_HSH) ? const_cast<const double2 *>(gst)[rowc] : make_double2(q[rowc], 0.0);
  if (threadIdx.x == 0) s_arrived = 0;
  if (t0 < nslots) s_x[t0] = x0;
  if (t1 < nslots) s_x[t1] = x1;
  for (int t = threadIdx.x + 2 * NT; t < nslots; t += NT) s_x[t] = xv[min(wk[t / WIN_UNIT] + (t & (WIN_UNIT - 1)), G - 1)];
#pragma unroll
  for (int u = 0; u < STEPS; ++u) {
    const int k = 128 * u + 2 * lane;
    if (k >= n) { v[u].x = static_cast<VT>(0.0); ss[u] &= 0xffff0000u; if (PQ) c[u].x = 0.0; }
    if (k + 1 >= n) { v[u].y = static_cast<VT>(0.0); ss[u] &= 0x0000ffffu; if (PQ) c[u].y = 0.0; }
  }
  constexpr bool PRE = (VAR & WIN_PREFETCH) != 0 && (!PQ || NSTEP == 1);
  hpair vn[STEPS]; double2 cn[STEPS]; unsigned sn[STEPS];
  auto request_next = [&](int kb) {
#pragma unroll
    for (int u = 0; u < STEPS; ++u) {
      const int k = kb + 128 * u + 2 * lane;
      const bool ok = k < n;
      if (ok) { const h2v t2 = __builtin_nontemporal_load(hv2 + (k >> 1)); vn[u] = WinVal<VT>::make(t2.x, t2.y); } else vn[u] = WinVal<VT>::make(0.0, 0.0);
      sn[u] = ok ? __builtin_nontemporal_load(sl2 + (k >> 1)) : 0u;
      if (PQ && (MODE == MODE_GRAD || STORE)) { if (ok) { const d2v t2 = __builtin_nontemporal_load(cv2 + (k >> 1)); cn[u] = make_double2(t2.x, t2.y); } else cn[u] = make_double2(0.0, 0.0); }
    }
  };
  if (PRE && n > 128 * STEPS) request_next(128 * STEPS);
  __syncthreads();
  double as = 0.0, at = 0.0, gs_ = 0.0, gt_ = 0.0;
    auto batch = [&](const hpair (&vv)[STEPS], const unsigned (&sv)[STEPS], const double2 (&cv)[STEPS]) {
#pragma unroll
      for (int u = 0; u < STEPS; ++u) {
        const double2 y0 = s_x[sv[u] & 0x7fffu], y1 = s_x[(sv[u] >> 16) & 0x7fffu];
        const double hx = vv[u].x, hy = vv[u].y;
        as += hx * y0.x; at += hx * y0.y; as += hy * y1.x; at += hy * y1.y;
        if (GHC && (MODE == MODE_GRAD || STORE) && !PQ) {
          const double g0 = (sv[u] & 0x8000u) ? hx : 0.0, g1 = (sv[u] & 0x80000000u) ? hy : 0.0;
          gs_ += g0 * y0.x; gt_ += g0 * y0.y; gs_ += g1 * y1.x; gt_ += g1 * y1.y;
        }
        if ((MODE == MODE_GRAD || STORE) && PQ) { gs_ += cv[u].x * y0.x; gt_ += cv[u].x * y0.y; gs_ += cv[u].y * y1.x; gt_ += cv[u].y * y1.y; }
      }
    };
    constexpr int B = 128 * STEPS;
    if (PRE) {
      for (int kb = 0;;) {
        batch(v, ss, c);
        kb += B; if (kb >= n) break;
        if (kb + B < n) request(kb + B, n);
        batch(vn, sn, cn);
        kb += B; if (kb >= n) break;
        if (kb + B < n) request_next(kb + B);
      }
    } else {
      for (int kb = 0; kb < n; kb += B) {
        if (kb > 0) request(kb, n);
        batch(v, ss, c);
      }
    }

  as = wave_sum(as); at = wave_sum(at);
  if ((MODE == MODE_GRAD || STORE) && GHC) { gs_ = wave_sum(gs_); gt_ = wave_sum(gt_); }
  const int lane_t = static_cast<int>(__builtin_amdgcn_mbcnt_hi(~0u, __builtin_amdgcn_mbcnt_lo(~0u, 0u)));
  double a0 = 0.0, a1 = 0.0, a2 = 0.0, a3 = 0.0;
  if (live) {
    const DevAtomP ap = ff.atom[tl_t];
    if (MODE == MODE_HSH) {
      const double ts = ap.eta * tl_a.x + as, tt = ap.eta * tl_a.y + at;
      a0 = ts * tl_a.x; a1 = tt * tl_a.y;
      a2 = tl_b.x * tl_a.x; a3 = tl_b.y * tl_a.y;
      if (STORE && lane_t == 0) { rs_all[rowc] = make_double2(as, at); rs_gh[rowc] = make_double2(gs_, gt_); }
    } else {
      const double mu = scal[S_MU];
      const double4 pr = PQ ? pqrow[row] : make_double4(0.0, 0.0, 0.0, 0.0);
      const double g1 = -ap.chi - ap.eta * tl_a.x - as - pr.x;
      const double g2 = -1.0 - ap.eta * tl_a.y - at;
      a0 = g1 * g1; a1 = g2 * g2;
      const double qi = tl_b.x;
      const double hq_all = as - mu * at, hq_res = (as - gs_) - mu * (at - gt_);
      if (PQ) a2 = pq_est_row(ap, ff.Zpq[tl_t], pr, qi, hq_all, gs_ - mu * gt_);
      else a2 = ap.chi * qi + 0.5 * ap.eta * qi * qi + 0.5 * qi * (hq_all + hq_res);
      if (lane_t == 0) { gst[rowc] = make_double2(g1, g2); if (STORE) { rs_all[rowc] = make_double2(as, at); rs_gh[rowc] = make_double2(gs_, gt_); } }
    }
  }
  int arrived = 0;
  if (lane_t == 0) {
    s_row[wave][0] = a0; s_row[wave][1] = a1; s_row[wave][2] = a2; s_row[wave][3] = a3;
    __builtin_amdgcn_fence(__ATOMIC_RELEASE, "workgroup");
    arrived = __hip_atomic_fetch_add(&s_arrived, 1, __ATOMIC_RELAXED, __HIP_MEMORY_SCOPE_WORKGROUP);
  }
  arrived = __builtin_amdgcn_readfirstlane(arrived);
  if (arrived != WIN_ROWS - 1) return;
  __builtin_amdgcn_fence(__ATOMIC_ACQUIRE, "workgroup");
  if (lane_t < 4) {
    double sum = 0.0;
#pragma unroll
    for (int w = 0; w < WIN_ROWS; ++w) sum += s_row[w][lane_t];
    __hip_atomic_store(partials + (static_cast<size_t>(pbase) + blockIdx.x) * 4 + lane_t, sum, __ATOMIC_RELAXED, __HIP_MEMORY_SCOPE_AGENT);
  }
  };
  if (gh) whole(std::true_type{}); else whole(std::false_type{});
}

struct WinPassArgs {
  int N, G, S10; DevFF ff; const unsigned short *sl10; const double *hess; const float *hess32; const int *n10, *rows_sorted, *win_k, *win_cnt;
  const double2 *xv, *hst; double2 *gst; const double2 *qst; const double *q; const int *type; const double *scal; double *partials; double2 *rs_all, *rs_gh; const double *hsc; const double4 *pqrow;
  const int *grouplist; int ngroups, pbase; const double *stopflag; const int *gflags; int roword;
  int win_maxunits; hipStream_t stream;
};
template <int MODE, bool STORE, bool PQ, int NSTEP = 2, int VAR = 0, class VT = double>
inline void launch_win(const WinPassArgs &a) {
  const VT *values = [&] { if constexpr (std::is_same<VT, float>::value) return a.hess32; else return a.hess; }();
  k_spmv_win<MODE, STORE, PQ, NSTEP, VAR, VT><<<a.ngroups, 64 * WIN_ROWS, static_cast<size_t>(a.win_maxunits) * WIN_UNIT * sizeof(double2), a.stream>>>(
      a.N, a.G, a.S10, a.ff, a.sl10, values, a.n10, a.rows_sorted, a.win_k, a.win_cnt, a.xv, a.hst, a.gst, a.qst, a.q, a.type, a.scal, a.partials, a.rs_all, a.rs_gh, a.hsc, a.pqrow,
      a.grouplist, a.ngroups, a.pbase, a.stopflag, a.gflags, a.roword);
}
constexpr int SPMV_WPB = 16;
struct RowPassArgs {
  int N, S10; DevFF ff; const int *nb10; const double *hess; const int *n10;
  const double2 *xv, *hst; double2 *gst; const double2 *qst; const double *q; const int *type; const double *scal; double *partials;
  double2 *rs_all, *rs_gh; const double *hsc; const double4 *pqrow; int swz; const int *rowlist; int nrows, pbase; const double *stopflag;
  hipStream_t stream;
  int nblocks() const { return nblk(rowlist ? nrows : N, SPMV_WPB); }
};
template <int MODE, bool STORE, bool PQ, int PIPE>
inline void launch_row(const RowPassArgs &a) {
  k_spmv<MODE, STORE, PQ, PIPE><<<a.nblocks(), 64 * SPMV_WPB, 0, a.stream>>>(a.N, a.S10, a.ff, a.nb10, a.hess, a.n10, a.xv, a.hst, a.gst, a.qst, a.q, a.type, a.scal, a.partials, a.rs_all, a.rs_gh, a.hsc, a.pqrow, a.swz,
                                                                            a.rowlist, a.nrows, a.pbase, a.stopflag);
}

template <class F> inline double timed_launches_ms(Engine &e, int warm, int reps, F &&launch) {
  for (int r = 0; r < warm + reps; ++r) { if (r == warm) hipEventRecord(e.ev[2], e.stream); launch(); }
  hipEventRecord(e.ev[3], e.stream); hipEventSynchronize(e.ev[3]);
  float ms = 0; hipEventElapsedTime(&ms, e.ev[2], e.ev[3]);
  return static_cast<double>(ms) / reps;
}

}
```

Before: 24.05.

## Store per-row neighbor streams by window placement order instead of atom index

When the row stride is large enough and the window groups fit in the list capacity, the Hessian, slot and neighbor rows are written at the row's sorted window position (ridx) rather than at the atom index. All consumers (SpMV window and row kernels, nonbond, hydrogen-bond sweep, debug readers) are updated to index by placement. The window SpMV gains a BP specialization that issues the first batch of row loads before the scalar metadata loads, which become explicit s_load instructions. This is meant to make the streams contiguous per window group and hide load latency, at the cost of an extra rpos indirection on the per-atom paths and hand-written inline assembly.

```diff
diff --git a/include/rxmd_hip.h b/include/rxmd_hip.h
--- a/include/rxmd_hip.h
+++ b/include/rxmd_hip.h
@@ -104,7 +104,8 @@
   long long halo_calls, allreduce_calls;
   double ms_k_list10, ms_k_nonbond, ms_k_e3b, ms_k_e4b, ms_k_ehb, ms_k_bondorder, ms_k_assemble;
   double ms_k_winbuild;
-  int win_groups, win_max_units, win_in_use, reserved2;
+  int win_groups, win_max_units, win_in_use;
+  int streams_by_place;
   double place_ms_first, place_ms_kept;
   double place_total_ms, place_bytes_held;
   int place_draws;
diff --git a/rxmd_amd/_lib.py b/rxmd_amd/_lib.py
--- a/rxmd_amd/_lib.py
+++ b/rxmd_amd/_lib.py
@@ -24,7 +24,7 @@
                 ("ms_allreduce", C.c_double), ("ms_fold", C.c_double), ("halo_calls", C.c_longlong), ("allreduce_calls", C.c_longlong),
                 ("ms_k_list10", C.c_double), ("ms_k_nonbond", C.c_double), ("ms_k_e3b", C.c_double), ("ms_k_e4b", C.c_double), ("ms_k_ehb", C.c_double),
                 ("ms_k_bondorder", C.c_double), ("ms_k_assemble", C.c_double), ("ms_k_winbuild", C.c_double),
-                ("win_groups", C.c_int), ("win_max_units", C.c_int), ("win_in_use", C.c_int), ("reserved2", C.c_int),
+                ("win_groups", C.c_int), ("win_max_units", C.c_int), ("win_in_use", C.c_int), ("streams_by_place", C.c_int),
                 ("place_ms_first", C.c_double), ("place_ms_kept", C.c_double),
                 ("place_total_ms", C.c_double), ("place_bytes_held", C.c_double), ("place_draws", C.c_int),
                 ("spmv_nstep", C.c_int), ("spmv_var", C.c_int), ("reserved3", C.c_int), ("ms_k_blist", C.c_double),
@@ -35,7 +35,7 @@
         for name, _ in self._fields_:
             v = getattr(self, name)
             d[name] = list(v) if hasattr(v, "__len__") else v
-        d.pop("reserved"); d.pop("reserved2"); d.pop("reserved3")
+        d.pop("reserved"); d.pop("reserved3")
         return d
 
 
diff --git a/rxmd_amd/csrc/bonded.hip b/rxmd_amd/csrc/bonded.hip
--- a/rxmd_amd/csrc/bonded.hip
+++ b/rxmd_amd/csrc/bonded.hip
@@ -1000,7 +1000,7 @@
                                                     double *__restrict__ cf1, double *__restrict__ fnx, double *__restrict__ fny, double *__restrict__ fnz,
                                                     double *__restrict__ fx, double *__restrict__ fy, double *__restrict__ fz, double *__restrict__ pe,
                                                     double *__restrict__ fsx, double *__restrict__ fsy, double *__restrict__ fsz,
-                                                    const unsigned short *__restrict__ sl10, const int *__restrict__ rpos, const int *__restrict__ win_k, const unsigned char *__restrict__ stype, int G
+                                                    const unsigned short *__restrict__ sl10, const int *__restrict__ rpos, const int *__restrict__ win_k, const unsigned char *__restrict__ stype, int G, int byplace
 #ifdef RXMD_EHB_DEBUG
                                                     , int *dbg, int lim_n, int lim_b, int lim_nb
 #endif
@@ -1033,7 +1033,7 @@
     EHB_CHECK(2, ob, lim_b - 32, i)
     EHB_CHECK(3, n, S10 + 1, i)
     const double xi = x[i], yi = y[i], zi = z[i];
-    const size_t row = static_cast<size_t>(i) * S10;
+    const size_t row = static_cast<size_t>(byplace ? rpos[i] : i) * S10;
     const int *wk = SLOTS ? win_k + static_cast<size_t>(rpos[i] / WIN_ROWS) * WIN_MAXUNITS : nullptr;
     const int inx_l = (lane >= 1 && lane <= ff.nso && lane < 16) ? ff.inxn3hb[(ti * ff.n1 + 2) * ff.n1 + lane] : 0;
     if (lane < 16) { const DevHbP hp = ff.hb[inx_l]; s_hp[w][lane][0] = hp.r0hb; s_hp[w][lane][1] = hp.phb1; s_hp[w][lane][2] = hp.phb2; s_hp[w][lane][3] = hp.phb3; }
@@ -1252,7 +1252,7 @@
     const int ehb_grid = num_cu * (slots ? ehb_blocks_per_cu_sl : ehb_blocks_per_cu);
 #ifdef RXMD_EHB_DEBUG
     RX_HIP(hipMemsetAsync(ehb_cnt + EHB_REGIONS, 0, 4 * sizeof(int), stream));
-#define RX_EHB(SL) k_ehb_sweep<SL><<<ehb_grid, 256, 0, stream>>>(S10, dff, ehb_don, ehb_cnt, region_cap, boff, nbr, type, pos[0], pos[1], pos[2], bo0, nb10, n10, sorted_xyzi, perm, cf1, fnx, fny, fnz, frc[0], frc[1], frc[2], pe_d, fsort[0], fsort[1], fsort[2], sl10, rpos, win_k, sorted_type, G, ehb_cnt + EHB_REGIONS, N, static_cast<int>(bcap), NB)
+#define RX_EHB(SL) k_ehb_sweep<SL><<<ehb_grid, 256, 0, stream>>>(S10, dff, ehb_don, ehb_cnt, region_cap, boff, nbr, type, pos[0], pos[1], pos[2], bo0, nb10, n10, sorted_xyzi, perm, cf1, fnx, fny, fnz, frc[0], frc[1], frc[2], pe_d, fsort[0], fsort[1], fsort[2], sl10, rpos, win_k, sorted_type, G, streams_by_place ? 1 : 0, ehb_cnt + EHB_REGIONS, N, static_cast<int>(bcap), NB)
     if (slots) RX_EHB(true); else RX_EHB(false);
 #undef RX_EHB
     { int hd[EHB_REGIONS + 4]; RX_HIP(hipMemcpyAsync(hd, ehb_cnt, sizeof(hd), hipMemcpyDeviceToHost, stream)); RX_HIP(hipStreamSynchronize(stream));
@@ -1260,7 +1260,7 @@
       hd[4] = hd[EHB_REGIONS]; hd[5] = hd[EHB_REGIONS + 1]; hd[6] = hd[EHB_REGIONS + 2]; hd[7] = hd[EHB_REGIONS + 3];
       std::fprintf(stderr, "[ehb debug] donors %d  blocks/CU %d  first violation: code %d value %d aux %d lim %d   (N %d bcap %zu NB %d S10 %d rows10 %d)\n", hd[0], ehb_blocks_per_cu, hd[4], hd[5], hd[6], hd[7], N, bcap, NB, S10, rows10); }
 #else
-#define RX_EHB(SL) k_ehb_sweep<SL><<<ehb_grid, 256, 0, stream>>>(S10, dff, ehb_don, ehb_cnt, region_cap, boff, nbr, type, pos[0], pos[1], pos[2], bo0, nb10, n10, sorted_xyzi, perm, cf1, fnx, fny, fnz, frc[0], frc[1], frc[2], pe_d, fsort[0], fsort[1], fsort[2], sl10, rpos, win_k, sorted_type, G)
+#define RX_EHB(SL) k_ehb_sweep<SL><<<ehb_grid, 256, 0, stream>>>(S10, dff, ehb_don, ehb_cnt, region_cap, boff, nbr, type, pos[0], pos[1], pos[2], bo0, nb10, n10, sorted_xyzi, perm, cf1, fnx, fny, fnz, frc[0], frc[1], frc[2], pe_d, fsort[0], fsort[1], fsort[2], sl10, rpos, win_k, sorted_type, G, streams_by_place ? 1 : 0)
     if (slots) RX_EHB(true); else RX_EHB(false);
 #undef RX_EHB
 #endif
diff --git a/rxmd_amd/csrc/capi.hip b/rxmd_amd/csrc/capi.hip
--- a/rxmd_amd/csrc/capi.hip
+++ b/rxmd_amd/csrc/capi.hip
@@ -425,7 +425,7 @@
     }
     e.st.natoms = e.N;
     e.st.n_boundary_rows = (e.multi() && e.lists_valid && !e.rows_split_pending_invalid()) ? e.n_bnd : 0;
-    e.st.win_groups = e.win_groups; e.st.win_max_units = e.win_maxunits; e.st.win_in_use = e.win_used ? 1 : 0;
+    e.st.win_groups = e.win_groups; e.st.win_max_units = e.win_maxunits; e.st.win_in_use = e.win_used ? 1 : 0; e.st.streams_by_place = (e.lists_valid && e.streams_by_place) ? 1 : 0;
     e.st.spmv_launches_timed = e.pass_timed_n;
     e.st.ms_qeq_spmv = e.pass_timed_n > 0 ? e.pass_timed_ms / static_cast<double>(e.pass_timed_n) * static_cast<double>(e.st.spmv_launches) : 0.0;
     *out = e.st;
@@ -498,8 +498,10 @@
         std::vector<int> c(N); RX_HIP(hipMemcpy(c.data(), e.n10, sizeof(int) * N, hipMemcpyDeviceToHost));
         for (int &v : c) v &= rxmd::N10_COUNT;
         std::vector<double> row(e.S10);
+        std::vector<int> place(e.streams_by_place ? N : 0);
+        if (e.streams_by_place && N > 0) RX_HIP(hipMemcpy(place.data(), e.rpos, sizeof(int) * N, hipMemcpyDeviceToHost));
         for (int i = 0; i < N; ++i) {
-          RX_HIP(hipMemcpy(row.data(), e.hess + static_cast<size_t>(i) * e.S10, sizeof(double) * c[i], hipMemcpyDeviceToHost));
+          RX_HIP(hipMemcpy(row.data(), e.hess + static_cast<size_t>(e.streams_by_place ? place[i] : i) * e.S10, sizeof(double) * c[i], hipMemcpyDeviceToHost));
           double s = 0; for (int k = 0; k < c[i]; ++k) s += row[k];
           out[i] = s;
         }
@@ -537,8 +539,9 @@
           const int i = rs[r], g = static_cast<int>(r / rxmd::WIN_ROWS);
           if (i < 0 || i >= N) continue;
           const int cnt = c[i] & rxmd::N10_COUNT;
-          RX_HIP(hipMemcpy(ent.data(), e.nb10 + static_cast<size_t>(i) * e.S10, sizeof(int) * cnt, hipMemcpyDeviceToHost));
-          RX_HIP(hipMemcpy(sl.data(), e.sl10 + static_cast<size_t>(i) * e.S10, sizeof(unsigned short) * cnt, hipMemcpyDeviceToHost));
+          const size_t srow = e.streams_by_place ? r : static_cast<size_t>(i);
+          RX_HIP(hipMemcpy(ent.data(), e.nb10 + srow * e.S10, sizeof(int) * cnt, hipMemcpyDeviceToHost));
+          RX_HIP(hipMemcpy(sl.data(), e.sl10 + srow * e.S10, sizeof(unsigned short) * cnt, hipMemcpyDeviceToHost));
           int good = 0;
           for (int k = 0; k < cnt; ++k) {
             const unsigned en = static_cast<unsigned>(ent[k]);
diff --git a/rxmd_amd/csrc/engine.h b/rxmd_amd/csrc/engine.h
--- a/rxmd_amd/csrc/engine.h
+++ b/rxmd_amd/csrc/engine.h
@@ -134,6 +134,7 @@
 #endif
 constexpr int WIN_ROWS = WIN_ROWS_DEF;
 constexpr int WIN_UNIT = 8;
+constexpr int WIN_BP_MIN_STRIDE = 384;
 constexpr int WIN_MAXUNITS = 448;
 constexpr int WIN_BMW = 2048;
 
@@ -390,6 +391,9 @@
   static size_t win_groups_bound_for(const Grid &g, long long n) { return static_cast<size_t>(n) / WIN_ROWS + static_cast<size_t>(g.n[0]) * g.n[1] + 1; }
   double qeq_iters_smooth = -1.0;
   bool win_valid = false, win_used = false;
+  bool streams_by_place = false;
+  int stream_place_cap() const;
+  const int *stream_rpos() const { return streams_by_place ? rpos : nullptr; }
   void halo_refresh(double2 *v2, double *v1);
   void halo_staged(double *v, int ncomp);
   struct Round { int d0, n; };
diff --git a/rxmd_amd/csrc/engine.hip b/rxmd_amd/csrc/engine.hip
--- a/rxmd_amd/csrc/engine.hip
+++ b/rxmd_amd/csrc/engine.hip
@@ -593,6 +593,7 @@
   win_groups = h_err[8];
   max_row10 = h_err[3]; min_row10 = std::min(h_err[4], h_err[3]);
   win_maxunits = h_err[5]; win_valid = win_groups > 0 && h_err[6] == 0 && win_maxunits > 0 && (!multi() || (win_nbnd >= 0 && win_nbnd <= win_groups)) && !opt.spmv_no_win;
+  { const int cap = stream_place_cap(); streams_by_place = cap > 0 && S10 >= WIN_BP_MIN_STRIDE && h_err[6] == 0 && static_cast<long long>(win_groups) * WIN_ROWS <= cap; }
   lists_valid = true;
   if (!nb10_valid && !win_valid) require_nb10();
   collect_timers();
diff --git a/rxmd_amd/csrc/lists.hip b/rxmd_amd/csrc/lists.hip
--- a/rxmd_amd/csrc/lists.hip
+++ b/rxmd_amd/csrc/lists.hip
@@ -208,7 +208,7 @@
                                                  double *__restrict__ hsc, double4 *__restrict__ pqrow,
                                                  const double2 *__restrict__ xs0, double2 *__restrict__ s_all, double2 *__restrict__ s_gh, int *__restrict__ rowflag,
                                                  const int *__restrict__ rows_sorted, unsigned short *__restrict__ sl10, const int *__restrict__ rowcols, const int *__restrict__ grp_base, int *__restrict__ gflag,
-                                                 float *__restrict__ hess32 = nullptr) {
+                                                 float *__restrict__ hess32 = nullptr, int place_cap = 0) {
   __shared__ int s_q[L10_ROWS][128];
   __shared__ int s_K[L10_ROWS][32], s_E[L10_ROWS][32], s_L[L10_ROWS][32];
   __shared__ int s_ix2[256];
@@ -220,7 +220,9 @@
   if (threadIdx.x < 32) { t_lo[threadIdx.x] = 0x7fffffff; t_hi[threadIdx.x] = -1; }
   __syncthreads();
   const int ridx = xcd_swizzle(blockIdx.x, gridDim.x) * L10_ROWS + w;
-  if (ridx - w >= err[8] * WIN_ROWS) return;
+  const int ngroups = err[8];
+  if (ridx - w >= ngroups * WIN_ROWS) return;
+  const bool byplace = place_cap > 0 && S10 >= WIN_BP_MIN_STRIDE && err[6] == 0 && ngroups * WIN_ROWS <= place_cap;
   const int i_raw = rows_sorted[ridx];
   const bool rowlive = i_raw < N;
   const int i = rowlive ? i_raw : 0;
@@ -230,7 +232,7 @@
   int *cK = s_K[w], *cE = s_E[w], *cL = s_L[w];
   const double xi = x[i], yi = y[i], zi = z[i];
   const int ti = type[i];
-  const size_t row = static_cast<size_t>(i) * S10;
+  const size_t row = static_cast<size_t>(byplace ? ridx : i) * S10;
   double sni[3] = {0.0, 0.0, 0.0};
   if (!ORTHO) ref_norm(rm, xi, yi, zi, sni);
   double sxi = 0.0, syi = 0.0, szi = 0.0, Zi = 0.0, p_f = 0.0, p_hz = 0.0, p_bz = 0.0, p_ss = 0.0;
@@ -513,6 +515,12 @@
 #endif
   return nb10_sticky || opt.nb10_always || ff.pqeq || selfcheck || opt.spmv_win == 0 || opt.nonbond_win == 0 || opt.spmv_no_win || !win_valid;
 }
+int Engine::stream_place_cap() const {
+#ifdef RXMD_EXPERIMENTS
+  return 0;
+#endif
+  return opt.streams_by_place != 0 ? rows10 : 0;
+}
 void Engine::require_nb10() {
   if (nb10_valid) return;
   nb10_sticky = true;
@@ -538,7 +546,7 @@
 #define RX_LIST10_F(SC, PQF, OR, F)                                                                                                            \
   k_list10<SC, PQF, OR, F><<<std::max(win_groups, 1) * (WIN_ROWS / L10_ROWS_LAUNCH), 64 * L10_ROWS_LAUNCH, 0, stream>>>(N, S10, grid, rmesh, dff, cellid, cellstart, sorted_xyzi, pos[0], pos[1], pos[2], spos[0], spos[1], spos[2], type, gid, \
                                                     nb10_w, hess, n10, d_err, sorted_shl, shl[0], shl[1], shl[2], hsc, pqrow, sums_from_list ? xs : nullptr, sall, sgh, multi() ? flags : nullptr, \
-                                                    rows_sorted, sl10, rowcols, grp_base, gflag, F ? hess32 : nullptr)
+                                                    rows_sorted, sl10, rowcols, grp_base, gflag, F ? hess32 : nullptr, stream_place_cap())
   const bool f32 = qeq_bits_req == 32 && !ff.pqeq && hess32 != nullptr;
   win_valid = false;
   build_windows();
diff --git a/rxmd_amd/csrc/nonbonded.hip b/rxmd_amd/csrc/nonbonded.hip
--- a/rxmd_amd/csrc/nonbonded.hip
+++ b/rxmd_amd/csrc/nonbonded.hip
@@ -48,7 +48,8 @@
 __global__ void __launch_bounds__(64 * NB_WPB) k_nonbond(int N, int S10, DevFF ff, const int *__restrict__ nb10, const int *__restrict__ n10,
                                                   const double4 *__restrict__ pk, const double *__restrict__ x, const double *__restrict__ y, const double *__restrict__ z,
                                                   const double *__restrict__ q, const int *__restrict__ type,
-                                                  double *__restrict__ fx, double *__restrict__ fy, double *__restrict__ fz, double *__restrict__ pe, int assign) {
+                                                  double *__restrict__ fx, double *__restrict__ fy, double *__restrict__ fz, double *__restrict__ pe, int assign,
+                                                  const int *__restrict__ rplace) {
   __shared__ double sm[NB_WPB][3], sv[NB_WPB][6];
   const int lane = threadIdx.x & 63, w = __builtin_amdgcn_readfirstlane(static_cast<int>(threadIdx.x >> 6));
   if (threadIdx.x < 6 * NB_WPB) sv[threadIdx.x / 6][threadIdx.x % 6] = 0.0;
@@ -59,7 +60,7 @@
     const double xi = x[i], yi = y[i], zi = z[i], qi = q[i];
     const int ti = type[i];
     const int n = n10[i] & N10_COUNT;
-    const size_t row = static_cast<size_t>(i) * S10;
+    const size_t row = static_cast<size_t>(rplace ? rplace[i] : i) * S10;
     const int *ix2 = ff.inxn2 + ti * ff.n1;
     NbAcc acc = {0.0, 0.0, 0.0, 0.0, 0.0, 0.0, 0.0, 0.0, 0.0, 0.0, 0.0};
     for (int k0 = lane; k0 < n; k0 += 64 * NB_UNR) {
@@ -109,7 +110,7 @@
                                                                 const double4 *__restrict__ pk, const unsigned char *__restrict__ stype,
                                                                 const double *__restrict__ x, const double *__restrict__ y, const double *__restrict__ z,
                                                                 const double *__restrict__ q, const int *__restrict__ type,
-                                                                double *__restrict__ fx, double *__restrict__ fy, double *__restrict__ fz, double *__restrict__ pe, int assign) {
+                                                                double *__restrict__ fx, double *__restrict__ fy, double *__restrict__ fz, double *__restrict__ pe, int assign, int byplace) {
   extern __shared__ double4 s_p[];
   unsigned char *s_t = reinterpret_cast<unsigned char *>(s_p + static_cast<size_t>(maxunits) * WIN_UNIT);
   __shared__ double sm[WIN_ROWS][3], sv[WIN_ROWS][6];
@@ -132,7 +133,7 @@
     const double xi = x[i], yi = y[i], zi = z[i], qi = q[i];
     const int ti = type[i];
     const int n = n10[i] & N10_COUNT;
-    const size_t row = static_cast<size_t>(i) * S10;
+    const size_t row = static_cast<size_t>(byplace ? ridx : i) * S10;
     const int *ix2 = ff.inxn2 + ti * ff.n1;
     NbAcc acc = {0.0, 0.0, 0.0, 0.0, 0.0, 0.0, 0.0, 0.0, 0.0, 0.0, 0.0};
     for (int k0 = lane; k0 < n; k0 += 64 * NB_UNR) {
@@ -194,15 +195,15 @@
   const size_t lds = static_cast<size_t>(units) * WIN_UNIT * (sizeof(double4) + 1) + 16;
   if (win_valid && win_env && !list_selfcheck) {
 #define RX_NB_WIN(EN) k_nonbond_win<EN><<<win_groups, 64 * WIN_ROWS, lds, stream>>>(N, G, S10, dff, sl10, n10, rows_sorted, win_k, win_cnt, units, sorted_xyzi, sorted_type, pos[0], pos[1], pos[2], q, type, \
-                                                                 f0, f1, f2, scal + SCAL_PE, assign)
+                                                                 f0, f1, f2, scal + SCAL_PE, assign, streams_by_place ? 1 : 0)
     if (energy) RX_NB_WIN(true); else RX_NB_WIN(false);
 #undef RX_NB_WIN
     RX_HIP(hipGetLastError());
     return;
   }
   require_nb10();
-  if (energy) k_nonbond<true><<<nblk(N, NB_WPB), 64 * NB_WPB, 0, stream>>>(N, S10, dff, nb10, n10, sorted_xyzi, pos[0], pos[1], pos[2], q, type, f0, f1, f2, scal + SCAL_PE, assign);
-  else k_nonbond<false><<<nblk(N, NB_WPB), 64 * NB_WPB, 0, stream>>>(N, S10, dff, nb10, n10, sorted_xyzi, pos[0], pos[1], pos[2], q, type, f0, f1, f2, scal + SCAL_PE, assign);
-}
-
-}
+  if (energy) k_nonbond<true><<<nblk(N, NB_WPB), 64 * NB_WPB, 0, stream>>>(N, S10, dff, nb10, n10, sorted_xyzi, pos[0], pos[1], pos[2], q, type, f0, f1, f2, scal + SCAL_PE, assign, stream_rpos());
+  else k_nonbond<false><<<nblk(N, NB_WPB), 64 * NB_WPB, 0, stream>>>(N, S10, dff, nb10, n10, sorted_xyzi, pos[0], pos[1], pos[2], q, type, f0, f1, f2, scal + SCAL_PE, assign, stream_rpos());
+}
+
+}
diff --git a/rxmd_amd/csrc/pqeq.hip b/rxmd_amd/csrc/pqeq.hip
--- a/rxmd_amd/csrc/pqeq.hip
+++ b/rxmd_amd/csrc/pqeq.hip
@@ -40,7 +40,8 @@
                                                        const double4 *__restrict__ pk, const double4 *__restrict__ sorted_shl,
                                                        const double *__restrict__ x, const double *__restrict__ y, const double *__restrict__ z, const int *__restrict__ type,
                                                        const double *__restrict__ sx, const double *__restrict__ sy, const double *__restrict__ sz,
-                                                       double *__restrict__ nx, double *__restrict__ ny, double *__restrict__ nz, int edir, double efield) {
+                                                       double *__restrict__ nx, double *__restrict__ ny, double *__restrict__ nz, int edir, double efield,
+                                                       const int *__restrict__ rplace) {
   const int lane = threadIdx.x & 63;
   const int i = xcd_swizzle(blockIdx.x, gridDim.x) * (blockDim.x >> 6) + __builtin_amdgcn_readfirstlane(static_cast<int>(threadIdx.x >> 6));
   if (i >= N) return;
@@ -49,7 +50,7 @@
   const double hx = x[i] + s0, hy = y[i] + s1, hz = z[i] + s2;
   const double Zi = ff.Zpq[ti], Ki = ff.Kspq[ti];
   const int n = n10[i] & N10_COUNT;
-  const size_t row = static_cast<size_t>(i) * S10;
+  const size_t row = static_cast<size_t>(rplace ? rplace[i] : i) * S10;
   double f0 = 0.0, f1 = 0.0, f2 = 0.0;
   constexpr int SU = 8;
   for (int k0 = lane; k0 < n; k0 += 64 * SU) {
@@ -96,7 +97,7 @@
   else k_sorted_charge_p<<<nblk(G, 256), 256, 0, stream>>>(G, rootperm, q, sorted_xyzi);
   require_nb10();
   k_shell_update<<<nblk(N, 4), 256, 0, stream>>>(N, S10, dff, nb10, n10, sorted_xyzi, sorted_shl, pos[0], pos[1], pos[2], type, shl[0], shl[1], shl[2], cds, cd, cc_,
-                                                cfg.efield_dir, cfg.efield_strength * 23.060538);
+                                                cfg.efield_dir, cfg.efield_strength * 23.060538, stream_rpos());
   double *tmp[3] = {cds, cd, cc_};
   for (int a = 0; a < 3; ++a) RX_HIP(hipMemcpyAsync(shl[a], tmp[a], sizeof(double) * N, hipMemcpyDeviceToDevice, stream));
   pqeq_sorted_shells();
@@ -108,7 +109,7 @@
                                                        const double *__restrict__ x, const double *__restrict__ y, const double *__restrict__ z,
                                                        const double *__restrict__ q, const int *__restrict__ type,
                                                        const double *__restrict__ sx, const double *__restrict__ sy, const double *__restrict__ sz,
-                                                       double *__restrict__ fx, double *__restrict__ fy, double *__restrict__ fz, double *__restrict__ pe) {
+                                                       double *__restrict__ fx, double *__restrict__ fy, double *__restrict__ fz, double *__restrict__ pe, const int *__restrict__ rplace) {
   __shared__ double sm[4][3], sv[4][6];
   const int lane = threadIdx.x & 63, w = __builtin_amdgcn_readfirstlane(static_cast<int>(threadIdx.x >> 6));
   if (threadIdx.x < 24) sv[threadIdx.x / 6][threadIdx.x % 6] = 0.0;
@@ -121,7 +122,7 @@
     const int ti = type[i];
     const double Zi = ff.Zpq[ti], qic = qi + Zi;
     const int n = n10[i] & N10_COUNT;
-    const size_t row = static_cast<size_t>(i) * S10;
+    const size_t row = static_cast<size_t>(rplace ? rplace[i] : i) * S10;
     const int *ix2 = ff.inxn2 + ti * ff.n1;
     double f0 = 0.0, f1 = 0.0, f2 = 0.0;
     double v0 = 0.0, v1 = 0.0, v2 = 0.0, v3 = 0.0, v4 = 0.0, v5 = 0.0;
@@ -203,7 +204,7 @@
 void Engine::nonbonded_pqeq() {
   require_nb10();
   k_nonbond_pqeq<<<nblk(N, 4), 256, 0, stream>>>(N, S10, dff, nb10, n10, sorted_xyzi, sorted_shl, pos[0], pos[1], pos[2], q, type, shl[0], shl[1], shl[2],
-                                                frc[0], frc[1], frc[2], scal + SCAL_PE);
-}
-
-}
+                                                frc[0], frc[1], frc[2], scal + SCAL_PE, stream_rpos());
+}
+
+}
diff --git a/rxmd_amd/csrc/qeq.hip b/rxmd_amd/csrc/qeq.hip
--- a/rxmd_amd/csrc/qeq.hip
+++ b/rxmd_amd/csrc/qeq.hip
@@ -308,6 +308,7 @@
 WinPassArgs Engine::win_args(bool roword) const {
   WinPassArgs a{N, G, S10, dff, sl10, hess, hess32, n10, rows_sorted, win_k, win_cnt, xs, hst, gst, qst, q, type, scal, partials, wall, wgh, hsc, pqrow,
                 nullptr, win_groups, 0, nullptr, win_flag, 0, win_maxunits, stream};
+  a.byplace = streams_by_place;
   if (roword) { a.n10 = r_n10; a.type = r_type; a.hst = r_hst; a.gst = r_gst; a.rs_all = r_wall; a.rs_gh = r_wgh; a.roword = 1; }
   return a;
 }
@@ -347,6 +348,7 @@
     return a.ngroups;
   }
   RowPassArgs a = row_args();
+  a.rplace = stream_rpos();
   a.rs_all = c.ra; a.rs_gh = c.rg; a.rowlist = c.rowlist; a.nrows = c.nrows; a.pbase = c.pbase; a.stopflag = c.stopflag;
   st.spmv_nstep = 0; st.spmv_var = 0;
   qeq_bits_used = 64;
diff --git a/rxmd_amd/csrc/spmv_kernels.h b/rxmd_amd/csrc/spmv_kernels.h
--- a/rxmd_amd/csrc/spmv_kernels.h
+++ b/rxmd_amd/csrc/spmv_kernels.h
@@ -39,7 +39,8 @@
                                                const double *__restrict__ scal, double *__restrict__ partials,
                                                double2 *__restrict__ rs_all, double2 *__restrict__ rs_gh,
                                                const double *__restrict__ hsc, const double4 *__restrict__ pqrow, int swz,
-                                               const int *__restrict__ rowlist, int nrows, int pbase, const double *__restrict__ stopflag) {
+                                               const int *__restrict__ rowlist, int nrows, int pbase, const double *__restrict__ stopflag,
+                                               const int *__restrict__ rplace = nullptr) {
   if (stopflag && *stopflag != 0.0) return;
   const int lane = threadIdx.x & 63;
   const int wpb = blockDim.x >> 6;
@@ -48,7 +49,7 @@
   __shared__ double s_row[16][4];
   const int wave_in_wg = __builtin_amdgcn_readfirstlane(static_cast<int>(threadIdx.x >> 6));
   if (row < N) {
-    const size_t base = static_cast<size_t>(row) * S10;
+    const size_t base = static_cast<size_t>(rplace ? rplace[row] : row) * S10;
     unsigned e[UNR];
     double h[UNR], c[UNR];
     auto request = [&](int kb, int bound, unsigned (&ee)[UNR], double (&hh)[UNR], double (&cc)[UNR]) {
@@ -126,7 +127,7 @@
 template <class VT> struct WinVal;
 template <> struct WinVal<double> { typedef double2 pair; static __device__ inline pair make(double a, double b) { return make_double2(a, b); } };
 template <> struct WinVal<float> { typedef float2 pair; static __device__ inline pair make(float a, float b) { return make_float2(a, b); } };
-template <int MODE, bool STORE, bool PQ, int NSTEP = 2, int VAR = 0, class VT = double>
+template <int MODE, bool STORE, bool PQ, int NSTEP = 2, int VAR = 0, class VT = double, bool BP = false>
 __global__ void __launch_bounds__(64 * WIN_ROWS, 8) k_spmv_win(int N, int G, int S10, DevFF ff, const unsigned short *__restrict__ sl10, const VT *__restrict__ hess, const int *__restrict__ n10,
                                                             const int *__restrict__ rows_sorted, const int *__restrict__ win_k, const int *__restrict__ win_cnt,
                                                             const double2 *__restrict__ xv, const double2 *__restrict__ hst, double2 *__restrict__ gst,
@@ -152,24 +153,41 @@
   const int grp = grouplist ? (gidx < ngroups ? grouplist[gidx] : -1) : (gidx < ngroups ? gidx : -1);
   if (grp < 0) return;
   const int ridx = grp * WIN_ROWS + wave;
-  const int row = min(rows_sorted[ridx], N);
-  const int nslots = WIN_UNIT * win_cnt[grp];
   const int *wk = win_k + static_cast<size_t>(grp) * WIN_MAXUNITS;
   const int t0 = threadIdx.x, t1 = threadIdx.x + NT;
   const int wk0 = wk[t0 / WIN_UNIT], wk1 = wk[t1 / WIN_UNIT];
+  hpair v[STEPS]; double2 c[STEPS]; unsigned ss[STEPS];
+  if (BP) {
+    static_assert(128 * STEPS <= WIN_BP_MIN_STRIDE, "the first batch of a place is requested without a bound test");
+    const size_t pbase_ = static_cast<size_t>(ridx) * S10;
+    const h2v *ph = reinterpret_cast<const h2v *>(hess + pbase_);
+    const d2v *pc = reinterpret_cast<const d2v *>(PQ ? hsc + pbase_ : nullptr);
+    const unsigned *ps = reinterpret_cast<const unsigned *>(sl10 + pbase_);
+#pragma unroll
+    for (int u = 0; u < STEPS; ++u) {
+      const int k2 = 64 * u + lane;
+      const h2v t2 = __builtin_nontemporal_load(ph + k2); v[u] = WinVal<VT>::make(t2.x, t2.y);
+      ss[u] = __builtin_nontemporal_load(ps + k2);
+      if (PQ && (MODE == MODE_GRAD || STORE)) { const d2v t3 = __builtin_nontemporal_load(pc + k2); c[u] = make_double2(t3.x, t3.y); }
+    }
+  }
+  int rt1_row = 0, rt1_cnt = 0, rt1_flag = 1;
+  if constexpr (BP) {
+    const int *p_row = rows_sorted + ridx, *p_cnt = win_cnt + grp, *p_flag = gflags ? gflags + grp : win_cnt + grp;
+    asm volatile("s_load_dword %0, %3, 0x0\n\ts_load_dword %1, %4, 0x0\n\ts_load_dword %2, %5, 0x0\n\ts_waitcnt lgkmcnt(0)"
+                 : "=&s"(rt1_row), "=&s"(rt1_cnt), "=&s"(rt1_flag) : "s"(p_row), "s"(p_cnt), "s"(p_flag) : "memory");
+  } else { rt1_row = rows_sorted[ridx]; rt1_cnt = win_cnt[grp]; }
+  const int row = min(rt1_row, N);
+  const int nslots = WIN_UNIT * rt1_cnt;
   const bool live = row < N;
 #ifdef RXMD_EXPERIMENTS
-  const size_t base = static_cast<size_t>(live ? ((VAR & WIN_RANKROWS) ? ridx : row) : 0) * S10;
+  const size_t base = static_cast<size_t>(BP ? ridx : (live ? ((VAR & WIN_RANKROWS) ? ridx : row) : 0)) * S10;
 #else
-  const size_t base = static_cast<size_t>(live ? row : 0) * S10;
+  const size_t base = static_cast<size_t>(BP ? ridx : (live ? row : 0)) * S10;
 #endif
   const h2v *hv2 = reinterpret_cast<const h2v *>(hess + base);
   const d2v *cv2 = reinterpret_cast<const d2v *>(PQ ? hsc + base : nullptr);
   const unsigned *sl2 = reinterpret_cast<const unsigned *>(sl10 + base);
-  const bool gh = !((VAR & WIN_LEAN) != 0 && !PQ && gflags != nullptr) || gflags[grp] != 0;
-  auto whole = [&](auto ghc) {
-  constexpr bool GHC = decltype(ghc)::value;
-  hpair v[STEPS]; double2 c[STEPS]; unsigned ss[STEPS];
   auto request = [&](int kb, int bound) {
 #pragma unroll
     for (int u = 0; u < STEPS; ++u) {
@@ -180,10 +198,13 @@
       if (PQ && (MODE == MODE_GRAD || STORE)) { if (ok) { const d2v t2 = __builtin_nontemporal_load(cv2 + (k >> 1)); c[u] = make_double2(t2.x, t2.y); } else c[u] = make_double2(0.0, 0.0); }
     }
   };
+  const bool gh = !((VAR & WIN_LEAN) != 0 && !PQ && gflags != nullptr) || (BP ? rt1_flag : gflags[grp]) != 0;
+  auto whole = [&](auto ghc) {
+  constexpr bool GHC = decltype(ghc)::value;
   double2 x0 = make_double2(0.0, 0.0), x1 = x0;
   if (t0 < nslots) x0 = xv[min(wk0 + (t0 & (WIN_UNIT - 1)), G - 1)];
   if (t1 < nslots) x1 = xv[min(wk1 + (t1 & (WIN_UNIT - 1)), G - 1)];
-  request(0, live ? S10 : 0);
+  if (!BP) request(0, live ? S10 : 0);
   const int rowc = live ? (roword ? ridx : row) : 0;
   const int n = live ? (n10[rowc] & N10_COUNT) : 0;
   const int tl_t = type[rowc];
@@ -292,13 +313,17 @@
   const double2 *xv, *hst; double2 *gst; const double2 *qst; const double *q; const int *type; const double *scal; double *partials; double2 *rs_all, *rs_gh; const double *hsc; const double4 *pqrow;
   const int *grouplist; int ngroups, pbase; const double *stopflag; const int *gflags; int roword;
   int win_maxunits; hipStream_t stream;
+  bool byplace = false;
 };
 template <int MODE, bool STORE, bool PQ, int NSTEP = 2, int VAR = 0, class VT = double>
 inline void launch_win(const WinPassArgs &a) {
   const VT *values = [&] { if constexpr (std::is_same<VT, float>::value) return a.hess32; else return a.hess; }();
-  k_spmv_win<MODE, STORE, PQ, NSTEP, VAR, VT><<<a.ngroups, 64 * WIN_ROWS, static_cast<size_t>(a.win_maxunits) * WIN_UNIT * sizeof(double2), a.stream>>>(
-      a.N, a.G, a.S10, a.ff, a.sl10, values, a.n10, a.rows_sorted, a.win_k, a.win_cnt, a.xv, a.hst, a.gst, a.qst, a.q, a.type, a.scal, a.partials, a.rs_all, a.rs_gh, a.hsc, a.pqrow,
-      a.grouplist, a.ngroups, a.pbase, a.stopflag, a.gflags, a.roword);
+  auto go = [&](auto bp) {
+    k_spmv_win<MODE, STORE, PQ, NSTEP, VAR, VT, decltype(bp)::value><<<a.ngroups, 64 * WIN_ROWS, static_cast<size_t>(a.win_maxunits) * WIN_UNIT * sizeof(double2), a.stream>>>(
+        a.N, a.G, a.S10, a.ff, a.sl10, values, a.n10, a.rows_sorted, a.win_k, a.win_cnt, a.xv, a.hst, a.gst, a.qst, a.q, a.type, a.scal, a.partials, a.rs_all, a.rs_gh, a.hsc, a.pqrow,
+        a.grouplist, a.ngroups, a.pbase, a.stopflag, a.gflags, a.roword);
+  };
+  if (a.byplace) go(std::true_type{}); else go(std::false_type{});
 }
 constexpr int SPMV_WPB = 16;
 struct RowPassArgs {
@@ -306,12 +331,13 @@
   const double2 *xv, *hst; double2 *gst; const double2 *qst; const double *q; const int *type; const double *scal; double *partials;
   double2 *rs_all, *rs_gh; const double *hsc; const double4 *pqrow; int swz; const int *rowlist; int nrows, pbase; const double *stopflag;
   hipStream_t stream;
+  const int *rplace = nullptr;
   int nblocks() const { return nblk(rowlist ? nrows : N, SPMV_WPB); }
 };
 template <int MODE, bool STORE, bool PQ, int PIPE>
 inline void launch_row(const RowPassArgs &a) {
   k_spmv<MODE, STORE, PQ, PIPE><<<a.nblocks(), 64 * SPMV_WPB, 0, a.stream>>>(a.N, a.S10, a.ff, a.nb10, a.hess, a.n10, a.xv, a.hst, a.gst, a.qst, a.q, a.type, a.scal, a.partials, a.rs_all, a.rs_gh, a.hsc, a.pqrow, a.swz,
-                                                                            a.rowlist, a.nrows, a.pbase, a.stopflag);
+                                                                            a.rowlist, a.nrows, a.pbase, a.stopflag, a.rplace);
 }
 
 template <class F> inline double timed_launches_ms(Engine &e, int warm, int reps, F &&launch) {
```

New measurement: 24.92, median of 6. 3.6% higher.
